# adahbingee/pais-mvs

Measured on AMD Instinct MI355X. Metric: refined+expanded patches/sec, higher is better.
Workload: dtype f64

## Files before the change

### include/pais_test_hooks.h

```cpp
#ifndef PAIS_TEST_HOOKS_H
#define PAIS_TEST_HOOKS_H

#include "pais_feature.h"
#include "pais_mvs.h"

#ifdef __cplusplus
extern "C" {
#endif

int  pais_mvs_emulate(pais_mvs *m, int mode, int rank, int world);

typedef int (*pais_record_source_fn)(void *user, int n, const pais_candidate *cands, pais_patch_result *out, int has_seeds);
int  pais_mvs_set_record_source(pais_mvs *m, pais_record_source_fn fn, void *user);

int  pais_mvs_test_inject(pais_mvs *m, int what, int count);

typedef struct pais_test_swarm {
    double range_l[3], range_u[3];
    double iw, gbest_fitness;
    uint64_t stream_base;
    int32_t n, max_iteration, iteration, g_idx, started, run, local_k, continues;
    double result[4];
} pais_test_swarm;
int  pais_test_swarm_step(int device, pais_test_swarm *s, double *swarm);

typedef struct pais_test_feature_sizes {
    int32_t octaves, W, H, layers;
    int64_t num_cands, num_fit, num_keypoints;
} pais_test_feature_sizes;
int  pais_test_feature_stages(int device, const uint8_t *gray, int width, int height, int64_t stride,
                              const pais_feature_params *prm, int octave, pais_test_feature_sizes *sizes,
                              int64_t layer_floats, float *layers, int max_cands, int32_t *cands, int32_t *fit_int, double *fit_val);

#ifdef __cplusplus
}
#endif
#endif
```

### pais_mvs_amd/csrc/pais_capi.hip

```cpp
#include <hip/hip_runtime.h>
#include <limits.h>
#include <math.h>
#include <stdarg.h>
#include <stddef.h>
#include <stdio.h>
#include <stdlib.h>
#include <string.h>

#include <string>
#include <utility>
#include <vector>
#include <algorithm>

#include "../../include/pais_hip.h"
#include "../../include/pais_test_hooks.h"
#include "pais_dev.hpp"
#include "pais_host.hpp"
#include "pais_internal.h"

static thread_local std::string g_err;
static int fail(const char *what, hipError_t e)
{
    char buf[512];
    snprintf(buf, sizeof(buf), "%s: %s", what, hipGetErrorString(e));
    g_err = buf;
    return -2;
}
static int fail_msg(const char *what)
{
    g_err = what;
    return -1;
}
__attribute__((format(printf, 1, 2))) static int fail_fmt(const char *fmt, ...)
{
    char buf[512];
    va_list ap;
    va_start(ap, fmt);
    vsnprintf(buf, sizeof(buf), fmt, ap);
    va_end(ap);
    return fail_msg(buf);
}
#define HIPCHK(call)                                   \
    do {                                               \
        hipError_t e__ = (call);                       \
        if (e__ != hipSuccess) return fail(#call, e__); \
    } while (0)

struct EventPair {
    hipEvent_t a, b;
};

struct pais_ctx;
struct Timed {
    pais_ctx *ctx = nullptr;
    hipStream_t st = nullptr;
    std::vector<EventPair> *into = nullptr;
    EventPair e{nullptr, nullptr};
    bool on = false;
    int begin(pais_ctx *c, hipStream_t s, std::vector<EventPair> *v);
    int end();
};
struct LaunchStats {
    double ms = 0;
    int64_t launches = 0, items = 0;
};
struct TimedLaunch {
    pais_ctx *ctx;
    EventPair e{nullptr, nullptr};
    explicit TimedLaunch(pais_ctx *c) : ctx(c) {}
    TimedLaunch(TimedLaunch &&o) noexcept : ctx(o.ctx), e(o.e) { o.e = EventPair{nullptr, nullptr}; }
    ~TimedLaunch();
    int begin();
    int end();
    void collect(LaunchStats &s, int64_t items, int64_t launches = 1);
};
struct TraceOut {
    pais_launch::TraceSink sink{nullptr, nullptr, nullptr, 1, 1};
    std::vector<TimedLaunch> passes;
    int64_t launches = 0;
};
struct PassPlan {
    struct Slice { int lo, hi, parts; pais_launch::BatchView v; pais_launch::TraceSink trace; };
    pais_launch::BatchView all{};
    int nSl = 0, S = 1, afterGrid = 0, itNext = 0;
    bool useIter = false, useTile = false, useRing = false, hasSeeds = false;
    bool usePre = false;
    int ringCUs = 0;
    Slice sl[16];
    int *cnt = nullptr, *nextCnt = nullptr;
    const pais_candidate *d_cands = nullptr;
    Timed tp;
    TraceOut *trace = nullptr;
};

struct pais_ctx {
    int device = 0;
    hipStream_t stream = nullptr;
    int numCUs = 256;
    size_t ldsLimit = 64 * 1024;
    DevScene sc;
    DevBuf<DevCamera> d_cams;
    DevBuf<uint8_t> d_img;
    DevBuf<PaisImgT> d_imgF;
    DevBuf<double> d_edge;
    bool edgesOnTheFly = false;
    DevBuf<double> d_gauss;
    size_t imgBytes = 0, edgeBytes = 0;
    std::vector<int> camMaxLod;
    DevBuf<pais_candidate> d_cands;
    DevBuf<pais_patch_result> d_recs;
    PinBuf<pais_candidate> h_cands;
    PinBuf<pais_patch_result> h_recs;
    DevBuf<double> d_hp;
    DevBuf<double> d_ratios;
    DevBuf<int> d_counters;
    unsigned passSerial = 0;
    bool countersDirty = false;
    DevBuf<unsigned char> d_evalBlocks;
    DevBuf<unsigned char> d_win;
    DevBuf<int> d_active;
    DevBuf<unsigned long long> d_stat;
    unsigned long long *stat = nullptr;
    PinBuf<int> h_counters;
    DevBuf<unsigned char> d_psoStates;
    long splitAbove = 0;
    int psoMinPer = 64;
    int evalParts = 0;
    double partFill = 0.5;
    int psoStreams = 2;
    pais_launch::TileOpts tile;
    int arithLiteral = 0;
    bool tileVerify = false;
    bool tileDebug = false;
    int tileMode = 1;
    long tileAbove = 512;
    std::vector<hipStream_t> sub;
    std::vector<hipEvent_t> subDone;
    hipEvent_t forkEv = nullptr;
    DevBuf<pais_patch_state> d_states;
    DevBuf<int32_t> d_idx;
    DevBuf<double> d_particles, d_out;
    DevBuf<pais_view_state> d_vStates;
    DevBuf<pais_view_result> d_vOut;
    DevBuf<double> d_vTables, d_vHp;
    LaunchStats ncc;
    DevBuf<pais_loaded_patch> d_lIn;
    DevBuf<pais_patch_result> d_lOut;
    LaunchStats load;
    DevBuf<pais_patch_state> d_dStates;
    DevBuf<int32_t> d_dIdx;
    DevBuf<double> d_dParticles, d_dWeight, d_dSad, d_dColour, d_dH;
    DevBuf<pais_cost_detail> d_dRec;
    DevBuf<int8_t> d_dCode;
    LaunchStats detail;
    DevBuf<pais_candidate> d_tCands;
    DevBuf<pais_patch_result> d_tRecs;
    DevBuf<pais_pso_run_info> d_tRuns;
    DevBuf<pais_pso_iter> d_tIters;
    DevBuf<double> d_tParts;
    DevBuf<unsigned long long> d_tStat;
    LaunchStats trace;
    DevBuf<double> d_nbC;
    DevBuf<int32_t> d_nbN;
    bool fineTiming = false;
    std::vector<EventPair> evPso, evBegin, evAfter, evEval, evEval2;
    std::vector<EventPair> evFree;
    double psoMs = 0, beginMs = 0, afterMs = 0, evalMs = 0, eval2Ms = 0;
    hipEvent_t refEv = nullptr;
    std::vector<std::pair<float, float>> eval2Intervals;
    int64_t psoLaunches = 0, evalLaunches = 0, eval2Launches = 0, tileLaunches = 0, ringLaunches = 0;
    pais_ctx *parent = nullptr;
    std::vector<pais_ctx *> lanes;
    int openBatch = -1;
    double ringPerCam = 1843.0;
    int ringMode = 1;
    int preMode = 1;
    DevBuf<double> d_pre;
    DevBuf<unsigned> d_ring;
    DevBuf<unsigned> d_ringCtl;
    PinBuf<unsigned> h_ringCtl;
    DevBuf<int> d_arrive;
    bool ringUsed = false;
    bool ringSuppressed = false;
    bool ringSuppressOnce = false;
    int ringPendingN = 0;
    double ringTimeoutMs = 10000.0;
    long ringSeedAbove = 0;
    size_t ringMaxBytes = (size_t)512 << 20;
    int64_t ringFallbacks = 0;
    std::vector<EventPair> evRing;
    double ringMs = 0;
    PassPlan plan;
    bool planDone = true;
    int roundHint = 0;
};

static void build_gauss(const pais_config &cfg, std::vector<double> &g)
{
    const int S = cfg.patchSize, r = cfg.patchRadius;
    g.assign((size_t)S * S, 0.0);
    const double sigma = cfg.distWeighting;
    const double s2 = 1.0 / (2.0 * sigma * sigma);
    const double s = 1.0 / (2.0 * M_PI * sigma * sigma);
    for (int x = 0; x < S; ++x)
        for (int y = 0; y < S; ++y) {
            double e = -(pow((double)(x - r), 2) + pow((double)(y - r), 2)) * s2;
            g[(size_t)x * S + y] = s * exp(e);
        }
    double n = 0;
    for (size_t i = 0; i < g.size(); ++i) n += g[i];
    const double inv = 1.0 / n;
    for (size_t i = 0; i < g.size(); ++i) g[i] = g[i] * inv;
}

static int apply_config(pais_ctx *ctx, const pais_config *cfg)
{
    pais_config c = *cfg;
    c.patchSize = (c.patchRadius << 1) + 1;
    if (c.patchRadius < 1 || c.patchRadius > 127) return fail_msg("patchRadius out of range");
    if (c.particleNum < 1 || c.particleNum * 2 > PAIS_MAX_PARTICLES) return fail_msg("particleNum out of range");
    if (c.maxLOD < 0 || c.maxLOD >= PAIS_MAX_LEVELS) return fail_msg("maxLOD out of range");
    if (c.minLOD < 0) return fail_msg("minLOD out of range (negative)");
    if (!(c.textureVariation > 0)) return fail_msg("textureVariation out of range (must be > 0)");
    if (!(c.lodRatio > 0 && c.lodRatio < 1)) return fail_msg("lodRatio out of range (must be inside (0, 1))");
    if (c.maxIteration < 1) return fail_msg("maxIteration out of range (must be >= 1)");
    if (c.cellSize < 1) return fail_msg("cellSize out of range (must be >= 1)");
    std::vector<double> g;
    build_gauss(c, g);
    if (ctx->d_gauss) HIPCHK(hipStreamSynchronize(ctx->stream));
    HIPCHK(ctx->d_gauss.alloc(g.size() * sizeof(double)));
    HIPCHK(hipMemcpy(ctx->d_gauss, g.data(), g.size() * sizeof(double), hipMemcpyHostToDevice));
    ctx->sc.cfg = c;
    ctx->sc.gauss = ctx->d_gauss;
    for (int l = 0; l < PAIS_MAX_LEVELS; ++l) ctx->sc.lodScale[l] = pow(c.lodRatio, l);
    return 0;
}

extern "C" const char *pais_last_error(void) { return g_err.c_str(); }
extern "C" size_t pais_sizeof_config(void) { return sizeof(pais_config); }
extern "C" size_t pais_sizeof_camera_desc(void) { return sizeof(pais_camera_desc); }
extern "C" size_t pais_sizeof_candidate(void) { return sizeof(pais_candidate); }
extern "C" size_t pais_sizeof_patch_result(void) { return sizeof(pais_patch_result); }
extern "C" size_t pais_sizeof_view_state(void) { return sizeof(pais_view_state); }
extern "C" size_t pais_sizeof_view_result(void) { return sizeof(pais_view_result); }
extern "C" size_t pais_sizeof_cost_detail(void) { return sizeof(pais_cost_detail); }
extern "C" size_t pais_sizeof_pso_run_info(void) { return sizeof(pais_pso_run_info); }
extern "C" size_t pais_sizeof_pso_iter(void) { return sizeof(pais_pso_iter); }
static_assert(offsetof(pais_pso_run_info, range_u) == 24 && offsetof(pais_pso_run_info, init) == 48 && offsetof(pais_pso_run_info, ray) == 72 &&
              offsetof(pais_pso_run_info, run) == 96 && offsetof(pais_pso_run_info, n_particles) == 112 &&
              offsetof(pais_pso_run_info, iterations) == 120 && offsetof(pais_pso_run_info, cam_idx) == 128 &&
              sizeof(pais_pso_run_info) == 128 + 4 * PAIS_MAX_VIS, "pais_pso_run_info layout");
static_assert(offsetof(pais_pso_iter, gbest) == 8 && offsetof(pais_pso_iter, iw) == 32 && offsetof(pais_pso_iter, dispersion) == 40 &&
              offsetof(pais_pso_iter, velocity) == 48 && offsetof(pais_pso_iter, g_idx) == 56 && offsetof(pais_pso_iter, ended) == 64 &&
              sizeof(pais_pso_iter) == 72, "pais_pso_iter layout");
extern "C" uint32_t pais_rand31(uint64_t seed, uint64_t key, uint32_t run, uint32_t k) { return pais::rand31(seed, key, run, k); }
extern "C" uint64_t pais_child_key(uint64_t parent_key, int cam, int cx, int cy) { return pais::child_key(parent_key, cam, cx, cy); }

static int ctx_init(pais_ctx *ctx, const pais_config *cfg, int num_cams, const pais_camera_desc *cams, int device, uint64_t pso_seed);
static int ctx_init_work(pais_ctx *ctx);
extern "C" int pais_ctx_create(const pais_config *cfg, int num_cams, const pais_camera_desc *cams, int device,
                               uint64_t pso_seed, pais_ctx **out)
{
    if (!cfg || !cams || !out || num_cams <= 0) return fail_msg("pais_ctx_create: bad argument");
    int ndev = 0;
    hipError_t e0 = hipGetDeviceCount(&ndev);
    if (e0 != hipSuccess || ndev <= 0) return fail_msg("pais_ctx_create: no HIP device (this library has no CPU path)");
    if (device < 0 || device >= ndev) return fail_msg("pais_ctx_create: bad device index");
    HIPCHK(hipSetDevice(device));
    pais_ctx *ctx = new pais_ctx();
    const int rc = ctx_init(ctx, cfg, num_cams, cams, device, pso_seed);
    if (rc) { pais_ctx_destroy(ctx); return rc; }
    *out = ctx;
    return 0;
}

static int ctx_init(pais_ctx *ctx, const pais_config *cfg, int num_cams, const pais_camera_desc *cams, int device, uint64_t pso_seed)
{
    ctx->device = device;
    memset(&ctx->sc, 0, sizeof(ctx->sc));
    hipDeviceProp_t prop;
    HIPCHK(hipGetDeviceProperties(&prop, device));
    ctx->numCUs = prop.multiProcessorCount > 0 ? prop.multiProcessorCount : 256;
    ctx->ldsLimit = prop.sharedMemPerBlock > 0 ? (size_t)prop.sharedMemPerBlock : 64 * 1024;
    HIPCHK(hipStreamCreateWithFlags(&ctx->stream, hipStreamNonBlocking));
    ctx->sc.seed = pso_seed;
    ctx->sc.numCams = num_cams;
    int rc = apply_config(ctx, cfg);
    if (rc) return rc;
    const bool wantEdge = cfg->adaptiveGradientEnable != 0;
    const bool edgesGiven = wantEdge && cams[0].level_edge[0] != nullptr;

    std::vector<DevCamera> hc((size_t)num_cams);
    std::vector<size_t> imgOff((size_t)num_cams * PAIS_MAX_LEVELS, 0), edgeOff((size_t)num_cams * PAIS_MAX_LEVELS, 0);
    size_t imgBytes = 0, edgeBytes = 0;
    for (int c = 0; c < num_cams; ++c) {
        const pais_camera_desc &d = cams[c];
        if (d.max_lod < 0 || d.max_lod >= PAIS_MAX_LEVELS) return fail_msg("camera max_lod out of range");
        for (int l = 0; l <= d.max_lod; ++l) {
            if (!d.level_image[l] || d.level_width[l] <= 0 || d.level_height[l] <= 0) return fail_msg("camera level missing");
            if (d.level_width[l] > 65535 || d.level_height[l] > 65535) return fail_msg("camera level larger than 65535 pixels in one dimension");
            size_t px = (size_t)d.level_width[l] * d.level_height[l];
            if (px >= ((size_t)1 << 29)) return fail_msg("camera level of 2^29 pixels or more (32-bit tap offsets inside a level)");
            imgOff[(size_t)c * PAIS_MAX_LEVELS + l] = imgBytes;
            imgBytes = (imgBytes + px + 16 + 255) & ~(size_t)255;
            if (wantEdge && edgesGiven) {
                if (!d.level_edge[l]) return fail_msg("level_edge given for some levels only");
                edgeOff[(size_t)c * PAIS_MAX_LEVELS + l] = edgeBytes;
                edgeBytes = (edgeBytes + px * sizeof(double) + 255) & ~(size_t)255;
            }
        }
    }
    if (imgBytes >= ((size_t)1 << 40)) return fail_msg("pyramids of 2^40 bytes or more (a level's start is packed into 40 bits next to its homography)");
    HIPCHK(ctx->d_img.alloc(imgBytes));
    HIPCHK(hipMemsetAsync(ctx->d_img, 0, imgBytes, ctx->stream));
    for (int c = 0; c < num_cams; ++c) {
        const pais_camera_desc &d = cams[c];
        for (int l = 0; l <= d.max_lod; ++l) {
            const int w = d.level_width[l], h = d.level_height[l];
            const size_t stride = d.level_stride[l] > 0 ? (size_t)d.level_stride[l] : (size_t)w;
            HIPCHK(hipMemcpy2DAsync(ctx->d_img + imgOff[(size_t)c * PAIS_MAX_LEVELS + l], (size_t)w, d.level_image[l], stride, (size_t)w,
                                    (size_t)h, hipMemcpyHostToDevice, ctx->stream));
        }
    }
    ctx->imgBytes = imgBytes;
    {
        size_t maxMB = 256;
        if (const char *e = getenv("PAIS_TAP_FLOAT_MAX_MB")) maxMB = (size_t)strtoull(e, nullptr, 10);
        if (imgBytes <= (maxMB << 20)) {
            HIPCHK(ctx->d_imgF.alloc(imgBytes * sizeof(PaisImgT)));
            HIPCHK(pais_launch::expand_image(ctx->d_img, ctx->d_imgF, imgBytes, ctx->stream));
        }
    }
    if (wantEdge && edgesGiven && edgeBytes) {
        HIPCHK(ctx->d_edge.alloc(edgeBytes));
        for (int c = 0; c < num_cams; ++c) {
            const pais_camera_desc &d = cams[c];
            for (int l = 0; l <= d.max_lod; ++l) {
                size_t px = (size_t)d.level_width[l] * d.level_height[l];
                HIPCHK(hipMemcpyAsync((uint8_t *)ctx->d_edge.p + edgeOff[(size_t)c * PAIS_MAX_LEVELS + l], d.level_edge[l],
                                      px * sizeof(double), hipMemcpyHostToDevice, ctx->stream));
            }
        }
        ctx->edgeBytes = edgeBytes;
    }
    std::vector<unsigned long long> mm;
    if (wantEdge && !edgesGiven) {
        mm.assign((size_t)num_cams * PAIS_MAX_LEVELS * 2, 0ULL);
        for (size_t i = 0; i < mm.size(); i += 2) mm[i] = ~0ULL;
        DevBuf<unsigned long long> d_mm;
        HIPCHK(d_mm.alloc(mm.size() * sizeof(unsigned long long)));
        HIPCHK(hipMemcpyAsync(d_mm, mm.data(), mm.size() * sizeof(unsigned long long), hipMemcpyHostToDevice, ctx->stream));
        for (int c = 0; c < num_cams; ++c)
            for (int l = 0; l <= cams[c].max_lod; ++l)
                HIPCHK(pais_launch::level_edge_minmax(ctx->d_img + imgOff[(size_t)c * PAIS_MAX_LEVELS + l], cams[c].level_width[l],
                                                      cams[c].level_height[l], d_mm + ((size_t)c * PAIS_MAX_LEVELS + l) * 2, ctx->stream));
        HIPCHK(hipMemcpyAsync(mm.data(), d_mm, mm.size() * sizeof(unsigned long long), hipMemcpyDeviceToHost, ctx->stream));
        HIPCHK(hipStreamSynchronize(ctx->stream));
    }
    HIPCHK(hipStreamSynchronize(ctx->stream));
    ctx->edgesOnTheFly = wantEdge && !edgesGiven;
    for (int c = 0; c < num_cams; ++c) {
        const pais_camera_desc &d = cams[c];
        DevCamera &h = hc[c];
        memset(&h, 0, sizeof(h));
        memcpy(h.KR, d.KR, sizeof(h.KR));
        memcpy(h.KT, d.KT, sizeof(h.KT));
        memcpy(h.R, d.rotation, sizeof(h.R));
        memcpy(h.T, d.translation, sizeof(h.T));
        memcpy(h.C, d.center, sizeof(h.C));
        memcpy(h.optN, d.optical_normal, sizeof(h.optN));
        h.focal[0] = d.focal[0]; h.focal[1] = d.focal[1];
        h.pp[0] = d.principle_point[0]; h.pp[1] = d.principle_point[1];
        h.maxLOD = d.max_lod;
        ctx->camMaxLod.push_back(d.max_lod);
        for (int l = 0; l <= d.max_lod; ++l) {
            h.w[l] = d.level_width[l];
            h.h[l] = d.level_height[l];
            h.imgOff[l] = (uint64_t)imgOff[(size_t)c * PAIS_MAX_LEVELS + l];
            h.edgeOff[l] = (uint64_t)(edgeOff[(size_t)c * PAIS_MAX_LEVELS + l] / sizeof(double));
            if (!mm.empty()) {
                const unsigned long long lo = mm[((size_t)c * PAIS_MAX_LEVELS + l) * 2], hi = mm[((size_t)c * PAIS_MAX_LEVELS + l) * 2 + 1];
                memcpy(&h.edgeMin[l], &lo, 8);
                memcpy(&h.edgeMax[l], &hi, 8);
            }
        }
    }
    HIPCHK(ctx->d_cams.alloc(sizeof(DevCamera) * (size_t)num_cams));
    HIPCHK(hipMemcpy(ctx->d_cams, hc.data(), sizeof(DevCamera) * (size_t)num_cams, hipMemcpyHostToDevice));
    ctx->sc.cams = ctx->d_cams;
    ctx->sc.imgBlob = ctx->d_img;
    ctx->sc.imgF = ctx->d_imgF;
    ctx->sc.edgeBlob = ctx->d_edge;

    return ctx_init_work(ctx);
}

template <typename T> static void env_int(const char *name, T &v, long lo = LONG_MIN, long hi = LONG_MAX)
{
    const char *e = getenv(name);
    if (!e) return;
    const long x = atol(e);
    if (x >= lo && x <= hi) v = (T)x;
}
template <typename T> static void env_flag(const char *name, T &v)
{
    if (const char *e = getenv(name)) v = atoi(e) != 0;
}
static void env_real(const char *name, double &v, bool positiveOnly = false)
{
    const char *e = getenv(name);
    if (!e) return;
    const double x = atof(e);
    if (!positiveOnly || x > 0) v = x;
}
static int staging_chunk(const char *envName, int n, size_t perItemBytes)
{
    double mb = 256.0;
    env_real(envName, mb);
    const size_t bound = (size_t)std::max(0.0, mb * 1048576.0);
    return (int)std::min((size_t)n, std::max((size_t)1, bound / perItemBytes));
}

static int ctx_init_work(pais_ctx *ctx)
{
    HIPCHK(ctx->d_counters.alloc(sizeof(int) * 8));
    HIPCHK(hipMemset(ctx->d_counters, 0, sizeof(int) * 8));
    HIPCHK(ctx->d_stat.alloc(sizeof(unsigned long long) * 24));
    HIPCHK(hipMemset(ctx->d_stat, 0, sizeof(unsigned long long) * 24));
    ctx->stat = ctx->d_stat;
    HIPCHK(ctx->h_counters.alloc(sizeof(int) * 4));
    HIPCHK(ctx->d_ringCtl.alloc(PAIS_RING_CTL_BYTES * PAIS_RINGS));
    HIPCHK(hipMemset(ctx->d_ringCtl, 0, PAIS_RING_CTL_BYTES * PAIS_RINGS));
    HIPCHK(ctx->h_ringCtl.alloc(PAIS_RING_CTL_BYTES * PAIS_RINGS));
    memset(ctx->h_ringCtl, 0, PAIS_RING_CTL_BYTES * PAIS_RINGS);
    ctx->splitAbove = 3L * ctx->numCUs * 12;
    env_int("PAIS_EVAL_PARTS", ctx->evalParts, 1, 4);
    if (ctx->evalParts == 3) ctx->evalParts = 0;
    env_real("PAIS_PART_FILL", ctx->partFill, true);
    env_int("PAIS_SPLIT_ABOVE", ctx->splitAbove, 1);
    env_int("PAIS_PSO_MINPER", ctx->psoMinPer, 1, INT_MAX);
    env_int("PAIS_PSO_STREAMS", ctx->psoStreams, 1, 16);
    env_int("PAIS_PSO_RING", ctx->ringMode, INT_MIN, INT_MAX);
    env_int("PAIS_PRE_SETUP", ctx->preMode, INT_MIN, INT_MAX);
    env_real("PAIS_RING_PER_CAM", ctx->ringPerCam);
    env_int("PAIS_RING_SEED_ABOVE", ctx->ringSeedAbove);
    long ringMaxMB = 0;
    env_int("PAIS_RING_MAX_MB", ringMaxMB, 1);
    if (ringMaxMB) ctx->ringMaxBytes = (size_t)ringMaxMB << 20;
    env_int("PAIS_TILE", ctx->tileMode, INT_MIN, INT_MAX);
    env_flag("PAIS_TILE_DEBUG", ctx->tileDebug);
    env_flag("PAIS_TILE_VERIFY", ctx->tileVerify);
    env_int("PAIS_TILE_STRIP_SPLIT", ctx->tile.stripSteps, 1, INT_MAX);
    env_flag("PAIS_TILE_NOTILES", ctx->tile.noTiles);
    env_int("PAIS_TILE_ABOVE", ctx->tileAbove, 1);
    env_flag("PAIS_FINE_TIMING", ctx->fineTiming);
    if (const char *e = getenv("PAIS_ARITH")) ctx->arithLiteral = (strcmp(e, "literal") == 0);
    if (const char *e = getenv("PAIS_RING_TIMEOUT_MS")) {
        const double v = atof(e);
        if (v == 0.0 && e[0] == '0') ctx->ringTimeoutMs = 0.0;
        else if (v >= 1.0 && v <= 600000.0) ctx->ringTimeoutMs = v;
        else fprintf(stderr, "pais: PAIS_RING_TIMEOUT_MS=%s ignored (0, or 1 .. 600000 ms)\n", e);
    }
    HIPCHK(hipEventCreateWithFlags(&ctx->forkEv, hipEventDisableTiming));
    for (int i = 0; i + 1 < ctx->psoStreams; ++i) {
        hipStream_t st; hipEvent_t ev;
        HIPCHK(hipStreamCreateWithFlags(&st, hipStreamNonBlocking));
        HIPCHK(hipEventCreateWithFlags(&ev, hipEventDisableTiming));
        ctx->sub.push_back(st);
        ctx->subDone.push_back(ev);
    }
    return 0;
}

extern "C" void pais_ctx_destroy(pais_ctx *ctx)
{
    if (!ctx) return;
    (void)hipSetDevice(ctx->device);
    if (ctx->parent) {
        auto &v = ctx->parent->lanes;
        for (size_t i = 0; i < v.size(); ++i)
            if (v[i] == ctx) { v.erase(v.begin() + (long)i); break; }
        ctx->parent = nullptr;
    }
    while (!ctx->lanes.empty()) {
        pais_ctx *l = ctx->lanes.back();
        ctx->lanes.pop_back();
        l->parent = nullptr;
        pais_ctx_destroy(l);
    }
    if (ctx->stream) (void)hipStreamSynchronize(ctx->stream);
    for (auto *v : {&ctx->evPso, &ctx->evBegin, &ctx->evAfter, &ctx->evEval, &ctx->evEval2, &ctx->evRing, &ctx->evFree})
        for (auto &p : *v) { (void)hipEventDestroy(p.a); (void)hipEventDestroy(p.b); }
    for (auto st : ctx->sub) (void)hipStreamDestroy(st);
    for (auto ev : ctx->subDone) (void)hipEventDestroy(ev);
    if (ctx->forkEv) (void)hipEventDestroy(ctx->forkEv);
    if (ctx->refEv) (void)hipEventDestroy(ctx->refEv);
    pais_launch::ring_profile_print();
    if (ctx->stream) (void)hipStreamDestroy(ctx->stream);
    delete ctx;
}

extern "C" int pais_ctx_set_config(pais_ctx *ctx, const pais_config *cfg)
{
    if (!ctx || !cfg) return fail_msg("pais_ctx_set_config: bad argument");
    HIPCHK(hipSetDevice(ctx->device));
    if (cfg->adaptiveGradientEnable && !ctx->d_edge && !ctx->edgesOnTheFly)
        return fail_msg("adaptiveGradientEnable needs the gradient weighting enabled at create time (edge pyramids or their on-the-fly statistics)");
    if (ctx->parent) return fail_msg("pais_ctx_set_config: a lane takes its configuration from its parent");
    if (ctx->openBatch >= 0) return fail_msg("pais_ctx_set_config: a batch is open on this context");
    for (pais_ctx *l : ctx->lanes)
        if (l->openBatch >= 0) return fail_msg("pais_ctx_set_config: a batch is open on a lane of this context");
    for (pais_ctx *l : ctx->lanes) HIPCHK(hipStreamSynchronize(l->stream));
    int rc = apply_config(ctx, cfg);
    if (rc) return rc;
    for (pais_ctx *l : ctx->lanes) {
        l->sc.cfg = ctx->sc.cfg;
        l->sc.gauss = ctx->sc.gauss;
        for (int i = 0; i < PAIS_MAX_LEVELS; ++i) l->sc.lodScale[i] = ctx->sc.lodScale[i];
    }
    return 0;
}

extern "C" int pais_ctx_fork_lane(pais_ctx *parent, pais_ctx **out)
{
    if (!parent || !out) return fail_msg("pais_ctx_fork_lane: bad argument");
    if (parent->parent) return fail_msg("pais_ctx_fork_lane: a lane cannot be forked");
    HIPCHK(hipSetDevice(parent->device));
    pais_ctx *l = new pais_ctx();
    l->device = parent->device;
    l->numCUs = parent->numCUs;
    l->ldsLimit = parent->ldsLimit;
    l->camMaxLod = parent->camMaxLod;
    l->sc = parent->sc;
    l->edgesOnTheFly = parent->edgesOnTheFly;
    l->imgBytes = parent->imgBytes;
    l->edgeBytes = parent->edgeBytes;
    hipError_t e = hipStreamCreateWithFlags(&l->stream, hipStreamNonBlocking);
    if (e != hipSuccess) { delete l; return fail("hipStreamCreateWithFlags", e); }
    const int rc = ctx_init_work(l);
    if (rc) { pais_ctx_destroy(l); return rc; }
    l->fineTiming = parent->fineTiming;
    l->parent = parent;
    parent->lanes.push_back(l);
    *out = l;
    return 0;
}

extern "C" int pais_ctx_set_neighbor_radius(pais_ctx *ctx, double r)
{
    if (!ctx) return fail_msg("bad ctx");
    ctx->sc.cfg.neighborRadius = r;
    for (pais_ctx *l : ctx->lanes) l->sc.cfg.neighborRadius = r;
    return 0;
}

extern "C" void *pais_ctx_stream(pais_ctx *ctx) { return ctx ? (void *)ctx->stream : nullptr; }
extern "C" int pais_ctx_synchronize(pais_ctx *ctx)
{
    if (!ctx) return fail_msg("bad ctx");
    HIPCHK(hipSetDevice(ctx->device));
    HIPCHK(hipStreamSynchronize(ctx->stream));
    return 0;
}

static int get_event_pair(pais_ctx *ctx, EventPair &p)
{
    if (!ctx->evFree.empty()) {
        p = ctx->evFree.back();
        ctx->evFree.pop_back();
        return 0;
    }
    EventPair q{nullptr, nullptr};
    HIPCHK(hipEventCreate(&q.a));
    const hipError_t e = hipEventCreate(&q.b);
    if (e != hipSuccess) { (void)hipEventDestroy(q.a); return fail("hipEventCreate", e); }
    p = q;
    return 0;
}
static int drain_events(pais_ctx *ctx, std::vector<EventPair> &v, double &acc)
{
    for (auto &p : v) {
        float ms = 0;
        HIPCHK(hipEventElapsedTime(&ms, p.a, p.b));
        acc += ms;
        ctx->evFree.push_back(p);
    }
    v.clear();
    return 0;
}
int Timed::begin(pais_ctx *c, hipStream_t s, std::vector<EventPair> *v)
{
    ctx = c; st = s; into = v; on = c->fineTiming;
    if (!on) return 0;
    if (get_event_pair(c, e)) return -2;
    HIPCHK(hipEventRecord(e.a, s));
    return 0;
}
int Timed::end()
{
    if (!on) return 0;
    HIPCHK(hipEventRecord(e.b, st));
    into->push_back(e);
    return 0;
}

TimedLaunch::~TimedLaunch()
{
    if (e.a) ctx->evFree.push_back(e);
}
int TimedLaunch::begin()
{
    if (get_event_pair(ctx, e)) return -2;
    HIPCHK(hipEventRecord(e.a, ctx->stream));
    return 0;
}
int TimedLaunch::end()
{
    HIPCHK(hipEventRecord(e.b, ctx->stream));
    return 0;
}
void TimedLaunch::collect(LaunchStats &s, int64_t items, int64_t launches)
{
    float ms = 0;
    if (hipEventElapsedTime(&ms, e.a, e.b) == hipSuccess) s.ms += ms;
    s.launches += launches;
    s.items += items;
}

static int read_launch_stats(LaunchStats *s, const char *who, double *kernel_ms, int64_t *launches, int64_t *items, int reset)
{
    if (!s) return fail_fmt("%s: bad argument", who);
    if (kernel_ms) *kernel_ms = s->ms;
    if (launches) *launches = s->launches;
    if (items) *items = s->items;
    if (reset) *s = LaunchStats();
    return 0;
}

struct CamListRules {
    const char *who, *noun;
    int minCam;
    bool distinct;
    enum Ref {
        NoRef,
        AnyLevel,
        OwnLevels
    } ref;
};
static const CamListRules kFitnessRules = {"pais_fitness_batch", "state", 1, false, CamListRules::AnyLevel};
static const CamListRules kDetailRules = {"pais_fitness_detail", "state", 1, false, CamListRules::AnyLevel};
static const CamListRules kNccRules = {"pais_ncc_batch", "state", 2, true, CamListRules::OwnLevels};
static CamListRules candidate_rules(const char *who) { return CamListRules{who, "candidate", 0, false, CamListRules::NoRef}; }

static int check_cam_list(const pais_ctx *ctx, const CamListRules &R, int i, int num_cam, const int32_t *cam_idx, int ref_cam, int lod)
{
    const int nc = ctx->sc.numCams;
    if (num_cam < R.minCam || num_cam > PAIS_MAX_VIS)
        return fail_fmt("%s: %s %d: num_cam %d outside [%d, %d]", R.who, R.noun, i, num_cam, R.minCam, PAIS_MAX_VIS);
    if (R.ref != CamListRules::NoRef && (ref_cam < 0 || ref_cam >= nc))
        return fail_fmt("%s: %s %d: ref_cam %d out of range [0, %d)", R.who, R.noun, i, ref_cam, nc);
    for (int k = 0; k < num_cam; ++k) {
        const int c = cam_idx[k];
        bool twice = false;
        for (int j = 0; R.distinct && j < k; ++j) twice = twice || cam_idx[j] == c;
        if (c >= 0 && c < nc && !twice) continue;
        if (R.distinct)
            return fail_fmt("%s: %s %d: %s (cam_idx[%d] = %d)", R.who, R.noun, i, c < 0 || c >= nc ? "cam_idx out of range" : "duplicate camera in cam_idx",
                            k, c);
        return fail_fmt("%s: %s %d: cam_idx[%d] = %d out of range [0, %d)", R.who, R.noun, i, k, c, nc);
    }
    if (R.ref == CamListRules::AnyLevel && (lod < 0 || lod >= PAIS_MAX_LEVELS))
        return fail_fmt("%s: %s %d: lod %d outside [0, %d)", R.who, R.noun, i, lod, PAIS_MAX_LEVELS);
    if (R.ref == CamListRules::OwnLevels) {
        int maxLod = ctx->camMaxLod[ref_cam], lim = ref_cam;
        for (int k = 0; k < num_cam; ++k)
            if (ctx->camMaxLod[cam_idx[k]] < maxLod) {
                maxLod = ctx->camMaxLod[cam_idx[k]];
                lim = cam_idx[k];
            }
        if (lod < 0 || lod > maxLod)
            return fail_fmt("%s: %s %d: lod %d outside [0, %d] (max_lod of camera %d)", R.who, R.noun, i, lod, maxLod, lim);
    }
    return 0;
}

static int check_states(const pais_ctx *ctx, const CamListRules &R, int n_states, const pais_patch_state *states, int n_evals,
                        const int32_t *state_index, int &Kmax)
{
    Kmax = 1;
    for (int i = 0; i < n_states; ++i) {
        const pais_patch_state &s = states[i];
        const int rc = check_cam_list(ctx, R, i, s.num_cam, s.cam_idx, s.ref_cam, s.lod);
        if (rc) return rc;
        Kmax = std::max(Kmax, (int)s.num_cam);
    }
    for (int e = 0; e < n_evals; ++e)
        if (state_index[e] < 0 || state_index[e] >= n_states)
            return fail_fmt("%s: state_index[%d] = %d out of range [0, %d)", R.who, e, state_index[e], n_states);
    return 0;
}

static int check_candidates(const pais_ctx *ctx, const char *who, int n, const pais_candidate *cands, int &Kmax, int &hasSeeds)
{
    const CamListRules R = candidate_rules(who);
    Kmax = 1;
    hasSeeds = 0;
    for (int i = 0; i < n; ++i) {
        const pais_candidate &c = cands[i];
        const int rc = check_cam_list(ctx, R, i, c.num_cam, c.cam_idx, 0, 0);
        if (rc) return rc;
        if (c.type != PAIS_TYPE_SEED && c.type != PAIS_TYPE_EXPAND)
            return fail_fmt("%s: candidate %d: type %d is neither PAIS_TYPE_SEED nor PAIS_TYPE_EXPAND", who, i, c.type);
        Kmax = std::max(Kmax, (int)c.num_cam);
        if (c.type == PAIS_TYPE_SEED) hasSeeds = 1;
    }
    return 0;
}

extern "C" int pais_neighbor_count(pais_ctx *ctx, int n, const double *centers, double radius, int32_t *counts, double *kernel_ms)
{
    if (!ctx || n < 0 || (n && (!centers || !counts))) return fail_msg("pais_neighbor_count: bad argument");
    if (kernel_ms) *kernel_ms = 0;
    if (n == 0) return 0;
    HIPCHK(hipSetDevice(ctx->device));
    HIPCHK(ctx->d_nbC.reserve(ctx->stream, sizeof(double) * 3 * (size_t)n));
    HIPCHK(ctx->d_nbN.reserve(ctx->stream, sizeof(int32_t) * (size_t)n));
    HIPCHK(hipMemcpyAsync(ctx->d_nbC, centers, sizeof(double) * 3 * (size_t)n, hipMemcpyHostToDevice, ctx->stream));
    TimedLaunch t(ctx);
    if (t.begin()) return -2;
    HIPCHK(pais_launch::neighbor_count(ctx->d_nbC, n, radius, ctx->d_nbN, ctx->stream));
    if (t.end()) return -2;
    HIPCHK(hipMemcpyAsync(counts, ctx->d_nbN, sizeof(int32_t) * (size_t)n, hipMemcpyDeviceToHost, ctx->stream));
    HIPCHK(hipStreamSynchronize(ctx->stream));
    LaunchStats s;
    t.collect(s, n);
    if (kernel_ms) *kernel_ms = s.ms;
    return 0;
}

extern "C" int pais_ctx_set_fine_timing(pais_ctx *ctx, int on)
{
    if (!ctx) return fail_msg("pais_ctx_set_fine_timing: bad argument");
    if (on && !ctx->parent) {
        HIPCHK(hipSetDevice(ctx->device));
        if (!ctx->refEv) HIPCHK(hipEventCreate(&ctx->refEv));
        HIPCHK(hipEventRecord(ctx->refEv, ctx->stream));
        HIPCHK(hipStreamSynchronize(ctx->stream));
    }
    ctx->fineTiming = on != 0;
    for (pais_ctx *l : ctx->lanes) l->fineTiming = on != 0;
    return 0;
}

extern "C" int pais_fitness_batch(pais_ctx *ctx, int n_states, const pais_patch_state *states, int n_evals,
                                  const int32_t *state_index, const double *particles, double *out)
{
    if (!ctx || n_states < 0 || n_evals < 0) return fail_msg("pais_fitness_batch: bad argument");
    if (n_evals == 0) return 0;
    if (!states || !state_index || !particles || !out) return fail_msg("pais_fitness_batch: null pointer");
    HIPCHK(hipSetDevice(ctx->device));
    int Kmax = 1;
    const int rc = check_states(ctx, kFitnessRules, n_states, states, n_evals, state_index, Kmax);
    if (rc) return rc;
    HIPCHK(ctx->d_states.reserve(ctx->stream, sizeof(pais_patch_state) * (size_t)n_states));
    HIPCHK(ctx->d_idx.reserve(ctx->stream, sizeof(int32_t) * (size_t)n_evals));
    HIPCHK(ctx->d_particles.reserve(ctx->stream, sizeof(double) * 3 * (size_t)n_evals));
    HIPCHK(ctx->d_out.reserve(ctx->stream, sizeof(double) * (size_t)n_evals));
    HIPCHK(ctx->d_evalBlocks.reserve(ctx->stream, pais_launch::eval_block_bytes_host(Kmax) * (size_t)n_states));
    HIPCHK(ctx->d_win.reserve(ctx->stream, pais_launch::win_bytes_per_candidate(ctx->sc) * (size_t)n_states));
    HIPCHK(hipMemcpyAsync(ctx->d_states, states, sizeof(pais_patch_state) * (size_t)n_states, hipMemcpyHostToDevice, ctx->stream));
    HIPCHK(hipMemcpyAsync(ctx->d_idx, state_index, sizeof(int32_t) * (size_t)n_evals, hipMemcpyHostToDevice, ctx->stream));
    HIPCHK(hipMemcpyAsync(ctx->d_particles, particles, sizeof(double) * 3 * (size_t)n_evals, hipMemcpyHostToDevice, ctx->stream));
    Timed tf;
    if (tf.begin(ctx, ctx->stream, &ctx->evEval)) return -2;
    HIPCHK(pais_launch::fitness(ctx->sc, ctx->d_states, n_states, ctx->d_idx, ctx->d_particles, ctx->d_out, n_evals, Kmax,
                                ctx->d_evalBlocks, ctx->d_win, ctx->arithLiteral, ctx->stream));
    if (tf.end()) return -2;
    ctx->evalLaunches++;
    HIPCHK(hipMemcpyAsync(out, ctx->d_out, sizeof(double) * (size_t)n_evals, hipMemcpyDeviceToHost, ctx->stream));
    HIPCHK(hipStreamSynchronize(ctx->stream));
    return 0;
}

extern "C" int pais_ncc_batch(pais_ctx *ctx, int n, const pais_view_state *states, pais_view_result *out, double *tables, int stride)
{
    if (!ctx || n < 0) return fail_msg("pais_ncc_batch: bad argument");
    if (n == 0) return 0;
    if (!states || !out) return fail_msg("pais_ncc_batch: null pointer");
    if (tables && stride < 2) return fail_msg("pais_ncc_batch: table stride below 2");
    int Kmax = 2;
    for (int i = 0; i < n; ++i) {
        const pais_view_state &v = states[i];
        const int rc = check_cam_list(ctx, kNccRules, i, v.num_cam, v.cam_idx, v.ref_cam, v.lod);
        if (rc) return rc;
        if (tables && stride < v.num_cam) return fail_fmt("pais_ncc_batch: state %d: table stride %d below num_cam %d", i, stride, v.num_cam);
        Kmax = std::max(Kmax, (int)v.num_cam);
    }
    HIPCHK(hipSetDevice(ctx->device));
    const DevScene &sc = ctx->sc;
    const size_t hpBytes = sizeof(double) * (size_t)Kmax * sc.cfg.patchSize * sc.cfg.patchSize;
    const int hpInLds = (pais_launch::hp_in_lds(sc, Kmax) && pais_launch::ncc_lds_bytes(Kmax) + hpBytes <= ctx->ldsLimit) ? 1 : 0;
    long grid = (long)ctx->numCUs * (hpInLds ? 8 : 2);
    if (!hpInLds) {
        const long cap = (long)(((size_t)256 << 20) / hpBytes);
        grid = std::min(grid, std::max(1L, cap));
    }
    grid = std::min(grid, (long)n);
    const size_t tableBytes = tables ? sizeof(double) * (size_t)stride * stride * (size_t)n : 0;
    HIPCHK(ctx->d_vStates.reserve(ctx->stream, sizeof(pais_view_state) * (size_t)n));
    HIPCHK(ctx->d_vOut.reserve(ctx->stream, sizeof(pais_view_result) * (size_t)n));
    if (tables) HIPCHK(ctx->d_vTables.reserve(ctx->stream, tableBytes));
    if (!hpInLds) HIPCHK(ctx->d_vHp.reserve(ctx->stream, hpBytes * (size_t)grid));
    HIPCHK(hipMemcpyAsync(ctx->d_vStates, states, sizeof(pais_view_state) * (size_t)n, hipMemcpyHostToDevice, ctx->stream));
    TimedLaunch t(ctx);
    if (t.begin()) return -2;
    HIPCHK(pais_launch::ncc_batch(sc, ctx->d_vStates, n, ctx->d_vOut, tables ? ctx->d_vTables.p : nullptr, stride, ctx->d_vHp, (int)grid, Kmax,
                                  hpInLds, ctx->stream));
    if (t.end()) return -2;
    HIPCHK(hipMemcpyAsync(out, ctx->d_vOut, sizeof(pais_view_result) * (size_t)n, hipMemcpyDeviceToHost, ctx->stream));
    if (tables) HIPCHK(hipMemcpyAsync(tables, ctx->d_vTables, tableBytes, hipMemcpyDeviceToHost, ctx->stream));
    HIPCHK(hipStreamSynchronize(ctx->stream));
    t.collect(ctx->ncc, n);
    return 0;
}

extern "C" int pais_get_ncc_stats(pais_ctx *ctx, double *kernel_ms, int64_t *launches, int64_t *states, int reset)
{
    return read_launch_stats(ctx ? &ctx->ncc : nullptr, "pais_get_ncc_stats", kernel_ms, launches, states, reset);
}

static const CamListRules kLoadRules = {"pais_load_state_batch", "patch", 0, false, CamListRules::NoRef};

extern "C" int pais_load_state_batch(pais_ctx *ctx, int n, const pais_loaded_patch *in, pais_patch_result *out)
{
    if (n < 0) return fail_msg("pais_load_state_batch: bad argument (n < 0)");
    if (n == 0) return 0;
    const char *missing = !ctx ? "ctx" : !in ? "in" : !out ? "out" : nullptr;
    if (missing) return fail_fmt("pais_load_state_batch: null pointer (%s)", missing);
    for (int i = 0; i < n; ++i) {
        const int rc = check_cam_list(ctx, kLoadRules, i, in[i].num_cam, in[i].cam_idx, 0, 0);
        if (rc) return rc;
    }
    HIPCHK(hipSetDevice(ctx->device));
    const int chunk = staging_chunk("PAIS_LOAD_STAGING_MB", n, sizeof(pais_loaded_patch) + sizeof(pais_patch_result));
    HIPCHK(ctx->d_lIn.reserve(ctx->stream, sizeof(pais_loaded_patch) * (size_t)chunk));
    HIPCHK(ctx->d_lOut.reserve(ctx->stream, sizeof(pais_patch_result) * (size_t)chunk));
    for (int c0 = 0; c0 < n; c0 += chunk) {
        const int m = std::min(chunk, n - c0);
        HIPCHK(hipMemcpyAsync(ctx->d_lIn, in + c0, sizeof(pais_loaded_patch) * (size_t)m, hipMemcpyHostToDevice, ctx->stream));
        TimedLaunch t(ctx);
        if (t.begin()) return -2;
        HIPCHK(pais_launch::load_state(ctx->sc, ctx->d_lIn, ctx->d_lOut, m, (uint64_t)c0, ctx->stream));
        if (t.end()) return -2;
        HIPCHK(hipMemcpyAsync(out + c0, ctx->d_lOut, sizeof(pais_patch_result) * (size_t)m, hipMemcpyDeviceToHost, ctx->stream));
        HIPCHK(hipStreamSynchronize(ctx->stream));
        t.collect(ctx->load, m);
    }
    return 0;
}

extern "C" int pais_get_load_stats(pais_ctx *ctx, double *kernel_ms, int64_t *launches, int64_t *patches, int reset)
{
    return read_launch_stats(ctx ? &ctx->load : nullptr, "pais_get_load_stats", kernel_ms, launches, patches, reset);
}
extern "C" size_t pais_sizeof_loaded_patch(void) { return sizeof(pais_loaded_patch); }

extern "C" int pais_fitness_detail(pais_ctx *ctx, int n_states, const pais_patch_state *states, int n_evals, const int32_t *state_index,
                                   const double *particles, pais_cost_detail *out, double *weight, double *avg_sad, int8_t *pixel_code,
                                   double *colour, double *homographies, int cam_stride)
{
    if (!ctx || n_states < 0 || n_evals < 0) return fail_msg("pais_fitness_detail: bad argument");
    if (n_evals == 0) return 0;
    const char *missing = !states ? "states" : !state_index ? "state_index" : !particles ? "particles" : !out ? "out" : !weight ? "weight"
                          : !avg_sad ? "avg_sad" : !pixel_code ? "pixel_code" : nullptr;
    if (missing) return fail_fmt("pais_fitness_detail: null pointer (%s)", missing);
    int Kmax = 1;
    const int rc = check_states(ctx, kDetailRules, n_states, states, n_evals, state_index, Kmax);
    if (rc) return rc;
    for (int i = 0; (colour || homographies) && i < n_states; ++i)
        if (cam_stride < states[i].num_cam)
            return fail_fmt("pais_fitness_detail: state %d: cam_stride %d below num_cam %d", i, cam_stride, states[i].num_cam);
    HIPCHK(hipSetDevice(ctx->device));
    const DevScene &sc = ctx->sc;
    const size_t S2 = (size_t)sc.cfg.patchSize * sc.cfg.patchSize;
    const size_t perEval = sizeof(pais_cost_detail) + sizeof(int32_t) + 3 * sizeof(double) + S2 * (2 * sizeof(double) + 1) +
                           (colour ? sizeof(double) * (size_t)Kmax * S2 : 0) + (homographies ? sizeof(double) * 9 * (size_t)Kmax : 0);
    const int chunk = staging_chunk("PAIS_DETAIL_STAGING_MB", n_evals, perEval);
    hipStream_t st = ctx->stream;
    HIPCHK(ctx->d_dStates.reserve(st, sizeof(pais_patch_state) * (size_t)n_states));
    HIPCHK(ctx->d_evalBlocks.reserve(st, pais_launch::eval_block_bytes_host(Kmax) * (size_t)n_states));
    HIPCHK(ctx->d_win.reserve(st, pais_launch::win_bytes_per_candidate(sc) * (size_t)n_states));
    HIPCHK(ctx->d_dIdx.reserve(st, sizeof(int32_t) * (size_t)chunk));
    HIPCHK(ctx->d_dParticles.reserve(st, 3 * sizeof(double) * (size_t)chunk));
    HIPCHK(ctx->d_dRec.reserve(st, sizeof(pais_cost_detail) * (size_t)chunk));
    HIPCHK(ctx->d_dWeight.reserve(st, sizeof(double) * S2 * chunk));
    HIPCHK(ctx->d_dSad.reserve(st, sizeof(double) * S2 * chunk));
    HIPCHK(ctx->d_dCode.reserve(st, S2 * chunk));
    if (colour) HIPCHK(ctx->d_dColour.reserve(st, sizeof(double) * (size_t)Kmax * S2 * chunk));
    if (homographies) HIPCHK(ctx->d_dH.reserve(st, sizeof(double) * 9 * (size_t)Kmax * chunk));
    HIPCHK(hipMemcpyAsync(ctx->d_dStates, states, sizeof(pais_patch_state) * (size_t)n_states, hipMemcpyHostToDevice, ctx->stream));
    HIPCHK(pais_launch::state_blocks(sc, ctx->d_dStates, n_states, Kmax, ctx->d_evalBlocks, ctx->d_win, ctx->stream));
    std::vector<double> hCol(colour ? (size_t)Kmax * S2 * chunk : 0), hH(homographies ? (size_t)9 * Kmax * chunk : 0);
    for (int c0 = 0; c0 < n_evals; c0 += chunk) {
        const int n = std::min(chunk, n_evals - c0);
        HIPCHK(hipMemcpyAsync(ctx->d_dIdx, state_index + c0, sizeof(int32_t) * (size_t)n, hipMemcpyHostToDevice, ctx->stream));
        HIPCHK(hipMemcpyAsync(ctx->d_dParticles, particles + 3 * (size_t)c0, 3 * sizeof(double) * (size_t)n, hipMemcpyHostToDevice, ctx->stream));
        TimedLaunch t(ctx);
        if (t.begin()) return -2;
        HIPCHK(pais_launch::fitness_detail(sc, ctx->d_dIdx, ctx->d_dParticles, n, Kmax, ctx->d_evalBlocks, ctx->d_dRec, ctx->d_dWeight, ctx->d_dSad,
                                           ctx->d_dCode, colour ? ctx->d_dColour.p : nullptr, homographies ? ctx->d_dH.p : nullptr, ctx->stream));
        if (t.end()) return -2;
        HIPCHK(hipMemcpyAsync(out + c0, ctx->d_dRec, sizeof(pais_cost_detail) * (size_t)n, hipMemcpyDeviceToHost, ctx->stream));
        HIPCHK(hipMemcpyAsync(weight + S2 * c0, ctx->d_dWeight, sizeof(double) * S2 * n, hipMemcpyDeviceToHost, ctx->stream));
        HIPCHK(hipMemcpyAsync(avg_sad + S2 * c0, ctx->d_dSad, sizeof(double) * S2 * n, hipMemcpyDeviceToHost, ctx->stream));
        HIPCHK(hipMemcpyAsync(pixel_code + S2 * c0, ctx->d_dCode, S2 * n, hipMemcpyDeviceToHost, ctx->stream));
        if (colour) HIPCHK(hipMemcpyAsync(hCol.data(), ctx->d_dColour, sizeof(double) * (size_t)Kmax * S2 * n, hipMemcpyDeviceToHost, ctx->stream));
        if (homographies) HIPCHK(hipMemcpyAsync(hH.data(), ctx->d_dH, sizeof(double) * 9 * (size_t)Kmax * n, hipMemcpyDeviceToHost, ctx->stream));
        HIPCHK(hipStreamSynchronize(ctx->stream));
        t.collect(ctx->detail, n);
        for (int e = 0; e < n; ++e) {
            const size_t K = (size_t)states[state_index[c0 + e]].num_cam, g = (size_t)c0 + e;
            if (colour) memcpy(colour + g * cam_stride * S2, hCol.data() + (size_t)e * Kmax * S2, sizeof(double) * K * S2);
            if (homographies) memcpy(homographies + g * cam_stride * 9, hH.data() + (size_t)e * Kmax * 9, sizeof(double) * K * 9);
        }
    }
    return 0;
}

extern "C" int pais_get_detail_stats(pais_ctx *ctx, double *kernel_ms, int64_t *launches, int64_t *evals, int reset)
{
    return read_launch_stats(ctx ? &ctx->detail : nullptr, "pais_get_detail_stats", kernel_ms, launches, evals, reset);
}

static int pass_open(pais_ctx *ctx, PassPlan &P, int pass, int againCount)
{
    const DevScene &sc = ctx->sc;
    P.cnt = ctx->d_counters + 4 * (ctx->passSerial & 1);
    P.nextCnt = ctx->d_counters + 4 * ((ctx->passSerial + 1) & 1);
    ctx->passSerial++;
    if (P.tp.begin(ctx, ctx->stream, &ctx->evPso)) return -2;
    if (pass > 0)
        HIPCHK(pais_launch::pso_init(sc, P.all, ctx->d_active, P.cnt + 2));
    const bool tileOk = (ctx->tileMode == 2 || (ctx->tileMode == 1 && ctx->sc.imgF == nullptr)) && pais_launch::tile_eligible(P.all.Kmax);
    const int n = P.all.n, Nmax = P.all.Nmax;
    const int nPlan = ctx->roundHint > n ? ctx->roundHint : n;
    P.useIter = Nmax <= 64 && (long)nPlan * Nmax < (tileOk ? ctx->tileAbove : ctx->splitAbove);
    P.useTile = tileOk && !P.useIter;
    if (ctx->arithLiteral) P.useIter = P.useTile = false;
    const long ringWaves = (long)(P.hasSeeds && pass > 0 ? againCount : n) * Nmax;
    const size_t ringNeed = pais_launch::ring_words(n, Nmax, P.all.maxIt) * sizeof(unsigned);
    P.useRing = ctx->ringMode != 0 && !ctx->arithLiteral && !ctx->ringSuppressed && !P.useTile && Nmax <= 64 && n < (1 << 24) && ringNeed <= ctx->ringMaxBytes &&
                (P.hasSeeds ? (ctx->ringSeedAbove > 0 && ringWaves >= ctx->ringSeedAbove)
                            : (!P.useIter && ringWaves >= (long)(ctx->ringPerCam * P.all.Kmax)));
    if (P.useRing && nPlan > n && ctx->ringMode != 3) P.useRing = false;
    if (P.trace) P.useIter = P.useTile = P.useRing = false;
    if (P.useRing) P.useIter = false;
    P.ringCUs = ctx->numCUs;
    if (P.useRing) {
        HIPCHK(ctx->d_ring.reserve(ctx->stream, ringNeed));
        HIPCHK(ctx->d_arrive.reserve(ctx->stream, sizeof(int) * PAIS_ARRIVE_STRIDE * (size_t)n));
    }
    P.usePre = ctx->preMode != 0 && !ctx->arithLiteral && !P.useIter && !P.useTile && !(P.useRing && !pais_launch::pre_ring_ok(P.all.Kmax)) && !P.trace;
    P.all.pre = nullptr;
    if (P.usePre) {
        HIPCHK(ctx->d_pre.reserve(ctx->stream, pais_launch::pre_bytes_per_candidate(Nmax, P.all.Kmax) * (size_t)n));
        P.all.pre = ctx->d_pre;
        HIPCHK(pais_launch::pso_setup0(sc, P.all));
    }
    const int nRun = P.useIter ? (pass == 0 ? n : againCount) : n;
    int S = P.useRing ? 1 : ctx->psoStreams;
    if (nPlan > n) S = (int)((double)S * n / nPlan + 0.5);
    const int minPer = ctx->psoMinPer;
    if (nRun < S * minPer) S = (nRun + minPer - 1) / minPer;
    if (S < 1 || P.trace) S = 1;
    P.S = S;
    if (S > 1) HIPCHK(hipEventRecord(ctx->forkEv, ctx->stream));
    P.nSl = 0;
    for (int sI = 0; sI < S; ++sI) {
        PassPlan::Slice q;
        q.lo = (int)((long)nRun * sI / S);
        q.hi = (int)((long)nRun * (sI + 1) / S);
        if (q.hi <= q.lo) continue;
        const bool own = (S == 1) || (sI == 0);
        const hipStream_t st = own ? ctx->stream : ctx->sub[sI - 1];
        if (!own) HIPCHK(hipStreamWaitEvent(st, ctx->forkEv, 0));
        q.v = P.useIter ? P.all.slice(sc, 0, n, st) : P.all.slice(sc, q.lo, q.hi, st);
        q.trace = pais_launch::TraceSink{nullptr, nullptr, nullptr, 1, 1};
        if (P.trace) {
            const pais_launch::TraceSink &t = P.trace->sink;
            const size_t slot0 = (size_t)q.lo * t.maxRuns;
            q.trace = pais_launch::TraceSink{t.runs + slot0, t.iters + slot0 * t.rows, t.particles ? t.particles + slot0 * t.rows * Nmax * 11 : nullptr,
                                             t.maxRuns, t.rows};
        }
        q.parts = 1;
        if (P.useIter) {
            const long waves = (long)(q.hi - q.lo) * Nmax, resident = (long)((double)ctx->numCUs * 16 * ctx->partFill * n / nPlan);
            q.parts = ctx->evalParts > 0 ? ctx->evalParts : (waves * 4 <= resident ? 4 : (waves * 2 <= resident ? 2 : 1));
        }
        P.sl[P.nSl++] = q;
    }
    P.itNext = 0;
    return 0;
}

static int pass_iterations(pais_ctx *ctx, PassPlan &P, int itEnd)
{
    const DevScene &sc = ctx->sc;
    if (itEnd > P.all.maxIt + 1) itEnd = P.all.maxIt + 1;
    if (P.useRing) {
        if (P.itNext == 0 && itEnd > 0) {
            const unsigned long long ticks = (unsigned long long)(ctx->ringTimeoutMs * 1e5);
            auto ring = [&](int phase) {
                return pais_launch::pso_ring(sc, P.all, ctx->d_ring, ctx->d_ringCtl, ctx->d_arrive, ctx->stat, P.ringCUs, phase, ticks);
            };
            HIPCHK(ring(0));
            Timed te;
            if (te.begin(ctx, ctx->stream, &ctx->evRing)) return -2;
            HIPCHK(ring(1));
            if (te.end()) return -2;
            HIPCHK(hipMemcpyAsync(ctx->h_ringCtl, ctx->d_ringCtl, PAIS_RING_CTL_BYTES * PAIS_RINGS, hipMemcpyDeviceToHost, ctx->stream));
            ctx->ringUsed = true;
            ctx->evalLaunches++;
            ctx->eval2Launches++;
            ctx->ringLaunches++;
            P.itNext = P.all.maxIt + 1;
        }
        return 0;
    }
    TimedLaunch tpass(ctx);
    const bool timePass = P.trace && itEnd > P.itNext;
    if (timePass && tpass.begin()) return -2;
    for (int it = P.itNext; it < itEnd; ++it) {
        for (int k = 0; k < P.nSl; ++k) {
            const PassPlan::Slice &q = P.sl[k];
            Timed te;
            if (te.begin(ctx, q.v.stream, P.useIter ? &ctx->evEval : &ctx->evEval2)) return -2;
            if (P.useIter)
                HIPCHK(pais_launch::pso_iter(sc, q.v, ctx->d_active, P.cnt + 2, q.lo, q.hi, ctx->stat, it, 0, q.parts));
            else if (P.useTile) {
                HIPCHK(pais_launch::pso_tile(sc, q.v, ctx->tile, ctx->tileDebug ? ctx->stat + 8 : nullptr));
                HIPCHK(pais_launch::pso_eval(sc, q.v, ctx->tileVerify ? 2 : 1, ctx->stat + 18));
            } else if (ctx->arithLiteral)
                HIPCHK(pais_launch::pso_eval_literal(sc, q.v));
            else
                HIPCHK(pais_launch::pso_eval(sc, q.v, 0, nullptr));
            if (te.end()) return -2;
            ctx->evalLaunches++;
            if (!P.useIter) ctx->eval2Launches++;
            if (P.useTile) ctx->tileLaunches++;
            if (P.trace) {
                HIPCHK(pais_launch::pso_step_trace(sc, q.v, ctx->stat, q.trace));
                P.trace->launches++;
            } else if (!P.useIter)
                HIPCHK(pais_launch::pso_step(sc, q.v, ctx->stat));
        }
    }
    if (timePass) {
        if (tpass.end()) return -2;
        P.trace->passes.push_back(std::move(tpass));
    }
    if (itEnd > P.itNext) P.itNext = itEnd;
    return 0;
}

static int pass_join(pais_ctx *ctx, PassPlan &P)
{
    for (int sI = 1; sI < P.S; ++sI) {
        bool used = false;
        for (int k = 0; k < P.nSl; ++k) used = used || (P.sl[k].v.stream == ctx->sub[sI - 1]);
        if (!used) continue;
        HIPCHK(hipEventRecord(ctx->subDone[sI - 1], ctx->sub[sI - 1]));
        HIPCHK(hipStreamWaitEvent(ctx->stream, ctx->subDone[sI - 1], 0));
    }
    P.S = 1;
    return 0;
}

static int pass_close(pais_ctx *ctx, PassPlan &P)
{
    const DevScene &sc = ctx->sc;
    for (int k = 0; k < P.nSl; ++k) {
        const PassPlan::Slice &q = P.sl[k];
        if (P.useIter)
            HIPCHK(pais_launch::pso_iter(sc, q.v, ctx->d_active, P.cnt + 2, q.lo, q.hi, ctx->stat, P.all.maxIt + 1, 1, q.parts));
    }
    if (pass_join(ctx, P)) return -2;
    if (P.tp.end()) return -2;
    ctx->psoLaunches++;
    Timed ta;
    if (ta.begin(ctx, ctx->stream, &ctx->evAfter)) return -2;
    HIPCHK(pais_launch::after(sc, P.all.recs, P.all.n, ctx->d_hp, P.afterGrid, P.cnt, ctx->stat, P.all.Kmax, ctx->d_ratios, P.nextCnt, ctx->stream));
    if (ta.end()) return -2;
    return 0;
}

static int batch_setup(pais_ctx *ctx, PassPlan &P, int n, const pais_candidate *d_cands, pais_patch_result *d_out, int max_num_cam, int has_seeds)
{
    HIPCHK(hipSetDevice(ctx->device));
    const DevScene &sc = ctx->sc;
    int Kmax = max_num_cam > 0 ? max_num_cam : sc.numCams;
    if (Kmax > PAIS_MAX_VIS) Kmax = PAIS_MAX_VIS;
    if (Kmax > sc.numCams) Kmax = sc.numCams;
    if (Kmax < 1) Kmax = 1;
    const int Nmax = has_seeds ? sc.cfg.particleNum * 2 : sc.cfg.particleNum;
    const int S2 = sc.cfg.patchSize * sc.cfg.patchSize;
    const int afterGrid = n < 2048 ? n : 2048;
    {
        size_t hpNeed = (size_t)afterGrid * Kmax * S2 * sizeof(double);
        const size_t full = (size_t)2048 * Kmax * S2 * sizeof(double);
        if (hpNeed > ctx->d_hp.bytes && full < ((size_t)1 << 31)) hpNeed = full;
        HIPCHK(ctx->d_hp.reserve(ctx->stream, hpNeed));
    }
    HIPCHK(ctx->d_active.reserve(ctx->stream, sizeof(int) * (size_t)n));
    HIPCHK(ctx->d_evalBlocks.reserve(ctx->stream, pais_launch::eval_block_bytes_host(Kmax) * (size_t)n));
    HIPCHK(ctx->d_win.reserve(ctx->stream, pais_launch::win_bytes_per_candidate(sc) * (size_t)n));
    HIPCHK(ctx->d_psoStates.reserve(ctx->stream, pais_launch::pso_state_bytes_host(Nmax) * (size_t)n));
    HIPCHK(ctx->d_ratios.reserve(ctx->stream, sizeof(double) * PAIS_MAX_VIS * (size_t)n));
    P.all = pais_launch::BatchView{d_out, ctx->d_psoStates, ctx->d_evalBlocks, ctx->d_win, nullptr, n, Nmax, Kmax,
                                   has_seeds ? sc.cfg.maxIteration * 2 : sc.cfg.maxIteration, ctx->stream};
    P.hasSeeds = has_seeds != 0;
    P.afterGrid = afterGrid;
    P.d_cands = d_cands;

    if (ctx->countersDirty) HIPCHK(hipMemsetAsync(ctx->d_counters, 0, sizeof(int) * 8, ctx->stream));
    ctx->countersDirty = true;
    Timed tb;
    if (tb.begin(ctx, ctx->stream, &ctx->evBegin)) return -2;
    HIPCHK(pais_launch::begin(sc, P.all, d_cands, ctx->d_active, ctx->d_counters + 4 * (ctx->passSerial & 1) + 2));
    if (tb.end()) return -2;
    return 0;
}

static int ring_failed(pais_ctx *ctx, int n)
{
    if (!ctx->ringUsed) return 0;
    ctx->ringUsed = false;
    unsigned done = 0, err = 0;
    for (int r = 0; r < PAIS_RINGS; ++r) { done += ctx->h_ringCtl[(PAIS_RING_CTL_BYTES / 4) * r + PAIS_RING_CTL_DONE_WORD]; err |= ctx->h_ringCtl[(PAIS_RING_CTL_BYTES / 4) * r + PAIS_RING_CTL_ERROR_WORD]; }
    if (err == 0 && done == (unsigned)n) return 0;
    ctx->ringFallbacks++;
    if (getenv("PAIS_RING_VERBOSE") || (ctx->ringFallbacks == 1 && ctx->ringTimeoutMs > 0))
        fprintf(stderr, "[pais] k_pso_ring did not complete (error %u, %u of %d runs ended): the batch is re-run with one launch per iteration\n", err, done, n);
    return 1;
}

static int refine_device_once(pais_ctx *ctx, int n, const pais_candidate *d_cands, pais_patch_result *d_out, int max_num_cam, int has_seeds,
                              bool defer = false, TraceOut *trace = nullptr)
{
    PassPlan &P = ctx->plan;
    P.trace = trace;
    ctx->ringUsed = false;
    ctx->ringPendingN = 0;
    int rc = batch_setup(ctx, P, n, d_cands, d_out, max_num_cam, has_seeds);
    int againCount = 0;
    const int maxPass = has_seeds ? (PAIS_MAX_VIS + 2) : 1;
    for (int pass = 0; !rc && pass < maxPass; ++pass) {
        if ((rc = pass_open(ctx, P, pass, againCount)) != 0) break;
        if ((rc = pass_iterations(ctx, P, P.all.maxIt + 1)) != 0) { (void)pass_join(ctx, P); break; }
        if ((rc = pass_close(ctx, P)) != 0) break;
        if (!has_seeds && !ctx->ringUsed) break;
        if (!has_seeds && defer) { ctx->ringPendingN = n; break; }
        if (has_seeds) HIPCHK(hipMemcpyAsync(ctx->h_counters, P.cnt, sizeof(int) * 2, hipMemcpyDeviceToHost, ctx->stream));
        HIPCHK(hipStreamSynchronize(ctx->stream));
        if (ring_failed(ctx, n)) { ctx->roundHint = 0; return 1; }
        if (!has_seeds || ctx->h_counters[1] == 0) break;
        againCount = ctx->h_counters[1];
    }
    ctx->roundHint = 0;
    if (rc) return rc;
    ctx->countersDirty = false;
    return 0;
}

static int rerun_without_ring(pais_ctx *ctx, int n, const pais_candidate *d_cands, pais_patch_result *d_out, int max_num_cam, int has_seeds,
                              bool defer, int hint)
{
    ctx->ringSuppressed = true;
    ctx->countersDirty = true;
    ctx->roundHint = hint;
    const int rc = refine_device_once(ctx, n, d_cands, d_out, max_num_cam, has_seeds, defer);
    ctx->ringSuppressed = false;
    return rc;
}

static int refine_device(pais_ctx *ctx, int n, const pais_candidate *d_cands, pais_patch_result *d_out, int max_num_cam, int has_seeds, bool defer)
{
    const int hint = ctx->roundHint;
    const int rc = refine_device_once(ctx, n, d_cands, d_out, max_num_cam, has_seeds, defer);
    return rc == 1 ? rerun_without_ring(ctx, n, d_cands, d_out, max_num_cam, has_seeds, defer, hint) : rc;
}

extern "C" int pais_refine_batch_device(pais_ctx *ctx, int n, const pais_candidate *d_cands, pais_patch_result *d_out,
                                        int max_num_cam, int has_seeds)
{
    if (!ctx || n < 0) return fail_msg("pais_refine_batch_device: bad argument");
    if (n == 0) return 0;
    if (!d_cands || !d_out) return fail_msg("pais_refine_batch_device: null pointer");
    if (ctx->openBatch >= 0) return fail_msg("pais_refine_batch_device: a batch is open on this context");
    return refine_device(ctx, n, d_cands, d_out, max_num_cam, has_seeds, false);
}

extern "C" int pais_refine_batch_device_async(pais_ctx *ctx, int n, const pais_candidate *d_cands, pais_patch_result *d_out,
                                              int max_num_cam, int has_seeds)
{
    if (!ctx || n < 0) return fail_msg("pais_refine_batch_device_async: bad argument");
    if (n == 0) return 0;
    if (!d_cands || !d_out) return fail_msg("pais_refine_batch_device_async: null pointer");
    if (ctx->openBatch >= 0) return fail_msg("pais_refine_batch_device_async: a batch is open on this context");
    if (ctx->ringSuppressOnce) {
        ctx->ringSuppressOnce = false;
        return rerun_without_ring(ctx, n, d_cands, d_out, max_num_cam, has_seeds, true, ctx->roundHint);
    }
    return refine_device(ctx, n, d_cands, d_out, max_num_cam, has_seeds, true);
}

extern "C" int pais_ctx_batch_status(pais_ctx *ctx)
{
    if (!ctx) return fail_msg("pais_ctx_batch_status: bad argument");
    if (ctx->ringPendingN <= 0) return 0;
    const int n = ctx->ringPendingN;
    ctx->ringPendingN = 0;
    ctx->countersDirty = false;
    if (!ring_failed(ctx, n)) return 0;
    ctx->countersDirty = true;
    ctx->ringSuppressOnce = true;
    return 1;
}

extern "C" int pais_wire_header_device(pais_ctx *ctx, int rank, int count, int host_rc, uint32_t user_word, void *d_header)
{
    if (!ctx || !d_header) return fail_msg("pais_wire_header_device: bad argument");
    HIPCHK(hipSetDevice(ctx->device));
    HIPCHK(pais_launch::wire_header(d_header, ctx->ringPendingN > 0 ? ctx->d_ringCtl : nullptr, ctx->ringPendingN, rank, count, host_rc, user_word, ctx->stream));
    return 0;
}

extern "C" int pais_test_swarm_step(int device, pais_test_swarm *s, double *swarm)
{
    hipError_t e = hipSetDevice(device);
    if (e != hipSuccess) return (int)e;
    return pais_launch::test_swarm_step(s, swarm);
}

extern "C" int pais_ctx_set_round_hint(pais_ctx *ctx, int n_round)
{
    if (!ctx) return fail_msg("pais_ctx_set_round_hint: bad argument");
    ctx->roundHint = n_round > 0 ? n_round : 0;
    return 0;
}

extern "C" int pais_refine_batch_view(pais_ctx *ctx, int n, const pais_candidate *cands, const pais_patch_result **view)
{
    if (!ctx || n < 0) return fail_msg("pais_refine_batch: bad argument");
    if (n == 0) return 0;
    if (!cands || !view) return fail_msg("pais_refine_batch: null pointer");
    int rc = pais_refine_batch_begin(ctx, n, cands);
    if (rc) return rc;
    return pais_refine_batch_end(ctx, view);
}

extern "C" int pais_refine_batch_begin(pais_ctx *ctx, int n, const pais_candidate *cands)
{
    int rc = pais_refine_batch_open(ctx, n, cands, 1 << 20);
    if (rc) return rc;
    rc = pais_refine_batch_enqueue(ctx, 0);
    return rc < 0 ? rc : 0;
}

extern "C" int pais_refine_batch_enqueue(pais_ctx *ctx, int iterations)
{
    if (!ctx) return fail_msg("pais_refine_batch_enqueue: bad argument");
    if (ctx->openBatch < 0) return fail_msg("pais_refine_batch_enqueue: no batch is open on this context");
    if (ctx->planDone) return 1;
    HIPCHK(hipSetDevice(ctx->device));
    PassPlan &P = ctx->plan;
    const int itEnd = iterations > 0 && iterations < P.all.maxIt + 1 - P.itNext ? P.itNext + iterations : P.all.maxIt + 1;
    int rc = pass_iterations(ctx, P, itEnd);
    if (!rc && P.itNext <= P.all.maxIt) return 0;
    if (!rc) rc = pass_close(ctx, P);
    if (rc) { (void)pass_join(ctx, P); ctx->openBatch = -1; ctx->ringUsed = false; return rc; }
    ctx->countersDirty = false;
    HIPCHK(hipMemcpyAsync(ctx->h_recs, ctx->d_recs, sizeof(pais_patch_result) * (size_t)ctx->openBatch, hipMemcpyDeviceToHost, ctx->stream));
    ctx->planDone = true;
    return 1;
}

extern "C" int pais_refine_batch_end(pais_ctx *ctx, const pais_patch_result **view)
{
    if (!ctx || !view) return fail_msg("pais_refine_batch_end: bad argument");
    if (ctx->openBatch < 0) return fail_msg("pais_refine_batch_end: no batch is open on this context");
    if (!ctx->planDone) {
        const int rc = pais_refine_batch_enqueue(ctx, 0);
        if (rc < 0) return rc;
    }
    ctx->openBatch = -1;
    HIPCHK(hipSetDevice(ctx->device));
    HIPCHK(hipStreamSynchronize(ctx->stream));
    if (ring_failed(ctx, ctx->plan.all.n)) {
        const int n = ctx->plan.all.n;
        const int rc = rerun_without_ring(ctx, n, ctx->d_cands, ctx->d_recs, ctx->plan.all.Kmax, 0, false, ctx->roundHint);
        if (rc) return rc;
        HIPCHK(hipMemcpyAsync(ctx->h_recs, ctx->d_recs, sizeof(pais_patch_result) * (size_t)n, hipMemcpyDeviceToHost, ctx->stream));
        HIPCHK(hipStreamSynchronize(ctx->stream));
    }
    *view = ctx->h_recs;
    return 0;
}

extern "C" int pais_refine_batch_open(pais_ctx *ctx, int n, const pais_candidate *cands, int iterations)
{
    if (!ctx || n <= 0 || !cands) return fail_msg("pais_refine_batch_begin: bad argument");
    if (ctx->openBatch >= 0) return fail_msg("pais_refine_batch_begin: a batch is open on this context already");
    HIPCHK(hipSetDevice(ctx->device));
    ctx->ringUsed = false;
    int Kmax = 1, hasSeeds = 0;
    int rc = check_candidates(ctx, "pais_refine_batch", n, cands, Kmax, hasSeeds);
    if (rc) return rc;
    HIPCHK(ctx->d_cands.reserve(ctx->stream, sizeof(pais_candidate) * (size_t)n));
    HIPCHK(ctx->d_recs.reserve(ctx->stream, sizeof(pais_patch_result) * (size_t)n));
    HIPCHK(ctx->h_cands.reserve(ctx->stream, sizeof(pais_candidate) * (size_t)n));
    HIPCHK(ctx->h_recs.reserve(ctx->stream, sizeof(pais_patch_result) * (size_t)n));
    memcpy(ctx->h_cands, cands, sizeof(pais_candidate) * (size_t)n);
    HIPCHK(hipMemcpyAsync(ctx->d_cands, ctx->h_cands, sizeof(pais_candidate) * (size_t)n, hipMemcpyHostToDevice, ctx->stream));
    if (hasSeeds) {
        rc = pais_refine_batch_device(ctx, n, ctx->d_cands, ctx->d_recs, Kmax, 1);
        if (rc) return rc;
        HIPCHK(hipMemcpyAsync(ctx->h_recs, ctx->d_recs, sizeof(pais_patch_result) * (size_t)n, hipMemcpyDeviceToHost, ctx->stream));
        ctx->openBatch = n;
        ctx->planDone = true;
        return 0;
    }
    PassPlan &P = ctx->plan;
    rc = batch_setup(ctx, P, n, ctx->d_cands, ctx->d_recs, Kmax, 0);
    if (!rc) rc = pass_open(ctx, P, 0, 0);
    ctx->roundHint = 0;
    if (!rc && (rc = pass_iterations(ctx, P, iterations > 0 ? iterations : 0)) != 0) (void)pass_join(ctx, P);
    if (rc) { ctx->ringUsed = false; return rc; }
    ctx->openBatch = n;
    ctx->planDone = false;
    return 0;
}

extern "C" int pais_refine_batch(pais_ctx *ctx, int n, const pais_candidate *cands, pais_patch_result *out)
{
    if (n > 0 && !out) return fail_msg("pais_refine_batch: null pointer");
    const pais_patch_result *view = nullptr;
    int rc = pais_refine_batch_view(ctx, n, cands, &view);
    if (rc || n <= 0) return rc;
    memcpy(out, view, sizeof(pais_patch_result) * (size_t)n);
    return 0;
}

extern "C" int pais_pso_trace_shape(pais_ctx *ctx, int n, const pais_candidate *cands, int *rows_per_run, int *particles_per_row)
{
    if (!ctx || n < 0 || !rows_per_run || !particles_per_row) return fail_msg("pais_pso_trace_shape: bad argument");
    if (n > 0 && !cands) return fail_msg("pais_pso_trace_shape: null pointer (cands)");
    int Kmax = 1, hasSeeds = 0;
    const int rc = check_candidates(ctx, "pais_pso_trace_shape", n, cands, Kmax, hasSeeds);
    if (rc) return rc;
    const pais_config &cfg = ctx->sc.cfg;
    *rows_per_run = (hasSeeds ? 2 * cfg.maxIteration : cfg.maxIteration) + 1;
    *particles_per_row = hasSeeds ? 2 * cfg.particleNum : cfg.particleNum;
    return 0;
}

struct TraceScope {
    pais_ctx *ctx;
    unsigned long long *stat;
    bool fine, ringUsed;
    int roundHint, ringPendingN;
    int64_t launches[6];
    explicit TraceScope(pais_ctx *c) : ctx(c)
    {
        stat = c->stat;
        c->stat = c->d_tStat;
        fine = c->fineTiming;
        c->fineTiming = false;
        ringUsed = c->ringUsed;
        ringPendingN = c->ringPendingN;
        roundHint = c->roundHint;
        c->roundHint = 0;
        const int64_t l[6] = {c->psoLaunches, c->evalLaunches, c->eval2Launches, c->tileLaunches, c->ringLaunches, c->ringFallbacks};
        memcpy(launches, l, sizeof(launches));
    }
    ~TraceScope()
    {
        ctx->stat = stat;
        ctx->fineTiming = fine;
        ctx->ringUsed = ringUsed;
        ctx->ringPendingN = ringPendingN;
        ctx->roundHint = roundHint;
        ctx->psoLaunches = launches[0];
        ctx->evalLaunches = launches[1];
        ctx->eval2Launches = launches[2];
        ctx->tileLaunches = launches[3];
        ctx->ringLaunches = launches[4];
        ctx->ringFallbacks = launches[5];
        ctx->plan.trace = nullptr;
    }
};

extern "C" int pais_pso_trace(pais_ctx *ctx, int n, const pais_candidate *cands, int max_runs, pais_patch_result *out,
                              pais_pso_run_info *runs, pais_pso_iter *iters, double *particles)
{
    if (n == 0) return 0;
    if (!ctx) return fail_msg("pais_pso_trace: null pointer (ctx)");
    if (n < 0) return fail_msg("pais_pso_trace: n < 0");
    const char *missing = !cands ? "cands" : !out ? "out" : !runs ? "runs" : !iters ? "iters" : nullptr;
    if (missing) return fail_fmt("pais_pso_trace: null pointer (%s)", missing);
    if (max_runs < 1) return fail_fmt("pais_pso_trace: max_runs %d < 1", max_runs);
    if (ctx->openBatch >= 0) return fail_msg("pais_pso_trace: a stepwise batch is open on this context (pais_refine_batch_open .. _end)");
    int Kmax = 1, hasSeeds = 0;
    int rc = check_candidates(ctx, "pais_pso_trace", n, cands, Kmax, hasSeeds);
    if (rc) return rc;
    HIPCHK(hipSetDevice(ctx->device));
    const pais_config &cfg = ctx->sc.cfg;
    const int rows = (hasSeeds ? 2 * cfg.maxIteration : cfg.maxIteration) + 1;
    const int NP = hasSeeds ? 2 * cfg.particleNum : cfg.particleNum;
    const size_t runRows = (size_t)max_runs * rows;
    const size_t perCand = sizeof(pais_candidate) + sizeof(pais_patch_result) + (size_t)max_runs * sizeof(pais_pso_run_info) +
                           runRows * sizeof(pais_pso_iter) + (particles ? runRows * NP * 11 * sizeof(double) : 0);
    const int chunk = staging_chunk("PAIS_TRACE_STAGING_MB", n, perCand);
    if (!ctx->d_tStat) {
        HIPCHK(ctx->d_tStat.alloc(sizeof(unsigned long long) * 24));
        HIPCHK(hipMemset(ctx->d_tStat, 0, sizeof(unsigned long long) * 24));
    }
    HIPCHK(ctx->d_tCands.reserve(ctx->stream, sizeof(pais_candidate) * (size_t)chunk));
    HIPCHK(ctx->d_tRecs.reserve(ctx->stream, sizeof(pais_patch_result) * (size_t)chunk));
    HIPCHK(ctx->d_tRuns.reserve(ctx->stream, sizeof(pais_pso_run_info) * (size_t)max_runs * chunk));
    HIPCHK(ctx->d_tIters.reserve(ctx->stream, sizeof(pais_pso_iter) * runRows * chunk));
    if (particles) HIPCHK(ctx->d_tParts.reserve(ctx->stream, sizeof(double) * 11 * runRows * NP * chunk));
    TraceScope scope(ctx);
    for (int c0 = 0; c0 < n; c0 += chunk) {
        const int m = std::min(chunk, n - c0);
        const size_t nRuns = (size_t)max_runs * m;
        HIPCHK(hipMemcpyAsync(ctx->d_tCands, cands + c0, sizeof(pais_candidate) * (size_t)m, hipMemcpyHostToDevice, ctx->stream));
        HIPCHK(hipMemsetAsync(ctx->d_tRuns, 0, sizeof(pais_pso_run_info) * nRuns, ctx->stream));
        HIPCHK(hipMemsetAsync(ctx->d_tIters, 0, sizeof(pais_pso_iter) * nRuns * rows, ctx->stream));
        if (particles) HIPCHK(hipMemsetAsync(ctx->d_tParts, 0, sizeof(double) * 11 * nRuns * rows * NP, ctx->stream));
        TraceOut t;
        t.sink = pais_launch::TraceSink{ctx->d_tRuns, ctx->d_tIters, particles ? ctx->d_tParts.p : nullptr, max_runs, rows};
        rc = refine_device_once(ctx, m, ctx->d_tCands, ctx->d_tRecs, Kmax, hasSeeds, false, &t);
        if (rc) {
            (void)hipStreamSynchronize(ctx->stream);
            return rc < 0 ? rc : fail_msg("pais_pso_trace: unexpected ring pass");
        }
        HIPCHK(hipMemcpyAsync(out + c0, ctx->d_tRecs, sizeof(pais_patch_result) * (size_t)m, hipMemcpyDeviceToHost, ctx->stream));
        HIPCHK(hipMemcpyAsync(runs + (size_t)max_runs * c0, ctx->d_tRuns, sizeof(pais_pso_run_info) * nRuns, hipMemcpyDeviceToHost, ctx->stream));
        HIPCHK(hipMemcpyAsync(iters + runRows * c0, ctx->d_tIters, sizeof(pais_pso_iter) * nRuns * rows, hipMemcpyDeviceToHost, ctx->stream));
        if (particles)
            HIPCHK(hipMemcpyAsync(particles + runRows * NP * 11 * c0, ctx->d_tParts, sizeof(double) * 11 * nRuns * rows * NP, hipMemcpyDeviceToHost,
                                  ctx->stream));
        HIPCHK(hipStreamSynchronize(ctx->stream));
        for (TimedLaunch &p : t.passes) p.collect(ctx->trace, 0, 0);
        ctx->trace.launches += t.launches;
        for (int i = 0; i < m; ++i) ctx->trace.items += out[c0 + i].pso_evals;
    }
    return 0;
}

extern "C" int pais_get_trace_stats(pais_ctx *ctx, double *kernel_ms, int64_t *launches, int64_t *evals, int reset)
{
    return read_launch_stats(ctx ? &ctx->trace : nullptr, "pais_get_trace_stats", kernel_ms, launches, evals, reset);
}

static_assert(offsetof(pais_patch_result, imgPoint) == 136 && offsetof(pais_patch_result, key) == 1160 &&
              offsetof(pais_patch_result, type) == 1168 && offsetof(pais_patch_result, cam_idx) == 1200 &&
              offsetof(pais_patch_result, stage) == 1456 && sizeof(pais_patch_result) == 1488, "pais_patch_result layout");
static inline int wire_kw(int max_num_cam)
{
    int k = max_num_cam < 1 ? 1 : (max_num_cam > PAIS_MAX_VIS ? PAIS_MAX_VIS : max_num_cam);
    return (k + 1) & ~1;
}
extern "C" size_t pais_record_wire_bytes(int max_num_cam) { return 208 + 20 * (size_t)wire_kw(max_num_cam); }
extern "C" int pais_pack_records(int n, const pais_patch_result *recs, int max_num_cam, void *wire)
{
    if (n < 0 || (n && (!recs || !wire))) return fail_msg("pais_pack_records: bad argument");
    const int Kw = wire_kw(max_num_cam);
    const size_t WB = pais_record_wire_bytes(max_num_cam);
    for (int i = 0; i < n; ++i) {
        const unsigned char *r = (const unsigned char *)&recs[i];
        unsigned char *w = (unsigned char *)wire + WB * (size_t)i;
        memcpy(w, r, 136);
        memcpy(w + 136, r + 1160, 8);
        memcpy(w + 144, r + 1168, 32);
        memcpy(w + 176, r + 1456, 32);
        memcpy(w + 208, r + 136, 16 * (size_t)Kw);
        memcpy(w + 208 + 16 * (size_t)Kw, r + 1200, 4 * (size_t)Kw);
    }
    return 0;
}
extern "C" int pais_unpack_records(int n, const void *wire, int max_num_cam, pais_patch_result *recs)
{
    if (n < 0 || (n && (!recs || !wire))) return fail_msg("pais_unpack_records: bad argument");
    const int Kw = wire_kw(max_num_cam);
    const size_t WB = pais_record_wire_bytes(max_num_cam);
    for (int i = 0; i < n; ++i) {
        unsigned char *r = (unsigned char *)&recs[i];
        const unsigned char *w = (const unsigned char *)wire + WB * (size_t)i;
        memset(r, 0, sizeof(pais_patch_result));
        memcpy(r, w, 136);
        memcpy(r + 1160, w + 136, 8);
        memcpy(r + 1168, w + 144, 32);
        memcpy(r + 1456, w + 176, 32);
        memcpy(r + 136, w + 208, 16 * (size_t)Kw);
        memcpy(r + 1200, w + 208 + 16 * (size_t)Kw, 4 * (size_t)Kw);
    }
    return 0;
}
extern "C" int pais_pack_records_device(pais_ctx *ctx, int n, const pais_patch_result *d_recs, int max_num_cam, void *d_wire)
{
    if (!ctx || n < 0 || (n && (!d_recs || !d_wire))) return fail_msg("pais_pack_records_device: bad argument");
    HIPCHK(hipSetDevice(ctx->device));
    HIPCHK(pais_launch::pack_records(d_recs, n, wire_kw(max_num_cam), d_wire, ctx->stream));
    return 0;
}

static int collect_stats(pais_ctx *ctx, unsigned long long *st)
{
    HIPCHK(hipStreamSynchronize(ctx->stream));
    if (drain_events(ctx, ctx->evPso, ctx->psoMs)) return -2;
    if (drain_events(ctx, ctx->evBegin, ctx->beginMs)) return -2;
    if (drain_events(ctx, ctx->evAfter, ctx->afterMs)) return -2;
    if (drain_events(ctx, ctx->evEval, ctx->evalMs)) return -2;
    const hipEvent_t ref = ctx->parent ? ctx->parent->refEv : ctx->refEv;
    for (std::vector<EventPair> *v : {&ctx->evEval2, &ctx->evRing}) {
        for (auto &p : *v) {
            float a = 0, b = 0;
            if (ref && hipEventElapsedTime(&a, ref, p.a) == hipSuccess && hipEventElapsedTime(&b, ref, p.b) == hipSuccess)
                ctx->eval2Intervals.push_back(std::make_pair(a, b));
        }
        double ms = 0;
        if (drain_events(ctx, *v, ms)) return -2;
        if (v == &ctx->evRing) ctx->ringMs += ms;
        ctx->eval2Ms += ms;
        ctx->evalMs += ms;
    }
    HIPCHK(hipMemcpy(st, ctx->d_stat, sizeof(unsigned long long) * 24, hipMemcpyDeviceToHost));
    if (ctx->tileDebug)
        fprintf(stderr, "[pais tile] particles through the tiles %llu, DBL_MAX %llu, pending (checked walk) %llu; tiles staged %llu (%.1f KB each), cameras left in global memory %llu\n",
                st[8], st[9], st[10], st[11], st[11] ? (double)st[13] / (double)st[11] / 1024.0 : 0.0, st[12]);
    if (ctx->tileVerify) {
        double a, b;
        memcpy(&a, &st[20], 8); memcpy(&b, &st[21], 8);
        if (st[18])
// ... 73 lines not shown
```

### pais_mvs_amd/csrc/pais_internal.h

```cpp
#pragma once
#include <hip/hip_runtime.h>
#include <stdint.h>

#include "../../include/pais_hip.h"

#define PAIS_STAGE_DONE  0
#define PAIS_STAGE_PSO   1
#define PAIS_STAGE_AFTER 2
#define PAIS_STAGE_AFTER2 3
#define PAIS_STAGE_AFTER2_KEEP 4
#define PAIS_STAGE_AFTER2_SAME 7

struct DevCamera {
    double KR[9], KT[3], R[9], T[3], C[3], optN[3], focal[2], pp[2];
    int maxLOD;
    int pad;
    int w[PAIS_MAX_LEVELS], h[PAIS_MAX_LEVELS];
    uint64_t imgOff[PAIS_MAX_LEVELS];
    uint64_t edgeOff[PAIS_MAX_LEVELS];
    double edgeMin[PAIS_MAX_LEVELS], edgeMax[PAIS_MAX_LEVELS];
};

typedef float2 PaisImgT;

struct DevScene {
    pais_config cfg;
    const DevCamera *cams;
    const uint8_t *imgBlob;
    const PaisImgT *imgF;
    const double *edgeBlob;
    const double *gauss;
    double lodScale[PAIS_MAX_LEVELS];
    uint64_t seed;
    int numCams;
    int pad;
};

#ifndef PAIS_RINGS
#define PAIS_RINGS 8
#endif
#ifndef PAIS_ARRIVE_STRIDE
#define PAIS_ARRIVE_STRIDE 16
#endif
#define PAIS_RING_CTL_BYTES 128
#define PAIS_RING_CTL_DONE_WORD 17
#define PAIS_RING_CTL_ERROR_WORD 19

struct pais_test_swarm;
namespace pais_launch {
struct BatchView {
    pais_patch_result *recs;
    unsigned char *states;
    unsigned char *evalBlocks;
    unsigned char *win;
    double *pre;
    int n, Nmax, Kmax, maxIt;
    hipStream_t stream;
    BatchView slice(const DevScene &sc, int lo, int hi, hipStream_t st) const;
};
struct TraceSink {
    pais_pso_run_info *runs;
    pais_pso_iter *iters;
    double *particles;
    int maxRuns, rows;
};
struct TileOpts {
    int stripSteps = 16;
    int noTiles = 0;
};

size_t eval_block_bytes_host(int Kmax);
size_t win_bytes_per_candidate(const DevScene &sc);
size_t pso_state_bytes_host(int Nmax);
size_t pre_bytes_per_candidate(int Nmax, int Kmax);
hipError_t state_blocks(const DevScene &sc, const pais_patch_state *states, int nStates, int Kmax, unsigned char *evalBlocks, void *win,
                        hipStream_t stream);
hipError_t fitness(const DevScene &sc, const pais_patch_state *states, int nStates, const int32_t *idx, const double *particles,
                   double *out, int nEvals, int Kmax, unsigned char *evalBlocks, void *win, int literal, hipStream_t stream);
hipError_t fitness_detail(const DevScene &sc, const int32_t *idx, const double *particles, int nEvals, int Kmax, const unsigned char *evalBlocks,
                          pais_cost_detail *rec, double *weight, double *avgSad, int8_t *code, double *colour, double *H, hipStream_t stream);
hipError_t load_state(const DevScene &sc, const pais_loaded_patch *in, pais_patch_result *recs, int n, uint64_t key0, hipStream_t stream);
hipError_t neighbor_count(const double *centers, int n, double radius, int32_t *counts, hipStream_t stream);
hipError_t expand_image(const uint8_t *img, PaisImgT *out, size_t n, hipStream_t stream);
hipError_t level_edge_minmax(const uint8_t *img, int w, int h, unsigned long long *minmax, hipStream_t stream);
hipError_t pack_records(const pais_patch_result *recs, int n, int Kw, void *wire, hipStream_t stream);
hipError_t wire_header(void *header, const unsigned *ringCtl, int ringN, int rank, int count, int hostRc, uint32_t userWord, hipStream_t stream);

hipError_t begin(const DevScene &sc, const BatchView &v, const pais_candidate *cands, int *activeList, int *activeCount);
hipError_t pso_init(const DevScene &sc, const BatchView &v, int *activeList, int *activeCount);
hipError_t pso_setup0(const DevScene &sc, const BatchView &v);
hipError_t pso_eval(const DevScene &sc, const BatchView &v, int pendingOnly, unsigned long long *verify);
hipError_t pso_eval_literal(const DevScene &sc, const BatchView &v);
bool tile_eligible(int Kmax);
hipError_t pso_tile(const DevScene &sc, const BatchView &v, const TileOpts &o, unsigned long long *dbg);
hipError_t pso_iter(const DevScene &sc, const BatchView &v, const int *activeList, const int *activeCount, int listLo, int listHi,
                    unsigned long long *stat, int L, int finishOnly, int nparts);
hipError_t pso_step(const DevScene &sc, const BatchView &v, unsigned long long *stat);
hipError_t pso_step_trace(const DevScene &sc, const BatchView &v, unsigned long long *stat, const TraceSink &t);
size_t ring_words(int n, int Nmax, int maxIt);
bool pre_ring_ok(int Kmax);
hipError_t pso_ring(const DevScene &sc, const BatchView &v, unsigned *ring, unsigned *ctl, int *arrive, unsigned long long *stat, int waves,
                    int phase, unsigned long long timeoutTicks);
void ring_profile_print();
hipError_t after(const DevScene &sc, pais_patch_result *recs, int n, double *hpScratch, int grid, int *counters,
                 unsigned long long *stat, int Kmax, double *ratios, int *nextCounters, hipStream_t stream);
size_t ncc_lds_bytes(int Kmax);
bool hp_in_lds(const DevScene &sc, int Kmax);
hipError_t ncc_batch(const DevScene &sc, const pais_view_state *states, int n, pais_view_result *out, double *tables, int stride,
                     double *hpScratch, int grid, int Kmax, int hpInLds, hipStream_t stream);
int test_swarm_step(pais_test_swarm *s, double *swarm);
}
```

### pais_mvs_amd/csrc/pais_kernels.hip

```cpp
#include <hip/hip_runtime.h>
#include <stdint.h>
#include <stdlib.h>
#include <string.h>

#include "../../include/pais_hip.h"
#include "../../include/pais_test_hooks.h"
#include "pais_dev.hpp"
#include "pais_internal.h"

using namespace pais;

#ifndef PAIS_NS1_WAVES
#define PAIS_NS1_WAVES 2
#endif
#ifndef PAIS_NS2_WAVES
#define PAIS_NS2_WAVES 3
#endif
#define PAIS_EVAL_BOUNDS(NS) __launch_bounds__(64, (NS) == 1 ? PAIS_NS1_WAVES : PAIS_NS2_WAVES)
#ifndef PAIS_ITER_FREE_REGS_FROM
#define PAIS_ITER_FREE_REGS_FROM 2
#endif
#define PAIS_ITER_BOUNDS(P, NS) __launch_bounds__(64, (P) >= PAIS_ITER_FREE_REGS_FROM ? 1 : ((NS) == 1 ? PAIS_NS1_WAVES : PAIS_NS2_WAVES))
#ifndef PAIS_TWO_PIXELS_MAXK
#define PAIS_TWO_PIXELS_MAXK 6
// ... 769 lines not shown
        if (PRE) {
            status0 = rec[0];
            hv = lane < PAIS_H_STRIDE * Kmax ? rec[PAIS_PRE_HDR + lane] : 0.0;
        }
        const double pend = pendingOnly ? A.part[iLoad][0] : 1.0;
        if (!active || i >= Nrun || (pend != 1.0 && pendingOnly != 2)) continue;
        wave_sync();
        stage_eval_block(smem, src, nwMax, lane, v0, v1);
        wave_sync();
        double f4[4], w4[4];
        int st;
        if (PRE) st = eval_fitness_pre<NS, BYTES, ACCR, false>(sc, ep, cams, Hbuf, cbuf, win + (size_t)c * WS, rec, status0, hv, lane, f4, w4);
        else st = eval_fitness_parts<NS, BYTES, ACCR>(sc, ep, cams, Hbuf, cbuf, win + (size_t)c * WS, p0, p1, p2, lane, 0, 1, f4, w4);
        if (lane == 0) {
            const double v = st ? DBL_MAX : combine_parts(f4, w4);
            if (pendingOnly == 2 && pend != 1.0 && verify && A.fit[i] != v && (A.fit[i] == A.fit[i] || v == v)) {
                if (atomicAdd(&verify[0], 1ULL) == 0) {
                    verify[1] = ((unsigned long long)(unsigned)c << 32) | (unsigned)i;
                    verify[2] = (unsigned long long)__double_as_longlong(A.fit[i]);
                    verify[3] = (unsigned long long)__double_as_longlong(v);
                }
            }
            A.fit[i] = v;
        }
    }
}

#include "pais_tile2.hpp"
#include "pais_literal.hpp"


__device__ __forceinline__ int wave_argmin_lex(bool valid, double key, int tie)
{
    double k = key;
    int t = tie;
    int v = valid ? 1 : 0;
#pragma unroll
    for (int m = 32; m >= 1; m >>= 1) {
        const double ok = __shfl_xor(k, m, 64);
        const int ot = __shfl_xor(t, m, 64);
        const int ov = __shfl_xor(v, m, 64);
        const bool take = ov && (!v || ok < k || (ok == k && ot < t));
        k = take ? ok : k;
        t = take ? ot : t;
        v = take ? 1 : v;
    }
    return v ? t : -1;
}

template <int CTRL> __device__ __forceinline__ int dpp_mov_i(int v) { return __builtin_amdgcn_update_dpp(v, v, CTRL, 0xF, 0xF, false); }
template <int CTRL> __device__ __forceinline__ int dpp_get_i(int v) { return __builtin_amdgcn_update_dpp(0, v, CTRL, 0xF, 0xF, true); }
template <int CTRL> __device__ __forceinline__ void argmin_dpp_step(double &k, int &t, int &v)
{
    const int olo = dpp_get_i<CTRL>(__double2loint(k)), ohi = dpp_get_i<CTRL>(__double2hiint(k));
    const int ot = dpp_get_i<CTRL>(t), ov = dpp_get_i<CTRL>(v);
    const double ok = __hiloint2double(ohi, olo);
    const bool take = ov && (!v || ok < k || (ok == k && ot < t));
    k = take ? ok : k;
    t = take ? ot : t;
    v = take ? 1 : v;
}
__device__ __forceinline__ int wave_argmin_lex_n(bool valid, double key, int tie, int N)
{
    if (N > 32) return wave_argmin_lex(valid, key, tie);
    double k = key;
    int t = tie;
    int v = valid ? 1 : 0;
    if (N > 16) {
        const double ok = __shfl_xor(k, 16, 64);
        const int ot = __shfl_xor(t, 16, 64), ov = __shfl_xor(v, 16, 64);
        const bool take = ov && (!v || ok < k || (ok == k && ot < t));
        k = take ? ok : k;
        t = take ? ot : t;
        v = take ? 1 : v;
    }
    argmin_dpp_step<0x140>(k, t, v);
    argmin_dpp_step<0x141>(k, t, v);
    argmin_dpp_step<0x1B>(k, t, v);
    argmin_dpp_step<0xB1>(k, t, v);
    return __builtin_amdgcn_readfirstlane(v ? t : -1);
}

template <int CTRL> __device__ __forceinline__ double dpp_mov_d(double v)
{
    return __hiloint2double(dpp_mov_i<CTRL>(__double2hiint(v)), dpp_mov_i<CTRL>(__double2loint(v)));
}
template <int CTRL> __device__ __forceinline__ double dpp_get_d(double v)
{
    return __hiloint2double(dpp_get_i<CTRL>(__double2hiint(v)), dpp_get_i<CTRL>(__double2loint(v)));
}
__device__ __forceinline__ double swarm_sum_fast(double v, int N)
{
    if (N > 16) v += __shfl_xor(v, 16, 64);
    v += dpp_get_d<0x140>(v);
    v += dpp_get_d<0x141>(v);
    v += dpp_get_d<0x1B>(v);
    v += dpp_get_d<0xB1>(v);
    return lane_get(v, 0);
}
__device__ __forceinline__ bool swarm_mean_below(double t0, double t1, double t2, int lane, int N)
{
    const double own = lane < N ? (t0 + t1) + t2 : 0.0;
    const double fast = swarm_sum_fast(own, N) / (double)(3 * N);
    if (fabs(fast - 0.01) > 1e-9) return fast < 0.01;
    double s = 0;
    for (int j = 0; j < N; ++j) {
        s += lane_get(t0, j);
        s += lane_get(t1, j);
        s += lane_get(t2, j);
    }
    s /= (double)(3 * N);
    return s < 0.01;
}
__device__ __forceinline__ void swarm_update_gbest(double pbf, int lane, int N, double &gf, int &g)
{
    const int w = wave_argmin_lex_n(lane < N && pbf == pbf, pbf, 63 - lane, N);
    const int j = 63 - (w < 0 ? 63 : w);
    const double m = lane_get(pbf, j);
    if (w >= 0 && m <= gf) {
        gf = m;
        g = j;
    }
}
__device__ __forceinline__ bool swarm_mean_below_any(double t0, double t1, double t2, int lane, int N)
{
    if (N <= 32) return swarm_mean_below(t0, t1, t2, lane, N);
    double s = 0;
    for (int j = 0; j < N; ++j) {
        s += lane_get(t0, j);
        s += lane_get(t1, j);
        s += lane_get(t2, j);
    }
    s /= (double)(3 * N);
    return s < 0.01;
}
__device__ __forceinline__ void swarm_update_gbest_any(double pbf, int lane, int N, double &gf, int &g)
{
    if (N <= 32) {
        swarm_update_gbest(pbf, lane, N, gf, g);
        return;
    }
    for (int j = 0; j < N; ++j) {
        const double v = lane_get(pbf, j);
        if (v <= gf) {
            gf = v;
            g = j;
        }
    }
}
template <int n> __device__ __forceinline__ int rank_ror(double dj, int lane)
{
    const double o = dpp_get_d<0x120 + n>(dj);
    const int j = dpp_get_i<0x120 + n>(lane);
    return (o < dj || (o == dj && j < lane)) ? 1 : 0;
}
template <int n> __device__ __forceinline__ int rank_ror_other(double dj, double od, bool hiRow)
{
    const double o = dpp_get_d<0x120 + n>(od);
    return (o < dj || (o == dj && hiRow)) ? 1 : 0;
}
__device__ __forceinline__ int swarm_rank(double dj, int lane, int N)
{
    int rank = 0;
    rank += rank_ror<1>(dj, lane);  rank += rank_ror<2>(dj, lane);  rank += rank_ror<3>(dj, lane);  rank += rank_ror<4>(dj, lane);
    rank += rank_ror<5>(dj, lane);  rank += rank_ror<6>(dj, lane);  rank += rank_ror<7>(dj, lane);  rank += rank_ror<8>(dj, lane);
    rank += rank_ror<9>(dj, lane);  rank += rank_ror<10>(dj, lane); rank += rank_ror<11>(dj, lane); rank += rank_ror<12>(dj, lane);
    rank += rank_ror<13>(dj, lane); rank += rank_ror<14>(dj, lane); rank += rank_ror<15>(dj, lane);
    if (N > 16) {
        const double od = __shfl_xor(dj, 16, 64);
        const bool hiRow = (lane & 16) != 0;
        rank += (od < dj || (od == dj && hiRow)) ? 1 : 0;
        rank += rank_ror_other<1>(dj, od, hiRow);  rank += rank_ror_other<2>(dj, od, hiRow);  rank += rank_ror_other<3>(dj, od, hiRow);
        rank += rank_ror_other<4>(dj, od, hiRow);  rank += rank_ror_other<5>(dj, od, hiRow);  rank += rank_ror_other<6>(dj, od, hiRow);
        rank += rank_ror_other<7>(dj, od, hiRow);  rank += rank_ror_other<8>(dj, od, hiRow);  rank += rank_ror_other<9>(dj, od, hiRow);
        rank += rank_ror_other<10>(dj, od, hiRow); rank += rank_ror_other<11>(dj, od, hiRow); rank += rank_ror_other<12>(dj, od, hiRow);
        rank += rank_ror_other<13>(dj, od, hiRow); rank += rank_ror_other<14>(dj, od, hiRow); rank += rank_ror_other<15>(dj, od, hiRow);
    }
    return rank;
}

template <int CTRL> __device__ __forceinline__ void argmin4_dpp_step(double (&k)[4], int (&t)[4], int (&v)[4])
{
    int olo[4], ohi[4], ot[4], ov[4];
#pragma unroll
    for (int c = 0; c < 4; ++c) {
        olo[c] = dpp_get_i<CTRL>(__double2loint(k[c]));
        ohi[c] = dpp_get_i<CTRL>(__double2hiint(k[c]));
        ot[c] = dpp_get_i<CTRL>(t[c]);
        ov[c] = dpp_get_i<CTRL>(v[c]);
    }
#pragma unroll
    for (int c = 0; c < 4; ++c) {
        const double ok = __hiloint2double(ohi[c], olo[c]);
        const bool take = ov[c] && (!v[c] || ok < k[c] || (ok == k[c] && ot[c] < t[c]));
        k[c] = take ? ok : k[c];
        t[c] = take ? ot[c] : t[c];
        v[c] = take ? 1 : v[c];
    }
}
__device__ __forceinline__ void wave_argmin4_lex_n(const bool (&valid)[4], const double (&key)[4], const int (&tie)[4], int N, int (&out)[4])
{
    double k[4];
    int t[4], v[4];
#pragma unroll
    for (int c = 0; c < 4; ++c) { k[c] = key[c]; t[c] = tie[c]; v[c] = valid[c] ? 1 : 0; }
    if (N > 16) {
#pragma unroll
        for (int c = 0; c < 4; ++c) {
            const double ok = __shfl_xor(k[c], 16, 64);
            const int ot = __shfl_xor(t[c], 16, 64), ov = __shfl_xor(v[c], 16, 64);
            const bool take = ov && (!v[c] || ok < k[c] || (ok == k[c] && ot < t[c]));
            k[c] = take ? ok : k[c];
            t[c] = take ? ot : t[c];
            v[c] = take ? 1 : v[c];
        }
    }
    argmin4_dpp_step<0x140>(k, t, v);
    argmin4_dpp_step<0x141>(k, t, v);
    argmin4_dpp_step<0x1B>(k, t, v);
    argmin4_dpp_step<0xB1>(k, t, v);
#pragma unroll
    for (int c = 0; c < 4; ++c) out[c] = __builtin_amdgcn_readfirstlane(v[c] ? t[c] : -1);
}

__device__ __forceinline__ void pso_move_own(int i, int N, int localK, double iw, const double *u, const double *pos,
                                             const double *pb, double fitj, double pbf, int lane, const double *gB,
                                             const double *rl, const double *ru, const double *vecI, const double *nbI,
                                             double *outP, double *outV, double *outNb)
{
    const double pw = 1.2, gw = 1.5, lw = 1.0, nw = 1.0;
    const double pVecW = pw * u[0], gVecW = gw * u[1], lVecW = lw * u[2], nVecW = nw * u[3];
    const bool pv = lane < N;
    const double pp0 = lane_get(pb[0], i), pp1 = lane_get(pb[1], i), pp2 = lane_get(pb[2], i);
    double dj;
    {
        const double d0 = pp0 - pb[0], d1 = pp1 - pb[1], d2 = pp2 - pb[2];
        dj = 0;
        dj += d0 * d0;
        dj += d1 * d1;
        dj += d2 * d2;
        dj = (lane == i) ? DBL_MAX : (!pv ? __builtin_inf() : dj);
    }
    int rank = 0;
    if (N <= 32) {
        rank = swarm_rank(dj, lane, N);
    } else {
        for (int j = 0; j < N; ++j) {
            const double o = lane_get(dj, j);
            rank += (o < dj || (o == dj && j < lane)) ? 1 : 0;
        }
    }
    const bool sel = pv && rank < localK;
    const double fitI = lane_get(fitj, i);
    if (N <= 32) {
        double FDR[3];
        for (int d = 0; d < 3; ++d) {
            const double pd = lane_get(pos[d], i);
            FDR[d] = (fitI - pbf) / fabs(pd - pb[d]);
        }
        const bool valid[4] = {sel && pbf < DBL_MAX, pv && lane != i && FDR[0] > -DBL_MAX, pv && lane != i && FDR[1] > -DBL_MAX,
                               pv && lane != i && FDR[2] > -DBL_MAX};
        const double key[4] = {pbf, -FDR[0], -FDR[1], -FDR[2]};
        const int tie[4] = {rank * 64 + lane, lane, lane, lane};
        int win[4];
        wave_argmin4_lex_n(valid, key, tie, N, win);
        const int lIdx4 = (win[0] < 0) ? i : (win[0] & 63);
        for (int d = 0; d < 3; ++d) {
            const int wn = win[1 + d];
            const double o = lane_get(pb[d], wn < 0 ? 0 : wn);
            outNb[d] = (wn < 0) ? nbI[d] : o;
        }
        for (int d = 0; d < 3; ++d) {
            double p = lane_get(pos[d], i);
            const double pbi = lane_get(pb[d], i), pbl = lane_get(pb[d], lIdx4);
            double v = iw * vecI[d] + pVecW * (pbi - p) + gVecW * (gB[d] - p) + lVecW * (pbl - p) + nVecW * (outNb[d] - p);
            outV[d] = v;
            p += v;
            if (p > ru[d]) p = ru[d];
            if (p < rl[d]) p = rl[d];
            outP[d] = p;
        }
        return;
    }
    const int w = wave_argmin_lex_n(sel && pbf < DBL_MAX, pbf, rank * 64 + lane, N);
    const int lIdx = (w < 0) ? i : (w & 63);
    for (int d = 0; d < 3; ++d) {
        const double pd = lane_get(pos[d], i);
        const double FDR = (fitI - pbf) / fabs(pd - pb[d]);
        const bool cand = pv && lane != i && FDR > -DBL_MAX;
        const int wn = wave_argmin_lex_n(cand, -FDR, lane, N);
        const double o = lane_get(pb[d], wn < 0 ? 0 : wn);
        outNb[d] = (wn < 0) ? nbI[d] : o;
    }
    for (int d = 0; d < 3; ++d) {
        double p = lane_get(pos[d], i);
        const double pbi = lane_get(pb[d], i), pbl = lane_get(pb[d], lIdx);
        double v = iw * vecI[d] + pVecW * (pbi - p) + gVecW * (gB[d] - p) + lVecW * (pbl - p) + nVecW * (outNb[d] - p);
        outV[d] = v;
        p += v;
        if (p > ru[d]) p = ru[d];
        if (p < rl[d]) p = rl[d];
        outP[d] = p;
    }
}

template <int nparts, int NS, bool BYTES, bool ACCR>
__global__ PAIS_ITER_BOUNDS(nparts, NS) void k_pso_iter(DevScene sc, unsigned char *states, const int *activeList,
                                            const int *activeCount, int listLo, int listHi, int Nmax, int Kmax,
                                            pais_patch_result *recs, unsigned long long *stat, int L, int finishOnly,
                                            const unsigned char *evalBlocks, size_t evalBlockBytes, const WinPix *win)
{
    extern __shared__ __attribute__((aligned(16))) unsigned char smem0[];
    unsigned char *smem = smem0 + (threadIdx.x >> 6) * eval_lds_bytes(NS, Kmax, ACCR);
    EvalPatch *ep = (EvalPatch *)smem;
    EvalCam *cams = (EvalCam *)(smem + sizeof(EvalPatch));
    double *Hbuf = (double *)(smem + eval_block_bytes(Kmax));
    double *cbuf = Hbuf + Kmax * PAIS_H_STRIDE;
    const int lane = threadIdx.x & 63;
    const size_t SB = pso_state_bytes(Nmax);
    const int WS = win_stride(sc);
    const int per = finishOnly ? 1 : Nmax * nparts;
    const int nAct = *activeCount;
    const int total = ((listHi < nAct ? listHi : nAct) - listLo) * per;
    for (int t = eval_first_task(); t < total; t += eval_task_stride()) {
        const int lp = t / per, ip = t - lp * per;
        const int c = activeList[listLo + lp];
        const int i = ip / nparts, part = ip - i * nparts;
        PsoState *hd = (PsoState *)(states + SB * (size_t)c);
        const uint64_t *src = (const uint64_t *)(evalBlocks + evalBlockBytes * (size_t)c);
        const int nwMax = (int)(eval_block_bytes(Kmax) / 8);
        const uint64_t v0 = lane < nwMax ? src[lane] : 0, v1 = lane + 64 < nwMax ? src[lane + 64] : 0;
        PsoArrays Wb = pso_arrays((unsigned char *)hd, Nmax, L & 1);
        PsoArrays Rb = pso_arrays((unsigned char *)hd, Nmax, (L > 0 ? L - 1 : 0) & 1);
        const int jl = lane < Nmax ? lane : 0;
        const int active = __builtin_amdgcn_readfirstlane(hd->active), N = __builtin_amdgcn_readfirstlane(hd->N),
                  maxIt = __builtin_amdgcn_readfirstlane(hd->maxIt);
        PsoState::IterDyn dr = hd->dyn[(L > 0 ? L - 1 : 0) & 1];
        dr.started = __builtin_amdgcn_readfirstlane(dr.started);
        dr.iteration = __builtin_amdgcn_readfirstlane(dr.iteration);
        dr.gIdx = __builtin_amdgcn_readfirstlane(dr.gIdx);
        const double rl[3] = {hd->rangeL[0], hd->rangeL[1], hd->rangeL[2]};
        const double ru[3] = {hd->rangeU[0], hd->rangeU[1], hd->rangeU[2]};
        const uint64_t streamBase = hd->streamBase;
        const int runIdx = __builtin_amdgcn_readfirstlane(hd->run), localK = __builtin_amdgcn_readfirstlane(hd->localK);
        double pos[3], pb[3];
        for (int d = 0; d < 3; ++d) {
            pos[d] = Rb.pos[jl][d];
            pb[d] = Rb.pBest[jl][d];
        }
        double fitj;
        if (nparts == 1) {
            fitj = Rb.fit[jl];
        } else {
            double f4[4], w4[4];
            bool bad = false;
            for (int a = 0; a < 4; ++a) {
                f4[a] = Rb.part[jl][2 * a];
                w4[a] = Rb.part[jl][2 * a + 1];
                bad = bad || (w4[a] < 0);
            }
            fitj = bad ? DBL_MAX : combine_parts(f4, w4);
        }
        double pbf = Rb.pBestFit[jl];
        const double vecI[3] = {Rb.vec[i][0], Rb.vec[i][1], Rb.vec[i][2]};
        const double nbI[3] = {Rb.nBest[i][0], Rb.nBest[i][1], Rb.nBest[i][2]};
        const double q0 = Wb.pos[i][0], q1 = Wb.pos[i][1], q2 = Wb.pos[i][2];
        if (!active || i >= N) continue;
        double p0, p1, p2;
        if (L == 0) {
            p0 = q0;
            p1 = q1;
            p2 = q2;
        } else {
            int it, g;
            double gf, iw;
            if (!dr.started) {
                pbf = fitj;
                g = 0;
                gf = lane_get(pbf, 0);
                iw = dr.iw;
                it = 0;
            } else {
                if (fitj < pbf) {
                    pbf = fitj;
                    pb[0] = pos[0];
                    pb[1] = pos[1];
                    pb[2] = pos[2];
                }
                g = dr.gIdx;
                gf = dr.gBestFitness;
                const double niw = dr.iw - 1.0 / maxIt;
                iw = niw > 0.4 ? niw : 0.4;
                it = dr.iteration + 1;
            }
            if (N <= 32) {
                swarm_update_gbest(pbf, lane, N, gf, g);
            } else {
                for (int j = 0; j < N; ++j) {
                    const double v = lane_get(pbf, j);
                    if (v <= gf) {
                        gf = v;
                        g = j;
                    }
                }
            }
            const double gB[3] = {lane_get(pb[0], g), lane_get(pb[1], g), lane_get(pb[2], g)};
            bool finished = it >= maxIt;
            if (!finished) {
                const double a0 = fabs(pos[0] - gB[0]), a1 = fabs(pos[1] - gB[1]), a2 = fabs(pos[2] - gB[2]);
                bool dispBelow;
                if (N <= 32) {
                    dispBelow = swarm_mean_below(a0, a1, a2, lane, N);
                } else {
                    double disp = 0;
                    for (int j = 0; j < N; ++j) {
                        disp += lane_get(a0, j);
                        disp += lane_get(a1, j);
                        disp += lane_get(a2, j);
                    }
                    disp /= (double)(3 * N);
                    dispBelow = disp < 0.01;
                }
                if (dispBelow) {
                    const double v0 = fabs(Rb.vec[jl][0]), v1 = fabs(Rb.vec[jl][1]), v2 = fabs(Rb.vec[jl][2]);
                    if (N <= 32) {
                        finished = swarm_mean_below(v0, v1, v2, lane, N);
                    } else {
                        double vel = 0;
                        for (int j = 0; j < N; ++j) {
                            vel += lane_get(v0, j);
                            vel += lane_get(v1, j);
                            vel += lane_get(v2, j);
                        }
                        vel /= (double)(3 * N);
                        finished = vel < 0.01;
                    }
                }
            }
            if (finished) {
                if (i == 0 && part == 0 && lane == 0) {
                    pais_patch_result *P = &recs[c];
                    double nn[3];
                    spherical2normal(gB[0], gB[1], nn);
                    P->fitness = gf;
                    P->normalS[0] = gB[0];
                    P->normalS[1] = gB[1];
                    for (int q = 0; q < 3; ++q) P->normal[q] = nn[q];
                    P->depth = gB[2];
                    const DevCamera &rc = sc.cams[hd->refCam];
                    for (int q = 0; q < 3; ++q) P->center[q] = hd->ray[q] * gB[2] + rc.C[q];
                    P->pso_runs += 1;
                    P->pso_iterations += it;
                    const int evals = N * (1 + it);
                    P->pso_evals += evals;
                    if (gf > sc.cfg.maxFitness) {
                        P->dropped = 1;
                        P->stage = PAIS_STAGE_DONE;
                    } else {
                        P->stage = PAIS_STAGE_AFTER;
                    }
                    hd->active = 0;
                    const int K = hd->K;
                    const unsigned long long perEval = (unsigned long long)(4 * K + 1 + (sc.cfg.adaptiveDistanceEnable ? 8 : 0) +
                                                                            (sc.cfg.adaptiveGradientEnable ? 8 : 0));
                    atomicAdd(&stat[0], (unsigned long long)evals);
                    atomicAdd(&stat[1], (unsigned long long)evals * perEval);
                    atomicAdd(&stat[2], 1ULL);
                }
                continue;
            }
            double u[4];
            const uint32_t k0 = (uint32_t)(6 * N + 3 + 4 * (it * N + i));
            for (int q = 0; q < 4; ++q) u[q] = uniform_from(streamBase, (uint32_t)runIdx, k0 + q);
            double nP[3], nV[3], nNb[3];
            pso_move_own(i, N, localK, iw, u, pos, pb, fitj, pbf, lane, gB, rl, ru, vecI, nbI, nP, nV, nNb);
            const double pbI[3] = {lane_get(pb[0], i), lane_get(pb[1], i), lane_get(pb[2], i)};
            const double pbfI = lane_get(pbf, i);
            if (lane == 0 && part == 0) {
                for (int d = 0; d < 3; ++d) {
                    Wb.pos[i][d] = nP[d];
                    Wb.vec[i][d] = nV[d];
                    Wb.pBest[i][d] = pbI[d];
                    Wb.nBest[i][d] = nNb[d];
                }
                Wb.pBestFit[i] = pbfI;
                if (i == 0) {
                    PsoState::IterDyn dw;
                    dw.iw = iw;
                    dw.gBestFitness = gf;
                    dw.gIdx = g;
                    dw.iteration = it;
                    dw.started = 1;
                    dw.pad = 0;
                    hd->dyn[L & 1] = dw;
                }
            }
            p0 = nP[0];
            p1 = nP[1];
            p2 = nP[2];
        }
        if (finishOnly) continue;
        wave_sync();
        stage_eval_block(smem, src, nwMax, lane, v0, v1);
        wave_sync();
        double f4[4], w4[4];
        const int st = eval_fitness_parts<NS, BYTES, ACCR>(sc, ep, cams, Hbuf, cbuf, win + (size_t)c * WS, p0, p1, p2, lane, part, nparts, f4, w4);
        if (lane == 0) {
            if (nparts == 1) {
                Wb.fit[i] = st ? DBL_MAX : combine_parts(f4, w4);
            } else {
                for (int a = part; a < 4; a += nparts) {
                    Wb.part[i][2 * a] = st ? 0.0 : f4[a];
                    Wb.part[i][2 * a + 1] = st ? -1.0 : w4[a];
                }
            }
        }
    }
}


template <int CTRL> __device__ __forceinline__ void group_min_step(double &k, int &j)
{
    const double ok = dpp_get_d<CTRL>(k);
    const int oj = dpp_get_i<CTRL>(j);
    const bool take = oj >= 0 && (j < 0 || ok < k || (ok == k && oj < j));
    k = take ? ok : k;
    j = take ? oj : j;
}
template <int CTRL> __device__ __forceinline__ void group_max_step(double &k, int &j, double &val)
{
    const double ok = dpp_get_d<CTRL>(k), oval = dpp_get_d<CTRL>(val);
    const int oj = dpp_get_i<CTRL>(j);
    const bool take = oj >= 0 && (j < 0 || ok > k || (ok == k && oj < j));
    k = take ? ok : k;
    j = take ? oj : j;
    val = take ? oval : val;
}
__device__ __forceinline__ void pso_move_lanes(int N, int localK, double iw, int it, uint64_t sb, uint32_t run, double (*pos)[3],
                                               double (*vec)[3], const double (*pBest)[3], double (*nBest)[3], const double *fit,
                                               const double *pBestFit, const double *gBest, const double *rangeL, const double *rangeU,
                                               int lane)
{
    const double pw = 1.2, gw = 1.5, lw = 1.0, nw = 1.0;
    const int sh = N <= 16 ? 2 : (N <= 32 ? 1 : 0), G = 1 << sh;
    const int i0 = lane >> sh, s = lane & (G - 1);
    const bool live = i0 < N;
    const int i = live ? i0 : 0;
    const double pp0 = pBest[i][0], pp1 = pBest[i][1], pp2 = pBest[i][2];
    const double pI[3] = {pos[i][0], pos[i][1], pos[i][2]};
    const double vI[3] = {vec[i][0], vec[i][1], vec[i][2]};
    const double nbI[3] = {nBest[i][0], nBest[i][1], nBest[i][2]};
    const double fitness = fit[i];
    double u[4];
    const uint32_t k0 = (uint32_t)(6 * N + 3 + 4 * (it * N + i));
    for (int q = 0; q < 4; ++q) u[q] = uniform_from(sb, run, k0 + q);
    const double pVecW = pw * u[0], gVecW = gw * u[1], lVecW = lw * u[2], nVecW = nw * u[3];
    const int np = (N + G - 1) >> sh;
    double maxFDR[3] = {-DBL_MAX, -DBL_MAX, -DBL_MAX};
    double nb[3] = {nbI[0], nbI[1], nbI[2]};
    int nj[3] = {-1, -1, -1};
#pragma unroll 1
    for (int p = 0; p < np; ++p) {
        const int j = s + (p << sh);
        const int jj = j < N ? j : 0;
        const double bd[3] = {pBest[jj][0], pBest[jj][1], pBest[jj][2]}, bf = pBestFit[jj];
        const bool other = j < N && j != i;
#pragma unroll
        for (int d = 0; d < 3; ++d) {
            const double FDR = (fitness - bf) / fabs(pI[d] - bd[d]);
            if (other && FDR > maxFDR[d]) {
                maxFDR[d] = FDR;
                nb[d] = bd[d];
                nj[d] = j;
            }
        }
    }
    if (G >= 2) {
#pragma unroll
        for (int d = 0; d < 3; ++d) group_max_step<0xB1>(maxFDR[d], nj[d], nb[d]);
    }
    if (G == 4) {
#pragma unroll
        for (int d = 0; d < 3; ++d) group_max_step<0x4E>(maxFDR[d], nj[d], nb[d]);
    }
    uint64_t taken = 0;
    double minFitness = DBL_MAX;
    int lIdx = i;
#pragma unroll 1
    for (int k = 0; k < localK; ++k) {
        double bd = 0;
        int bj = -1;
#pragma unroll 1
        for (int p = 0; p < np; ++p) {
            const int j = s + (p << sh);
            const int jj = j < N ? j : 0;
            double dj;
            {
                const double d0 = pp0 - pBest[jj][0], d1 = pp1 - pBest[jj][1], d2 = pp2 - pBest[jj][2];
                dj = 0;
                dj += d0 * d0;
                dj += d1 * d1;
                dj += d2 * d2;
                if (j == i) dj = DBL_MAX;
            }
            if (j < N && !((taken >> p) & 1) && (bj < 0 || dj < bd)) {
                bd = dj;
// ... 76 lines not shown
        }
        sb = hd->streamBase;
        run = hd->run;
        localK = hd->localK;
        double rNb[3];
        for (int d = 0; d < 3; ++d) {
            rPos[d] = sload<COH>(&A.pos[jl][d]);
            rVec[d] = sload<COH>(&A.vec[jl][d]);
            rPb[d] = sload<COH>(&A.pBest[jl][d]);
            rNb[d] = sload<COH>(&A.nBest[jl][d]);
        }
        const double rFit = sload<COH>(&A.fit[jl]);
        double rPbf = sload<COH>(&A.pBestFit[jl]);
        it = __builtin_amdgcn_readfirstlane(it);
        g = __builtin_amdgcn_readfirstlane(g);
        maxIt = __builtin_amdgcn_readfirstlane(maxIt);
        started = __builtin_amdgcn_readfirstlane(started);
        run = __builtin_amdgcn_readfirstlane(run);
        localK = __builtin_amdgcn_readfirstlane(localK);
        gf = lane_get(gf, 0);
        iw = lane_get(iw, 0);
        for (int d = 0; d < 3; ++d) {
            rl[d] = lane_get(rl[d], 0);
            ru[d] = lane_get(ru[d], 0);
        }
        sb = (uint64_t)__double_as_longlong(lane_get(__longlong_as_double((long long)sb), 0));
        if (!started) {
            rPbf = rFit;
            g = 0;
            gf = lane_get(rPbf, 0);
            it = 0;
        } else {
            if (rFit < rPbf) {
                rPbf = rFit;
                rPb[0] = rPos[0];
                rPb[1] = rPos[1];
                rPb[2] = rPos[2];
            }
            const double niw = iw - 1.0 / maxIt;
            iw = niw > 0.4 ? niw : 0.4;
            it += 1;
        }
        swarm_update_gbest_any(rPbf, lane, N, gf, g);
        if (lane < N) {
            for (int d = 0; d < 3; ++d) {
                pos[lane][d] = rPos[d];
                vec[lane][d] = rVec[d];
                pBest[lane][d] = rPb[d];
                nBest[lane][d] = rNb[d];
            }
            fit[lane] = rFit;
            pBestFit[lane] = rPbf;
        }
        __syncthreads();
    } else {
        for (int i = lane; i < N; i += 64) {
            for (int d = 0; d < 3; ++d) {
                pos[i][d] = sload<COH>(&A.pos[i][d]);
                vec[i][d] = sload<COH>(&A.vec[i][d]);
                pBest[i][d] = sload<COH>(&A.pBest[i][d]);
                nBest[i][d] = sload<COH>(&A.nBest[i][d]);
            }
            fit[i] = sload<COH>(&A.fit[i]);
            pBestFit[i] = sload<COH>(&A.pBestFit[i]);
        }
        __syncthreads();
        it = sload<COH>(&hd->iteration);
        g = sload<COH>(&hd->gIdx);
        gf = sload<COH>(&hd->gBestFitness);
        iw = sload<COH>(&hd->iw);
        const int started = sload<COH>(&hd->started);
        if (!started) {
            for (int i = lane; i < N; i += 64) pBestFit[i] = fit[i];
            __syncthreads();
            g = 0;
            gf = pBestFit[0];
            for (int j = 0; j < N; ++j)
                if (pBestFit[j] <= gf) { gf = pBestFit[j]; g = j; }
            it = 0;
        } else {
            for (int i = lane; i < N; i += 64) {
                if (fit[i] < pBestFit[i]) {
                    pBestFit[i] = fit[i];
                    pBest[i][0] = pos[i][0];
                    pBest[i][1] = pos[i][1];
                    pBest[i][2] = pos[i][2];
                }
            }
            __syncthreads();
            for (int j = 0; j < N; ++j)
                if (pBestFit[j] <= gf) { gf = pBestFit[j]; g = j; }
            const double niw = iw - 1.0 / maxIt;
            iw = niw > 0.4 ? niw : 0.4;
            it += 1;
        }
    }
    bool finished = it >= maxIt;
    double tDisp = __builtin_nan(""), tVel = __builtin_nan("");
    if (!finished && lanes && !Sink::on) {
        const double g0 = lane_get(rPb[0], g), g1 = lane_get(rPb[1], g), g2 = lane_get(rPb[2], g);
        if (swarm_mean_below_any(fabs(rPos[0] - g0), fabs(rPos[1] - g1), fabs(rPos[2] - g2), lane, N))
            finished = swarm_mean_below_any(fabs(rVec[0]), fabs(rVec[1]), fabs(rVec[2]), lane, N);
    } else if (!finished) {
        const double g0 = pBest[g][0], g1 = pBest[g][1], g2 = pBest[g][2];
        double disp = 0;
        for (int i = 0; i < N; ++i) {
            disp += fabs(pos[i][0] - g0);
            disp += fabs(pos[i][1] - g1);
            disp += fabs(pos[i][2] - g2);
        }
        disp /= (double)(3 * N);
        if constexpr (Sink::on) tDisp = disp;
        if (disp < 0.01) {
            double vel = 0;
            for (int i = 0; i < N; ++i) {
                vel += fabs(vec[i][0]);
                vel += fabs(vec[i][1]);
                vel += fabs(vec[i][2]);
            }
            vel /= (double)(3 * N);
            if constexpr (Sink::on) tVel = vel;
            finished = vel < 0.01;
        }
    }
    if constexpr (Sink::on) {
        const int run = hd->run;
        if (run >= 0 && run < sink.maxRuns && it >= 0 && it < sink.rows) {
            const size_t slot = (size_t)c * sink.maxRuns + run;
            if (lane == 0) {
                pais_pso_iter *row = sink.iters + slot * sink.rows + it;
                row->gbest_fitness = gf;
                row->gbest[0] = pBest[g][0];
                row->gbest[1] = pBest[g][1];
                row->gbest[2] = pBest[g][2];
                row->iw = iw;
                row->dispersion = tDisp;
                row->velocity = tVel;
                row->g_idx = g;
                row->iteration = it;
                row->ended = finished ? 1 : 0;
            }
            pais_pso_run_info *ri = sink.runs + slot;
            if (it == 0) {
                if (lane == 0) {
                    for (int d = 0; d < 3; ++d) {
                        ri->range_l[d] = hd->rangeL[d];
                        ri->range_u[d] = hd->rangeU[d];
                        ri->init[d] = hd->init[d];
                        ri->ray[d] = hd->ray[d];
                    }
                    ri->run = run;
                    ri->ref_cam = hd->refCam;
                    ri->lod = hd->LOD;
                    ri->num_cam = hd->K;
                    ri->n_particles = N;
                    ri->max_iteration = maxIt;
                }
                for (int k = lane; k < hd->K && k < PAIS_MAX_VIS; k += 64) ri->cam_idx[k] = hd->camIdx[k];
            }
            if (finished && lane == 0) ri->iterations = it;
            if (sink.particles) {
                double *dst = sink.particles + (slot * sink.rows + it) * (size_t)sink.NP * 11;
                for (int i = lane; i < N && i < sink.NP; i += 64) {
                    double *q = dst + (size_t)i * 11;
                    for (int d = 0; d < 3; ++d) {
                        q[d] = pos[i][d];
                        q[3 + d] = vec[i][d];
                        q[6 + d] = pBest[i][d];
                    }
                    q[9] = fit[i];
                    q[10] = pBestFit[i];
                }
            }
        }
    }
    if (!finished) {
        const double gB[3] = {pBest[g][0], pBest[g][1], pBest[g][2]};
        if (lanes) {
            pso_move_lanes(N, localK, iw, it, sb, (uint32_t)run, pos, vec, pBest, nBest, fit, pBestFit, gB, rl, ru, lane);
        } else {
            const double rangeL[3] = {hd->rangeL[0], hd->rangeL[1], hd->rangeL[2]};
            const double rangeU[3] = {hd->rangeU[0], hd->rangeU[1], hd->rangeU[2]};
            const uint64_t streamBase = hd->streamBase;
            const uint32_t runIdx = (uint32_t)hd->run;
            const int nearK = hd->localK;
            for (int i = lane; i < N; i += 64) {
                double u[4];
                const uint32_t k0 = (uint32_t)(6 * N + 3 + 4 * (it * N + i));
                for (int q = 0; q < 4; ++q) u[q] = uniform_from(streamBase, runIdx, k0 + q);
                pso_move_particle(i, N, nearK, iw, u, pos, vec, pBest, nBest, fit, pBestFit, gB, rangeL, rangeU);
            }
        }
        __syncthreads();
        for (int i = lane; i < N; i += 64) {
            for (int d = 0; d < 3; ++d) {
                sstore<COH>(&A.pos[i][d], pos[i][d]);
                sstore<COH>(&A.vec[i][d], vec[i][d]);
                sstore<COH>(&A.pBest[i][d], pBest[i][d]);
                sstore<COH>(&A.nBest[i][d], nBest[i][d]);
            }
            sstore<COH>(&A.pBestFit[i], pBestFit[i]);
        }
        if (pre) swarm_eval_setup<COH>(sc, preEp, preCams, pos, N, pBestFit + Nmax, pre, preD, lane);
        if (lane == 0) {
            sstore<COH>(&hd->iteration, it);
            sstore<COH>(&hd->gIdx, g);
            sstore<COH>(&hd->gBestFitness, gf);
            sstore<COH>(&hd->iw, iw);
            sstore<COH>(&hd->started, 1);
        }
        return 1;
    } else if (lane == 0) {
        pais_patch_result *P = &recs[c];
        const double th = pBest[g][0], ph = pBest[g][1], dp = pBest[g][2];
        double nn[3];
        spherical2normal(th, ph, nn);
        P->fitness = gf;
        P->normalS[0] = th;
        P->normalS[1] = ph;
        for (int q = 0; q < 3; ++q) P->normal[q] = nn[q];
        P->depth = dp;
        const DevCamera &rc = sc.cams[hd->refCam];
        for (int q = 0; q < 3; ++q) P->center[q] = hd->ray[q] * dp + rc.C[q];
        P->pso_runs += 1;
        P->pso_iterations += it;
        const int evals = N * (1 + it);
        P->pso_evals += evals;
        if (gf > sc.cfg.maxFitness) {
            P->dropped = 1;
            P->stage = PAIS_STAGE_DONE;
        } else {
            P->stage = PAIS_STAGE_AFTER;
        }
        hd->active = 0;
        const int K = hd->K;
        const unsigned long long perEval = (unsigned long long)(4 * K + 1 + (sc.cfg.adaptiveDistanceEnable ? 8 : 0) +
                                                                (sc.cfg.adaptiveGradientEnable ? 8 : 0));
        atomicAdd(&stat[0], (unsigned long long)evals);
        atomicAdd(&stat[1], (unsigned long long)evals * perEval);
        atomicAdd(&stat[2], 1ULL);
        atomicAdd(&stat[5], (unsigned long long)evals);
        atomicAdd(&stat[6], (unsigned long long)evals * perEval);
        if (COH) {
            atomicAdd(&stat[22], (unsigned long long)evals);
            atomicAdd(&stat[23], (unsigned long long)evals * perEval);
        }
    }
    return 0;
}
template <bool COH = false, class Sink = StepNoSink>
__device__ int pso_step_wave(const DevScene &sc, pais_patch_result *recs, int c, PsoState *hd, int N, int Nmax,
                             unsigned char *smem, unsigned long long *stat, int lane, const EvalPatch *preEp = nullptr,
                             const EvalCam *preCams = nullptr, double *pre = nullptr, size_t preD = 0, const Sink &sink = Sink())
{
    if (N <= 64) return pso_step_body<COH, Sink, true>(sc, recs, c, hd, N, Nmax, smem, stat, lane, preEp, preCams, pre, preD, sink);
    return pso_step_body<COH, Sink, false>(sc, recs, c, hd, N, Nmax, smem, stat, lane, preEp, preCams, pre, preD, sink);
}
__device__ int pso_step_wave_ring(const DevScene &sc, pais_patch_result *recs, int c, PsoState *hd, int N, int Nmax, unsigned char *smem,
                                  unsigned long long *stat, int lane, const EvalPatch *preEp, const EvalCam *preCams, double *pre, size_t preD)
{
    return pso_step_body<true, StepNoSink, true>(sc, recs, c, hd, N, Nmax, smem, stat, lane, preEp, preCams, pre, preD, StepNoSink());
}
__global__ __launch_bounds__(64, 4) void k_pso_step(DevScene sc, pais_patch_result *recs, unsigned char *states, int n,
                                                 int Nmax, unsigned long long *stat, const unsigned char *evalBlocks, size_t evalBlockBytes,
                                                 double *pre, int Kmax)
{
    extern __shared__ __attribute__((aligned(16))) unsigned char smem0[];
    unsigned char *smem = smem0 + (pre ? evalBlockBytes : 0);
    const size_t preD = pre_rec_doubles(Kmax);
    const int nwMax = (int)(evalBlockBytes / 8);
    __builtin_amdgcn_s_setprio(3);
    const int lane = threadIdx.x;
    const size_t SB = pso_state_bytes(Nmax);
    for (int c = blockIdx.x; c < n; c += gridDim.x) {
        PsoState *hd = (PsoState *)(states + SB * (size_t)c);
        const int active = hd->active, N = __builtin_amdgcn_readfirstlane(hd->N);
        if (!active) continue;
        if (pre) {
            const uint64_t *src = (const uint64_t *)(evalBlocks + evalBlockBytes * (size_t)c);
            wave_sync();
            stage_eval_block(smem0, src, nwMax, lane, lane < nwMax ? src[lane] : 0, lane + 64 < nwMax ? src[lane + 64] : 0);
            wave_sync();
        }
        pso_step_wave(sc, recs, c, hd, N, Nmax, smem, stat, lane, (const EvalPatch *)smem0, (const EvalCam *)(smem0 + sizeof(EvalPatch)),
                      pre ? pre + preD * (size_t)Nmax * (size_t)c : nullptr, preD);
    }
}

__global__ __launch_bounds__(64, 4) void k_pso_step_trace(DevScene sc, pais_patch_result *recs, unsigned char *states, int n, int Nmax,
                                                       unsigned long long *stat, StepTraceSink sink)
{
    extern __shared__ __attribute__((aligned(16))) unsigned char smem0[];
    __builtin_amdgcn_s_setprio(3);
    const int lane = threadIdx.x;
    const size_t SB = pso_state_bytes(Nmax);
    for (int c = blockIdx.x; c < n; c += gridDim.x) {
        PsoState *hd = (PsoState *)(states + SB * (size_t)c);
        const int active = hd->active, N = __builtin_amdgcn_readfirstlane(hd->N);
        if (!active) continue;
        pso_step_wave<false, StepTraceSink>(sc, recs, c, hd, N, Nmax, smem0, stat, lane, nullptr, nullptr, nullptr, 0, sink);
    }
}

__global__ __launch_bounds__(64) void k_pso_setup0(DevScene sc, unsigned char *states, int n, int Nmax, const unsigned char *evalBlocks,
                                                   size_t evalBlockBytes, double *pre, int Kmax)
{
    extern __shared__ __attribute__((aligned(16))) unsigned char smem0[];
    double(*pos)[3] = (double(*)[3])(smem0 + evalBlockBytes);
    double *scr = (double *)(pos + Nmax);
    const int lane = threadIdx.x;
    const size_t SB = pso_state_bytes(Nmax);
    const size_t preD = pre_rec_doubles(Kmax);
    const int nwMax = (int)(evalBlockBytes / 8);
    for (int c = blockIdx.x; c < n; c += gridDim.x) {
        PsoState *hd = (PsoState *)(states + SB * (size_t)c);
        if (!hd->active) continue;
        PsoArrays A = pso_arrays((unsigned char *)hd, Nmax);
        const int N = hd->N;
        const uint64_t *src = (const uint64_t *)(evalBlocks + evalBlockBytes * (size_t)c);
        wave_sync();
        stage_eval_block(smem0, src, nwMax, lane, lane < nwMax ? src[lane] : 0, lane + 64 < nwMax ? src[lane + 64] : 0);
        for (int i = lane; i < N; i += 64)
            for (int d = 0; d < 3; ++d) pos[i][d] = A.pos[i][d];
        wave_sync();
        swarm_eval_setup<false>(sc, (const EvalPatch *)smem0, (const EvalCam *)(smem0 + sizeof(EvalPatch)), pos, N, scr,
                                pre + preD * (size_t)Nmax * (size_t)c, preD, lane);
    }
}

#define PAIS_RING_EMPTY 0xFFFFFFFFu
struct RingCtl { unsigned head, pad0[15]; unsigned tail, done, total, error, pad1[12]; };
static_assert(sizeof(RingCtl) == PAIS_RING_CTL_BYTES, "RingCtl layout (pais_internal.h)");

__global__ __launch_bounds__(256) void k_ring_init(unsigned char *states, int n, int Nmax, unsigned *ring, unsigned segWords, RingCtl *ctl)
{
    const int c = blockIdx.x * 256 + threadIdx.x;
    if (c >= n) return;
    RingCtl *rc = &ctl[c % PAIS_RINGS];
    atomicAdd(&rc->total, 1u);
    const PsoState *hd = (const PsoState *)(states + pso_state_bytes(Nmax) * (size_t)c);
    if (!hd->active) {
        atomicAdd(&rc->done, 1u);
        return;
    }
    const int N = hd->N;
    const unsigned base = atomicAdd(&rc->tail, (unsigned)N);
    unsigned *seg = ring + (size_t)(c % PAIS_RINGS) * segWords;
    for (int j = 0; j < N; ++j) seg[base + j] = ((unsigned)c << 8) | (unsigned)j;
}

#ifndef PAIS_RING_PROFILE
#define PAIS_RING_PROFILE 0
#endif
#if PAIS_RING_PROFILE
__device__ unsigned long long g_ringProf[8];
#define PAIS_RP_MARK(v) const unsigned long long v = __builtin_amdgcn_s_memtime();
#else
#define PAIS_RP_MARK(v)
#endif
template <int NS, bool BYTES, bool ACCR, bool PRE>
__global__ PAIS_EVAL_BOUNDS(NS) void k_pso_ring(DevScene sc, pais_patch_result *recs, unsigned char *states, int n, int Nmax, int Kmax,
                                                const unsigned char *evalBlocks, size_t evalBlockBytes, const WinPix *win, unsigned *ringAll,
                                                unsigned segWords, RingCtl *ctlAll, int *arrive, unsigned long long *stat, size_t ldsPerWave,
                                                unsigned long long timeoutTicks, double *pre)
{
    const size_t preD = pre_rec_doubles(Kmax);
    extern __shared__ __attribute__((aligned(16))) unsigned char smem0[];
    unsigned char *smem = smem0 + (threadIdx.x >> 6) * ldsPerWave;
    EvalPatch *ep = (EvalPatch *)smem;
    EvalCam *cams = (EvalCam *)(smem + sizeof(EvalPatch));
    double *Hbuf = (double *)(smem + eval_block_bytes(Kmax));
    double *cbuf = Hbuf + Kmax * PAIS_H_STRIDE;
    const int lane = threadIdx.x & 63;
    const size_t SB = pso_state_bytes(Nmax);
    const int WS = win_stride(sc);
    const int nwMax = (int)(eval_block_bytes(Kmax) / 8);
    const int myRing = (int)(blockIdx.x % PAIS_RINGS);
    RingCtl *ctl = &ctlAll[myRing];
    unsigned *ring = ringAll + (size_t)myRing * segWords;
    const unsigned cap = segWords;
    const unsigned total = ctl->total;
    for (;;) {
        PAIS_RP_MARK(rpA)
        unsigned idx = 0;
        if (lane == 0) idx = __hip_atomic_fetch_add(&ctl->head, 1u, __ATOMIC_RELAXED, __HIP_MEMORY_SCOPE_AGENT);
        idx = (unsigned)__builtin_amdgcn_readfirstlane((int)idx);
        if (idx >= cap) break;
        PAIS_RP_MARK(rpB)
        unsigned e = PAIS_RING_EMPTY;
        unsigned long long t0 = 0;
        for (int spins = 0;; ++spins) {
            e = rload(&ring[idx]);
            if (e != PAIS_RING_EMPTY) break;
            if ((spins & 7) == 7) {
                if (rload(&ctl->done) >= total) break;
                if (rload(&ctl->error) != 0) break;
                const unsigned long long now = __builtin_amdgcn_s_memrealtime();
                if (spins == 7) t0 = now;
                if (now - t0 >= timeoutTicks) {
                    if (lane == 0) rstore(&ctl->error, 1u);
                    break;
                }
            }
            __builtin_amdgcn_s_sleep(32);
        }
        e = (unsigned)__builtin_amdgcn_readfirstlane((int)e);
        if (e == PAIS_RING_EMPTY) break;
        PAIS_RP_MARK(rpC)
        const int c = (int)(e >> 8), i = (int)(e & 255u);
        PsoState *hd = (PsoState *)(states + SB * (size_t)c);
        PsoArrays A = pso_arrays((unsigned char *)hd, Nmax);
        const uint64_t *src = (const uint64_t *)(evalBlocks + evalBlockBytes * (size_t)c);
        double *crec = PRE ? pre + preD * (size_t)Nmax * (size_t)c : nullptr;
        const double *rec = PRE ? crec + preD * (size_t)i : nullptr;
        double p0 = 0, p1 = 0, p2 = 0, status0 = 0, hv = 0;
        if (PRE) {
            status0 = cload(&rec[0]);
            hv = lane < PAIS_H_STRIDE * Kmax ? cload(&rec[PAIS_PRE_HDR + lane]) : 0.0;
        } else {
            p0 = cload(&A.pos[i][0]); p1 = cload(&A.pos[i][1]); p2 = cload(&A.pos[i][2]);
        }
        const uint64_t v0 = lane < nwMax ? src[lane] : 0, v1 = lane + 64 < nwMax ? src[lane + 64] : 0;
        const int N = hd->N;
        wave_sync();
        stage_eval_block(smem, src, nwMax, lane, v0, v1);
        wave_sync();
#if PAIS_RING_PROFILE
        asm volatile("s_waitcnt vmcnt(0)" ::: "memory");
#endif
        PAIS_RP_MARK(rpD)
        double f4[4], w4[4];
        int st;
        if (PRE) st = eval_fitness_pre<NS, BYTES, ACCR, true>(sc, ep, cams, Hbuf, cbuf, win + (size_t)c * WS, rec, status0, hv, lane, f4, w4);
        else st = eval_fitness_parts<NS, BYTES, ACCR>(sc, ep, cams, Hbuf, cbuf, win + (size_t)c * WS, p0, p1, p2, lane, 0, 1, f4, w4);
        int old = 0;
        PAIS_RP_MARK(rpE)
        if (lane == 0) {
            cstore(&A.fit[i], st ? DBL_MAX : combine_parts(f4, w4));
            asm volatile("s_waitcnt vmcnt(0)" ::: "memory");
            old = __hip_atomic_fetch_add(&arrive[(size_t)c * PAIS_ARRIVE_STRIDE], 1, __ATOMIC_RELAXED, __HIP_MEMORY_SCOPE_AGENT);
        }
        old = __builtin_amdgcn_readfirstlane(old);
#if PAIS_RING_PROFILE
        {
            const unsigned long long rpF = __builtin_amdgcn_s_memtime();
            if (lane == 0) {
                atomicAdd(&g_ringProf[0], rpB - rpA); atomicAdd(&g_ringProf[1], rpC - rpB); atomicAdd(&g_ringProf[2], rpD - rpC);
                atomicAdd(&g_ringProf[3], rpE - rpD); atomicAdd(&g_ringProf[4], rpF - rpE); atomicAdd(&g_ringProf[6], 1ULL);
            }
        }
        PAIS_RP_MARK(rpG)
#endif
        if (old != N - 1) continue;
        __builtin_amdgcn_s_setprio(3);
        if (lane == 0) cstore(&arrive[(size_t)c * PAIS_ARRIVE_STRIDE], 0);
        wave_sync();
        const int cont = pso_step_wave_ring(sc, recs, c, hd, __builtin_amdgcn_readfirstlane(N), Nmax, smem + (PRE ? eval_block_bytes(Kmax) : 0), stat, lane, ep, cams, crec, preD);
        asm volatile("s_waitcnt vmcnt(0)" ::: "memory");
        wave_sync();
        if (__builtin_amdgcn_readfirstlane(cont)) {
            unsigned base = 0;
            if (lane == 0) base = __hip_atomic_fetch_add(&ctl->tail, (unsigned)N, __ATOMIC_RELAXED, __HIP_MEMORY_SCOPE_AGENT);
            base = (unsigned)__builtin_amdgcn_readfirstlane((int)base);
            if (base + (unsigned)N > cap) {
                if (lane == 0) rstore(&ctl->error, 2u);
                break;
            }
            if (lane < N) rstore(&ring[base + lane], ((unsigned)c << 8) | (unsigned)lane);
        } else if (lane == 0) {
            __hip_atomic_fetch_add(&ctl->done, 1u, __ATOMIC_RELAXED, __HIP_MEMORY_SCOPE_AGENT);
        }
        __builtin_amdgcn_s_setprio(0);
#if PAIS_RING_PROFILE
        {
            const unsigned long long rpH = __builtin_amdgcn_s_memtime();
            if (lane == 0) { atomicAdd(&g_ringProf[5], rpH - rpG); atomicAdd(&g_ringProf[7], 1ULL); }
        }
#endif
    }
}

__global__ __launch_bounds__(64) void k_region_ratio(DevScene sc, const pais_patch_result *recs, int n, int stage, double *ratios, int Kmax)
{
    const int t = blockIdx.x * 64 + threadIdx.x;
    const int c = t / Kmax, k = t - c * Kmax;
    if (c >= n) return;
    const pais_patch_result *P = &recs[c];
    if (P->stage != stage || P->dropped || k >= P->num_cam) return;
    const int LOD = P->lod, refCam = P->ref_cam;
    const DevCamera &rc = sc.cams[refCam];
    const double s = sc.lodScale[LOD];
    const double center[3] = {P->center[0], P->center[1], P->center[2]};
    const double nrm[3] = {P->normal[0], P->normal[1], P->normal[2]};
    const int ci = P->cam_idx[k];
    const double d = -dot3(center, nrm);
    double invH[9], H[9];
    ref_plane_inverse(d, s, rc.KR, rc.KT, nrm, invH);
    patch_homography(ci == refCam, d, s, sc.cams[ci].KR, sc.cams[ci].KT, nrm, invH, H);
    double pt[2];
    cam_project(sc, refCam, center, pt, LOD);
    ratios[(size_t)c * PAIS_MAX_VIS + k] = region_ratio(pt[0], pt[1], sc.cfg.patchRadius, H);
}

template <int PHASE>
__global__ __launch_bounds__(64 * AFTER_WAVES) void k_after(DevScene sc, pais_patch_result *recs, int n, double *hpScratch,
                                                              int *counters, unsigned long long *stat, int Kmax, double *ratios,
                                                              int hpInLds, int *nextCounters)
{
    if (PHASE == 2 && nextCounters && blockIdx.x == 0 && threadIdx.x == 0) {
        nextCounters[0] = 0;
        nextCounters[1] = 0;
        nextCounters[2] = 0;
    }
    extern __shared__ __attribute__((aligned(16))) unsigned char smem[];
    pais_patch_result *st = (pais_patch_result *)smem;
    size_t off = (sizeof(pais_patch_result) + 15) & ~(size_t)15;
    double *table = (double *)(smem + off); off += sizeof(double) * Kmax * Kmax;
    double *Hn = (double *)(smem + off); off += sizeof(double) * 9 * Kmax;
    int *flag = (int *)(smem + off); off += 16;
    const int lane = threadIdx.x & 63, wave = threadIdx.x >> 6;
    const bool lead = threadIdx.x == 0;
    const int S2 = sc.cfg.patchSize * sc.cfg.patchSize;
    double *hp = hpInLds ? (double *)(smem + off) : hpScratch + (size_t)blockIdx.x * Kmax * S2;
    for (int c = blockIdx.x; c < n; c += gridDim.x) {
        const int stg = recs[c].stage;
        if (PHASE == 1 ? (stg != PAIS_STAGE_AFTER) : (stg != PAIS_STAGE_AFTER2 && stg != PAIS_STAGE_AFTER2_KEEP && stg != PAIS_STAGE_AFTER2_SAME))
            continue;
        __syncthreads();
        copy_record(st, &recs[c], threadIdx.x, 64 * AFTER_WAVES);
        __syncthreads();

        const int nccBefore = st->ncc_tables;
        double *rat = ratios + (size_t)c * PAIS_MAX_VIS;
        if (PHASE == 1) {
            const int refBefore = st->ref_cam, lodBefore = st->lod, numBefore = st->num_cam;
            remove_invisible_camera(sc, st, hp, table, Hn, flag, rat, lane, wave);
            const bool removedNone = st->num_cam == numBefore;
            set_reference_camera(sc, st, lane);
            set_depth_and_ray(sc, st, lane);
            set_depth_range(sc, st, lane);
            set_lod(sc, st, lane);

            bool again = false;
            if (st->type != PAIS_TYPE_EXPAND && !st->dropped) {
                const int afterRef = st->ref_cam, afterNum = st->num_cam;
                const int cnt = st->count;
                const bool cond = (st->before_ref != afterRef || st->before_num != afterNum) && (cnt <= st->total_cam_num);
                __syncthreads();
                if (lead) {
                    st->after_ref = afterRef;
                    st->after_num = afterNum;
                    st->count = cnt + 1;
                }
                __syncthreads();
                if (cond) {
                    if (st->num_cam < sc.cfg.minCamNum) {
                        __syncthreads();
                        if (lead) {
                            st->fitness = DBL_MAX;
                            st->priority = DBL_MAX;
                            st->dropped = 1;
                        }
                        __syncthreads();
                    } else {
                        again = true;
                        __syncthreads();
                        if (lead) {
                            st->before_ref = st->ref_cam;
                            st->before_num = st->num_cam;
                            st->stage = PAIS_STAGE_PSO;
                        }
                        __syncthreads();
                    }
                }
            }
            if (!again) {
                set_priority_and_image_point(sc, st, lane);
                __syncthreads();
                if (lead)
                    st->stage = st->dropped ? PAIS_STAGE_DONE
                                            : ((st->ref_cam == refBefore && st->lod == lodBefore)
                                                   ? (removedNone ? PAIS_STAGE_AFTER2_SAME : PAIS_STAGE_AFTER2_KEEP)
                                                   : PAIS_STAGE_AFTER2);
            }
            __syncthreads();
            if (lead && again) atomicAdd(&counters[1], 1);
        } else {
            if (stg == PAIS_STAGE_AFTER2_SAME) {
                if (lead) st->ncc_tables += 1;
            } else {
                remove_invisible_camera(sc, st, hp, table, Hn, flag, rat, lane, wave);
            }
            __syncthreads();
            int finalStage = PAIS_DONE;
            if (!st->dropped) {
                bool off = false;
                const double X[3] = {st->center[0], st->center[1], st->center[2]};
                for (int i = threadIdx.x; i < sc.numCams; i += 64 * AFTER_WAVES) {
                    const DevCamera &cam = sc.cams[i];
                    double pt[2];
                    project_raw(cam.R, cam.T, cam.focal, cam.pp, 1.0, X, pt);
                    if (!in_image_d(pt, cam.w[0], cam.h[0])) {
                        off = true;
                    } else {
                        const int rx = min(cv_round(pt[0]), cam.w[0] - 1), ry = min(cv_round(pt[1]), cam.h[0] - 1);
                        if (sc.imgBlob[cam.imgOff[0] + (size_t)ry * cam.w[0] + rx] == 0) off = true;
                    }
                }
                finalStage = __syncthreads_or(off ? 1 : 0) ? PAIS_DONE_OFF_SCENE : PAIS_DONE_IN_SCENE;
            }
            if (lead) st->stage = finalStage;
        }
        __syncthreads();
        if (lead) {
            atomicAdd(&stat[3], (unsigned long long)(st->ncc_tables - nccBefore));
            atomicAdd(&stat[4], (unsigned long long)(st->ncc_tables - nccBefore) * (unsigned long long)st->total_cam_num);
        }
        __syncthreads();
        copy_record(&recs[c], st, threadIdx.x, 64 * AFTER_WAVES);
    }
}

__global__ __launch_bounds__(64 * AFTER_WAVES) void k_ncc_batch(DevScene sc, const pais_view_state *states, int n,
                                                                  pais_view_result *out, double *tables, int stride,
                                                                  double *hpScratch, int Kmax, int hpInLds)
{
    extern __shared__ __attribute__((aligned(16))) unsigned char smem[];
    pais_view_result *res = (pais_view_result *)smem;
    size_t off = (sizeof(pais_view_result) + 15) & ~(size_t)15;
    double *table = (double *)(smem + off); off += sizeof(double) * Kmax * Kmax;
    double *Hn = (double *)(smem + off); off += sizeof(double) * 9 * Kmax;
    int *flag = (int *)(smem + off); off += 16;
    const int tid = threadIdx.x, lane = tid & 63, wave = tid >> 6;
    const int r = sc.cfg.patchRadius, S = sc.cfg.patchSize, S2 = S * S;
    double *hp = hpInLds ? (double *)(smem + off) : hpScratch + (size_t)blockIdx.x * Kmax * S2;
    for (int s = blockIdx.x; s < n; s += gridDim.x) {
        const pais_view_state *V = &states[s];
        const int K = V->num_cam, LOD = V->lod, refCam = V->ref_cam;
        const double center[3] = {V->center[0], V->center[1], V->center[2]};
        const double nrm[3] = {V->normal[0], V->normal[1], V->normal[2]};
        __syncthreads();
        {
            uint32_t *w = (uint32_t *)res;
            for (int i = tid; i < (int)(sizeof(pais_view_result) / 4); i += 64 * AFTER_WAVES) w[i] = 0;
        }
        for (int i = tid; i < K * K; i += 64 * AFTER_WAVES) table[i] = 0;
        if (tid == 0) *flag = 0;
        if (wave == 0) view_homographies(sc, refCam, sc.lodScale[LOD], V->cam_idx, K, center, nrm, Hn, lane);
        __syncthreads();

        double pt[2];
        cam_project(sc, refCam, center, pt, LOD);
        if (wave == AFTER_WAVES - 1)
            for (int c = lane; c < K; c += 64) res->region_ratio[c] = region_ratio(pt[0], pt[1], r, Hn + 9 * c);

        view_warp_patches(sc, V->cam_idx, K, LOD, Hn, pt[0] - r, pt[1] - r, hp, flag, lane, wave);
        __syncthreads();
        const bool dropSample = *flag != 0;
        if (!dropSample) view_fill_table(hp, K, S2, table, lane, wave);
        __syncthreads();
        if (tid == 0) {
            if (dropSample) {
                res->dropped = PAIS_VIEW_DROP_SAMPLE;
            } else {
                double correlation = 0;
                for (int i = 0; i < K; ++i)
                    for (int j = 0; j < K; ++j) correlation += table[i * K + j];
                correlation /= (double)(K * K - K);
                double maxCorr = -DBL_MAX;
                int maxIdx = 0;
                for (int i = 0; i < K; ++i) {
                    double corrSum = 0;
                    for (int j = 0; j < K; ++j) corrSum += table[i * K + j];
                    if (corrSum >= maxCorr) {
                        maxIdx = i;
                        maxCorr = corrSum;
                    }
                }
                int nn = 0;
                for (int i = 0; i < K; ++i) {
                    const int ci = V->cam_idx[i];
                    const DevCamera &cam = sc.cams[ci];
                    const double dd = nrm[0] * (-cam.optN[0]) + nrm[1] * (-cam.optN[1]) + nrm[2] * (-cam.optN[2]);
                    int why = PAIS_VIEW_KEEP;
                    if (res->region_ratio[i] < sc.cfg.minRegionRatio) why = PAIS_VIEW_REGION;
                    else if (dd < 0) why = PAIS_VIEW_BACKFACING;
                    else if (i != maxIdx && table[maxIdx * K + i] < sc.cfg.minCorrelation) why = PAIS_VIEW_CORRELATION;
                    res->reason[i] = why;
                    if (why == PAIS_VIEW_KEEP) res->kept_idx[nn++] = ci;
                }
                res->correlation = correlation;
                res->max_idx = maxIdx;
                res->num_kept = nn;
                res->dropped = nn < sc.cfg.minCamNum ? PAIS_VIEW_DROP_MINCAM : 0;
            }
        }
        if (tables) {
            double *T = tables + (size_t)s * stride * stride;
            for (int i = tid; i < stride * stride; i += 64 * AFTER_WAVES) {
                const int a = i / stride, b = i - a * stride;
                T[i] = (a < K && b < K) ? table[a * K + b] : 0.0;
            }
        }
        __syncthreads();
        {
            const uint32_t *src = (const uint32_t *)res;
            uint32_t *dst = (uint32_t *)&out[s];
            for (int i = tid; i < (int)(sizeof(pais_view_result) / 4); i += 64 * AFTER_WAVES) dst[i] = src[i];
        }
    }
}

__global__ __launch_bounds__(256) void k_pack_records(const pais_patch_result *recs, int n, int Kw, uint32_t *wire)
{
    const int wordsPerSlot = 52 + 5 * Kw;
    for (size_t t = (size_t)blockIdx.x * 256 + threadIdx.x; t < (size_t)n * wordsPerSlot; t += (size_t)gridDim.x * 256) {
        const int r = (int)(t / wordsPerSlot), w = (int)(t - (size_t)r * wordsPerSlot);
        const uint32_t *src = (const uint32_t *)&recs[r];
        int sw;
        if (w < 34) sw = w;
        else if (w < 36) sw = 290 + (w - 34);
        else if (w < 44) sw = 292 + (w - 36);
        else if (w < 52) sw = 364 + (w - 44);
        else if (w < 52 + 4 * Kw) sw = 34 + (w - 52);
        else sw = 300 + (w - 52 - 4 * Kw);
        wire[t] = src[sw];
    }
}

__global__ __launch_bounds__(64) void k_wire_header(uint32_t *hdr, const RingCtl *ctl, int ringN, int rank, int count, int hostRc, uint32_t userWord)
{
    if (threadIdx.x >= 16) return;
    int rc = hostRc;
    if (rc == 0 && ctl) {
        unsigned done = 0, err = 0;
        for (int r = 0; r < PAIS_RINGS; ++r) { done += ctl[r].done; err |= ctl[r].error; }
        if (err != 0 || done != (unsigned)ringN) rc = PAIS_WIRE_RC_RING_RETRY;
    }
    const uint32_t w[4] = {PAIS_WIRE_MAGIC, (uint32_t)rc, (uint32_t)count, (uint32_t)rank};
    hdr[threadIdx.x] = threadIdx.x < 4 ? w[threadIdx.x] : (threadIdx.x == 4 ? userWord : 0u);
}

__global__ __launch_bounds__(256) void k_expand_image(const uint8_t *img, PaisImgT *out, size_t n)
{
    for (size_t i = (size_t)blockIdx.x * 256 + threadIdx.x; i < n; i += (size_t)gridDim.x * 256) {
        const int a = img[i], b = (i + 1 < n) ? img[i + 1] : 0;
        PaisImgT v;
        v.x = a;
        v.y = b - a;
        out[i] = v;
    }
}
__global__ __launch_bounds__(256) void k_level_edge_minmax(const uint8_t *img, int w, int h, unsigned long long *minmax)
{
    __shared__ unsigned long long red[8];
    const int x = blockIdx.x * 256 + threadIdx.x;
    unsigned long long lo = ~0ULL, hi = 0ULL;
    if (x < w) {
        const int xl = x > 0 ? x - 1 : (w > 1 ? 1 : 0), xr = x < w - 1 ? x + 1 : (w > 1 ? w - 2 : 0);
        for (int r = 0; r < 16; ++r) {
            const int y = blockIdx.y * 16 + r;
            if (y >= h) break;
            const int yu = y > 0 ? y - 1 : (h > 1 ? 1 : 0), yd = y < h - 1 ? y + 1 : (h > 1 ? h - 2 : 0);
            const double gx = (double)img[(size_t)y * w + xr] - (double)img[(size_t)y * w + xl];
            const double gy = (double)img[(size_t)yd * w + x] - (double)img[(size_t)yu * w + x];
            const unsigned long long u = (unsigned long long)__double_as_longlong(sqrt(gx * gx + gy * gy));
            lo = u < lo ? u : lo;
            hi = u > hi ? u : hi;
        }
    }
    for (int s = 32; s >= 1; s >>= 1) {
        const unsigned long long ol = __shfl_xor(lo, s, 64), oh = __shfl_xor(hi, s, 64);
        lo = ol < lo ? ol : lo;
        hi = oh > hi ? oh : hi;
    }
    const int wave = threadIdx.x >> 6;
    if ((threadIdx.x & 63) == 0) {
        red[wave] = lo;
        red[4 + wave] = hi;
    }
    __syncthreads();
    if (threadIdx.x == 0) {
        for (int q = 1; q < 4; ++q) {
            lo = red[q] < lo ? red[q] : lo;
            hi = red[4 + q] > hi ? red[4 + q] : hi;
        }
        if (lo != ~0ULL) atomicMin(&minmax[0], lo);
        atomicMax(&minmax[1], hi);
    }
}

__global__ __launch_bounds__(256) void k_neighbor_count(const double *centers, int n, double radius, int32_t *counts)
{
    __shared__ double tile[256 * 3];
    const int i = blockIdx.x * 256 + threadIdx.x;
    const bool has = i < n;
    const double cx = has ? centers[3 * i] : 0, cy = has ? centers[3 * i + 1] : 0, cz = has ? centers[3 * i + 2] : 0;
    int cnt = 0;
    for (int base = 0; base < n; base += 256) {
        const int m = (n - base) < 256 ? (n - base) : 256;
        __syncthreads();
        for (int t = threadIdx.x; t < 3 * m; t += 256) tile[t] = centers[3 * (size_t)base + t];
        __syncthreads();
        for (int j = 0; j < m; ++j) {
            const double dx = cx - tile[3 * j], dy = cy - tile[3 * j + 1], dz = cz - tile[3 * j + 2];
            double s2 = 0;
            s2 += dx * dx;
            s2 += dy * dy;
            s2 += dz * dz;
            const double dist = sqrt(s2);
            cnt += ((base + j) != i && !(dist > radius)) ? 1 : 0;
        }
    }
    if (has) counts[i] = cnt;
}

namespace pais_launch {

template <auto Kern, class... A> static hipError_t launch(dim3 grid, dim3 block, size_t lds, hipStream_t stream, const A &...args)
{
    if (lds > 64 * 1024) {
        static size_t setFor[64] = {0};
        int dev = 0;
        hipError_t e = hipGetDevice(&dev);
        if (e != hipSuccess) return e;
        const bool known = dev >= 0 && dev < 64;
        if (!known || lds > setFor[dev]) {
            e = hipFuncSetAttribute((const void *)Kern, hipFuncAttributeMaxDynamicSharedMemorySize, (int)lds);
            if (e != hipSuccess) return e;
            if (known) setFor[dev] = lds;
        }
    }
    hipLaunchKernelGGL(Kern, grid, block, lds, stream, args...);
    return hipGetLastError();
}
static inline unsigned grid_for(long n, long cap) { return (unsigned)(n < 1 ? 1 : (n < cap ? n : cap)); }
static const long EVAL_GRID_CAP = 262144;

static size_t ncc_scratch_bytes(size_t recBytes, int Kmax)
{
    return ((recBytes + 15) & ~(size_t)15) + sizeof(double) * Kmax * Kmax + sizeof(double) * 9 * Kmax + 16;
}
size_t ncc_lds_bytes(int Kmax) { return ncc_scratch_bytes(sizeof(pais_view_result), Kmax); }
static size_t hp_bytes(const DevScene &sc, int Kmax) { return sizeof(double) * (size_t)Kmax * sc.cfg.patchSize * sc.cfg.patchSize; }
bool hp_in_lds(const DevScene &sc, int Kmax) { return hp_bytes(sc, Kmax) <= 60 * 1024; }

#ifndef PAIS_TWO_PIXELS_REG_MAXK
#define PAIS_TWO_PIXELS_REG_MAXK 12
#endif
static inline int eval_shape(int Kmax) { return Kmax <= PAIS_TWO_PIXELS_MAXK ? 0 : (Kmax <= PAIS_TWO_PIXELS_REG_MAXK ? 1 : 2); }
static inline bool byte_taps(const DevScene &sc) { return sc.imgF == nullptr; }
template <class T, T V> struct Const { constexpr operator T() const { return V; } };
template <int V> using Int = Const<int, V>;
template <bool V> using Bool = Const<bool, V>;
template <class F> static hipError_t shape_dispatch(const DevScene &sc, int Kmax, F f)
{
    const int shape = eval_shape(Kmax);
    if (byte_taps(sc))
        return shape == 0 ? f(Int<2>(), Bool<true>(), Bool<false>())
                          : (shape == 1 ? f(Int<2>(), Bool<true>(), Bool<true>()) : f(Int<1>(), Bool<true>(), Bool<true>()));
    return shape == 0 ? f(Int<2>(), Bool<false>(), Bool<false>())
                      : (shape == 1 ? f(Int<2>(), Bool<false>(), Bool<true>()) : f(Int<1>(), Bool<false>(), Bool<true>()));
}

size_t eval_block_bytes_host(int Kmax) { return eval_block_bytes(Kmax); }
size_t win_bytes_per_candidate(const DevScene &sc) { return sizeof(WinPix) * (size_t)win_stride(sc); }
size_t pso_state_bytes_host(int Nmax) { return pso_state_bytes(Nmax); }
size_t pre_bytes_per_candidate(int Nmax, int Kmax) { return pre_rec_bytes(Kmax) * (size_t)Nmax; }

BatchView BatchView::slice(const DevScene &sc, int lo, int hi, hipStream_t st) const
{
    BatchView s = *this;
    s.recs = recs + lo;
    s.states = states + pso_state_bytes(Nmax) * (size_t)lo;
    s.evalBlocks = evalBlocks + eval_block_bytes(Kmax) * (size_t)lo;
    s.win = win + win_bytes_per_candidate(sc) * (size_t)lo;
    if (pre) s.pre = (double *)((unsigned char *)pre + pre_bytes_per_candidate(Nmax, Kmax) * (size_t)lo);
    s.n = hi - lo;
    s.stream = st;
    return s;
}

hipError_t state_blocks(const DevScene &sc, const pais_patch_state *states, int nStates, int Kmax, unsigned char *evalBlocks, void *win,
                        hipStream_t stream)
{
    if (nStates <= 0) return hipSuccess;
    return launch<k_state_blocks>(grid_for(nStates, 65536), dim3(64), 0, stream, sc, states, nStates, evalBlocks, eval_block_bytes(Kmax),
                                  (WinPix *)win);
}
hipError_t fitness(const DevScene &sc, const pais_patch_state *states, int nStates, const int32_t *idx, const double *particles,
                   double *out, int nEvals, int Kmax, unsigned char *evalBlocks, void *win, int literal, hipStream_t stream)
{
    if (nEvals <= 0) return hipSuccess;
    const hipError_t e = state_blocks(sc, states, nStates, Kmax, evalBlocks, win, stream);
    if (e != hipSuccess) return e;
    const unsigned char *blocks = evalBlocks;
    if (literal)
        return launch<k_fitness_lit>(grid_for(nEvals, 1 << 20), dim3(64), literal_lds_bytes(Kmax, sc.cfg.patchSize), stream, sc, idx, particles,
                                     out, nEvals, Kmax, blocks, eval_block_bytes(Kmax));
    return shape_dispatch(sc, Kmax, [&](auto ns, auto bytes, auto accr) {
        return launch<k_fitness<ns, bytes, accr>>(grid_for(nEvals, EVAL_GRID_CAP), dim3(64), eval_lds_bytes(ns, Kmax, accr), stream, sc, idx,
                                                  particles, out, nEvals, Kmax, blocks, eval_block_bytes(Kmax), (const WinPix *)win);
    });
}
hipError_t fitness_detail(const DevScene &sc, const int32_t *idx, const double *particles, int nEvals, int Kmax, const unsigned char *evalBlocks,
                          pais_cost_detail *rec, double *weight, double *avgSad, int8_t *code, double *colour, double *H, hipStream_t stream)
{
    if (nEvals <= 0) return hipSuccess;
    return launch<k_fitness_detail>(grid_for(nEvals, 1 << 20), dim3(64), literal_lds_bytes(Kmax, sc.cfg.patchSize), stream, sc, idx, particles,
                                    nEvals, Kmax, evalBlocks, eval_block_bytes(Kmax), rec, weight, avgSad, code, colour, H);
}

hipError_t begin(const DevScene &sc, const BatchView &v, const pais_candidate *cands, int *activeList, int *activeCount)
{
    if (v.n <= 0) return hipSuccess;
    return launch<k_begin<true>>(grid_for(v.n, 16384), dim3(64), 0, v.stream, sc, cands, v.recs, v.n, v.states, v.Nmax, activeList, activeCount,
                                 v.evalBlocks, eval_block_bytes(v.Kmax), (WinPix *)v.win);
}
hipError_t pso_init(const DevScene &sc, const BatchView &v, int *activeList, int *activeCount)
{
    return launch<k_pso_init>(grid_for(v.n, 65536), dim3(64), 0, v.stream, sc, v.recs, v.n, v.states, v.Nmax, activeList, activeCount,
                              v.evalBlocks, eval_block_bytes(v.Kmax), (WinPix *)v.win);
}

hipError_t load_state(const DevScene &sc, const pais_loaded_patch *in, pais_patch_result *recs, int n, uint64_t key0, hipStream_t stream)
{
    if (n <= 0) return hipSuccess;
    return launch<k_load_state>(grid_for(n, 16384), dim3(64), 0, stream, sc, in, recs, n, key0);
}
hipError_t expand_image(const uint8_t *img, PaisImgT *out, size_t n, hipStream_t stream)
{
    if (n == 0) return hipSuccess;
    return launch<k_expand_image>(grid_for((long)((n + 255) / 256), 1 << 20), dim3(256), 0, stream, img, out, n);
}
hipError_t level_edge_minmax(const uint8_t *img, int w, int h, unsigned long long *minmax, hipStream_t stream)
{
    return launch<k_level_edge_minmax>(dim3((w + 255) / 256, (h + 15) / 16), dim3(256), 0, stream, img, w, h, minmax);
}
hipError_t neighbor_count(const double *centers, int n, double radius, int32_t *counts, hipStream_t stream)
{
    if (n <= 0) return hipSuccess;
    return launch<k_neighbor_count>(dim3((n + 255) / 256), dim3(256), 0, stream, centers, n, radius, counts);
}
hipError_t pack_records(const pais_patch_result *recs, int n, int Kw, void *wire, hipStream_t stream)
{
    if (n <= 0) return hipSuccess;
    const size_t words = (size_t)n * (52 + 5 * Kw);
    return launch<k_pack_records>(grid_for((long)((words + 255) / 256), 65536), dim3(256), 0, stream, recs, n, Kw, (uint32_t *)wire);
}
hipError_t wire_header(void *header, const unsigned *ringCtl, int ringN, int rank, int count, int hostRc, uint32_t userWord, hipStream_t stream)
{
    return launch<k_wire_header>(dim3(1), dim3(64), 0, stream, (uint32_t *)header, (const RingCtl *)ringCtl, ringN, rank, count, hostRc, userWord);
}

hipError_t pso_eval(const DevScene &sc, const BatchView &v, int pendingOnly, unsigned long long *verify)
{
    const unsigned grid = grid_for((long)v.n * v.Nmax, pendingOnly == 1 ? 256 : EVAL_GRID_CAP);
    return shape_dispatch(sc, v.Kmax, [&](auto ns, auto bytes, auto accr) {
        constexpr int NS = ns;
        constexpr bool BYTES = bytes, ACCR = accr;
        auto go = [&](auto usePre) {
            return launch<k_pso_eval2<NS, BYTES, ACCR, usePre>>(grid, dim3(64), eval_lds_bytes(NS, v.Kmax, ACCR), v.stream, sc, v.states, v.n, v.Nmax,
                                                                v.Kmax, (const unsigned char *)v.evalBlocks, eval_block_bytes(v.Kmax),
                                                                (const WinPix *)v.win, pendingOnly, verify, (const double *)v.pre);
        };
        return v.pre ? go(Bool<true>()) : go(Bool<false>());
    });
}
#ifndef PAIS_PRE_RING_NS1
#define PAIS_PRE_RING_NS1 0
#endif
bool pre_ring_ok(int Kmax) { return PAIS_PRE_RING_NS1 || eval_shape(Kmax) != 2; }
hipError_t pso_setup0(const DevScene &sc, const BatchView &v)
{
    if (v.n <= 0) return hipSuccess;
    const size_t lds = eval_block_bytes(v.Kmax) + sizeof(double) * 3 * (size_t)v.Nmax + pre_scratch_bytes(v.Nmax);
    return launch<k_pso_setup0>(grid_for(v.n, 65536), dim3(64), lds, v.stream, sc, v.states, v.n, v.Nmax, (const unsigned char *)v.evalBlocks,
                                eval_block_bytes(v.Kmax), v.pre, v.Kmax);
}
hipError_t pso_eval_literal(const DevScene &sc, const BatchView &v)
{
    return launch<k_pso_eval_lit>(grid_for((long)v.n * v.Nmax, 1 << 20), dim3(64), literal_lds_bytes(v.Kmax, sc.cfg.patchSize), v.stream, sc,
                                  v.states, v.n, v.Nmax, v.Kmax, (const unsigned char *)v.evalBlocks, eval_block_bytes(v.Kmax));
}
bool tile_eligible(int Kmax) { return eval_shape(Kmax) == 2 && Kmax <= TILE_MAX_CAMS; }
template <int NP>
static hipError_t tile_launch(const DevScene &sc, const BatchView &v, const TileOpts &o, unsigned long long *dbg)
{
    const size_t lds = (160 * 1024) & ~(size_t)1023, fixed = tile2_fixed_lds_bytes(v.Kmax);
    if (fixed + 4096 > lds) return hipErrorInvalidValue;
    const int groups = (v.Nmax + TILE2_SLOTS - 1) / TILE2_SLOTS;
    return launch<k_pso_tile2<NP>>(grid_for((long)v.n * groups, 65536), dim3(64 * TILE2_WAVES), lds, v.stream, sc, v.states, v.n, v.Nmax, v.Kmax,
                                   (const unsigned char *)v.evalBlocks, eval_block_bytes(v.Kmax), (const WinPix *)v.win,
                                   o.noTiles ? 0 : (int)(lds - fixed), groups, o.stripSteps, dbg);
}
hipError_t pso_tile(const DevScene &sc, const BatchView &v, const TileOpts &o, unsigned long long *dbg)
{
    if (v.Kmax <= 28) return tile_launch<8>(sc, v, o, dbg);
    if (v.Kmax <= 44) return tile_launch<12>(sc, v, o, dbg);
    return tile_launch<16>(sc, v, o, dbg);
}
hipError_t pso_iter(const DevScene &sc, const BatchView &v, const int *activeList, const int *activeCount, int listLo, int listHi,
                    unsigned long long *stat, int L, int finishOnly, int nparts)
{
    if (listHi <= listLo) return hipSuccess;
    return shape_dispatch(sc, v.Kmax, [&](auto ns, auto bytes, auto accr) {
        constexpr int NS = ns;
        constexpr bool BYTES = bytes, ACCR = accr;
        auto go = [&](auto parts) {
            return launch<k_pso_iter<parts, NS, BYTES, ACCR>>(grid_for((long)(listHi - listLo) * (finishOnly ? 1 : v.Nmax * parts), EVAL_GRID_CAP),
                                                              dim3(64), eval_lds_bytes(NS, v.Kmax, ACCR), v.stream, sc, v.states, activeList, activeCount,
                                                              listLo, listHi, v.Nmax, v.Kmax, v.recs, stat, L, finishOnly,
                                                              (const unsigned char *)v.evalBlocks, eval_block_bytes(v.Kmax), (const WinPix *)v.win);
        };
        return nparts == 4 ? go(Int<4>()) : (nparts == 2 ? go(Int<2>()) : go(Int<1>()));
    });
}
static size_t ring_seg_words(int n, int Nmax, int maxIt) { return (size_t)((n + PAIS_RINGS - 1) / PAIS_RINGS) * Nmax * ((size_t)maxIt + 2); }
size_t ring_words(int n, int Nmax, int maxIt) { return ring_seg_words(n, Nmax, maxIt) * PAIS_RINGS; }
hipError_t pso_ring(const DevScene &sc, const BatchView &v, unsigned *ring, unsigned *ctl, int *arrive, unsigned long long *stat, int waves,
                    int phase, unsigned long long timeoutTicks)
{
    const int n = v.n, Nmax = v.Nmax, Kmax = v.Kmax;
    if (Nmax > 64) return hipErrorInvalidValue;
    const size_t words = ring_words(n, Nmax, v.maxIt), seg = ring_seg_words(n, Nmax, v.maxIt);
    if (seg >= 0xFFFFFFF0ull) return hipErrorInvalidValue;
    if (phase == 0) {
        hipError_t e = hipMemsetAsync(ring, 0xFF, words * sizeof(unsigned), v.stream);
        if (e != hipSuccess) return e;
        e = hipMemsetAsync(ctl, 0, sizeof(RingCtl) * PAIS_RINGS, v.stream);
        if (e != hipSuccess) return e;
        e = hipMemsetAsync(arrive, 0, sizeof(int) * PAIS_ARRIVE_STRIDE * (size_t)n, v.stream);
        if (e != hipSuccess) return e;
        return launch<k_ring_init>(dim3((n + 255) / 256), dim3(256), 0, v.stream, v.states, n, Nmax, ring, (unsigned)seg, (RingCtl *)ctl);
    }
    return shape_dispatch(sc, Kmax, [&](auto ns, auto bytes, auto accr) {
        constexpr int NS = ns;
        constexpr bool BYTES = bytes, ACCR = accr;
        const size_t stepBytes = v.pre ? eval_block_bytes(Kmax) + step_lds_bytes(Nmax) : sizeof(double) * (size_t)Nmax * (3 * 4 + 2) + 16;
        size_t per = eval_lds_bytes(NS, Kmax, ACCR);
        if (per < stepBytes) per = stepBytes;
        per = (per + 15) & ~(size_t)15;
        const long resident = (long)waves * (NS == 1 ? 4 * PAIS_NS1_WAVES : 4 * PAIS_NS2_WAVES);
        const unsigned grid = (grid_for((long)n * Nmax, resident) + PAIS_RINGS - 1) / PAIS_RINGS * PAIS_RINGS;
        auto go = [&](auto usePre) {
            return launch<k_pso_ring<NS, BYTES, ACCR, usePre>>(dim3(grid), dim3(64), per, v.stream, sc, v.recs, v.states, n, Nmax, Kmax,
                                                               (const unsigned char *)v.evalBlocks, eval_block_bytes(Kmax), (const WinPix *)v.win, ring,
                                                               (unsigned)seg, (RingCtl *)ctl, arrive, stat, per, timeoutTicks, v.pre);
        };
        return v.pre ? go(Bool<true>()) : go(Bool<false>());
    });
}
hipError_t pso_step(const DevScene &sc, const BatchView &v, unsigned long long *stat)
{
    const size_t lds = v.pre ? eval_block_bytes(v.Kmax) + step_lds_bytes(v.Nmax) : sizeof(double) * (size_t)v.Nmax * (3 * 4 + 2);
    return launch<k_pso_step>(grid_for(v.n, 65536), dim3(64), lds, v.stream, sc, v.recs, v.states, v.n, v.Nmax, stat,
                              (const unsigned char *)v.evalBlocks, eval_block_bytes(v.Kmax), v.pre, v.Kmax);
}
hipError_t pso_step_trace(const DevScene &sc, const BatchView &v, unsigned long long *stat, const TraceSink &t)
{
    if (v.n <= 0) return hipSuccess;
    StepTraceSink sink;
    sink.runs = t.runs;
    sink.iters = t.iters;
    sink.particles = t.particles;
    sink.maxRuns = t.maxRuns;
    sink.rows = t.rows;
    sink.NP = v.Nmax;
    return launch<k_pso_step_trace>(grid_for(v.n, 65536), dim3(64), sizeof(double) * (size_t)v.Nmax * (3 * 4 + 2), v.stream, sc, v.recs, v.states,
                                    v.n, v.Nmax, stat, sink);
}

hipError_t after(const DevScene &sc, pais_patch_result *recs, int n, double *hpScratch, int grid, int *counters,
                 unsigned long long *stat, int Kmax, double *ratios, int *nextCounters, hipStream_t stream)
{
    if (n <= 0) return hipSuccess;
    const int hpInLds = hp_in_lds(sc, Kmax) ? 1 : 0;
    const size_t lds = ncc_scratch_bytes(sizeof(pais_patch_result), Kmax) + (hpInLds ? hp_bytes(sc, Kmax) : 0);
    const dim3 rgrid((unsigned)(((long)n * Kmax + 63) / 64)), block(64 * AFTER_WAVES);
    hipError_t e = launch<k_region_ratio>(rgrid, dim3(64), 0, stream, sc, recs, n, PAIS_STAGE_AFTER, ratios, Kmax);
    if (e == hipSuccess)
        e = launch<k_after<1>>(dim3(grid), block, lds, stream, sc, recs, n, hpScratch, counters, stat, Kmax, ratios, hpInLds, (int *)nullptr);
    if (e == hipSuccess) e = launch<k_region_ratio>(rgrid, dim3(64), 0, stream, sc, recs, n, PAIS_STAGE_AFTER2, ratios, Kmax);
    if (e == hipSuccess)
        e = launch<k_after<2>>(dim3(grid), block, lds, stream, sc, recs, n, hpScratch, counters, stat, Kmax, ratios, hpInLds, nextCounters);
    return e;
}
hipError_t ncc_batch(const DevScene &sc, const pais_view_state *states, int n, pais_view_result *out, double *tables, int stride,
                     double *hpScratch, int grid, int Kmax, int hpInLds, hipStream_t stream)
{
    if (n <= 0) return hipSuccess;
    const size_t lds = ncc_lds_bytes(Kmax) + (hpInLds ? hp_bytes(sc, Kmax) : 0);
    return launch<k_ncc_batch>(dim3(grid), dim3(64 * AFTER_WAVES), lds, stream, sc, states, n, out, tables, stride, hpScratch, Kmax, hpInLds);
}

__global__ __launch_bounds__(64) void k_test_swarm_step(DevScene sc, pais_patch_result *recs, unsigned char *states, int Nmax,
                                                        unsigned long long *stat, int *continues)
{
    extern __shared__ __attribute__((aligned(16))) unsigned char smem0[];
    PsoState *hd = (PsoState *)states;
    const int N = __builtin_amdgcn_readfirstlane(hd->N);
    const int cont = pso_step_wave(sc, recs, 0, hd, N, Nmax, smem0, stat, (int)threadIdx.x);
    if (threadIdx.x == 0) *continues = cont;
}
int test_swarm_step(pais_test_swarm *s, double *swarm)
{
    if (!s || !swarm || s->n < 1 || s->n > 128) return (int)hipErrorInvalidValue;
    const int N = s->n;
    const size_t SB = pso_state_bytes(N), head = (sizeof(PsoState) + 15) & ~(size_t)15;
    unsigned char *host = (unsigned char *)calloc(1, SB);
    if (!host) return (int)hipErrorOutOfMemory;
    PsoState *hd = (PsoState *)host;
    for (int d = 0; d < 3; ++d) {
        hd->rangeL[d] = s->range_l[d];
        hd->rangeU[d] = s->range_u[d];
        hd->ray[d] = d == 2 ? 1.0 : 0.0;
    }
    hd->iw = s->iw;
    hd->gBestFitness = s->gbest_fitness;
    hd->streamBase = s->stream_base;
    hd->gIdx = s->g_idx;
    hd->N = N;
    hd->maxIt = s->max_iteration;
    hd->iteration = s->iteration;
    hd->active = 1;
    hd->run = s->run;
    hd->localK = s->local_k;
    hd->started = s->started;
    hd->K = 3;
    double *arr = (double *)(host + head);
    for (int i = 0; i < N; ++i) {
        for (int a = 0; a < 4; ++a)
            for (int d = 0; d < 3; ++d) arr[(size_t)a * 3 * N + 3 * i + d] = swarm[14 * i + 3 * a + d];
        arr[(size_t)12 * N + i] = swarm[14 * i + 12];
        arr[(size_t)13 * N + i] = swarm[14 * i + 13];
    }
    unsigned char *dev = nullptr;
    const size_t offRec = (SB + 255) & ~(size_t)255, offStat = offRec + ((sizeof(pais_patch_result) + 255) & ~(size_t)255),
                 offCam = offStat + 256, offCont = offCam + ((sizeof(DevCamera) + 255) & ~(size_t)255), total = offCont + 256;
    hipError_t e = hipMalloc((void **)&dev, total);
    if (e == hipSuccess) e = hipMemset(dev, 0, total);
    if (e == hipSuccess) e = hipMemcpy(dev, host, SB, hipMemcpyHostToDevice);
    pais_patch_result rec;
    int cont = 0;
    if (e == hipSuccess) {
        DevScene sc;
        memset(&sc, 0, sizeof(sc));
        sc.cams = (const DevCamera *)(dev + offCam);
        sc.cfg.maxFitness = 10.0;
        sc.numCams = 1;
        e = launch<k_test_swarm_step>(dim3(1), dim3(64), sizeof(double) * (size_t)N * (3 * 4 + 2) + 16, nullptr, sc,
                                      (pais_patch_result *)(dev + offRec), dev, N, (unsigned long long *)(dev + offStat), (int *)(dev + offCont));
    }
    if (e == hipSuccess) e = hipDeviceSynchronize();
    if (e == hipSuccess) e = hipMemcpy(host, dev, SB, hipMemcpyDeviceToHost);
    if (e == hipSuccess) e = hipMemcpy(&rec, dev + offRec, sizeof(rec), hipMemcpyDeviceToHost);
    if (e == hipSuccess) e = hipMemcpy(&cont, dev + offCont, sizeof(int), hipMemcpyDeviceToHost);
    if (e == hipSuccess) {
        for (int i = 0; i < N; ++i) {
            for (int a = 0; a < 4; ++a)
                for (int d = 0; d < 3; ++d) swarm[14 * i + 3 * a + d] = arr[(size_t)a * 3 * N + 3 * i + d];
            swarm[14 * i + 12] = arr[(size_t)12 * N + i];
            swarm[14 * i + 13] = arr[(size_t)13 * N + i];
        }
        s->iw = hd->iw;
        s->gbest_fitness = hd->gBestFitness;
        s->g_idx = hd->gIdx;
        s->iteration = hd->iteration;
        s->started = hd->started;
        s->continues = cont;
        s->result[0] = rec.fitness;
        s->result[1] = rec.normalS[0];
        s->result[2] = rec.normalS[1];
        s->result[3] = rec.depth;
    }
    if (dev) (void)hipFree(dev);
    free(host);
    return (int)e;
}

void ring_profile_print()
{
#if PAIS_RING_PROFILE
    unsigned long long h[8] = {0};
    if (hipMemcpyFromSymbol(h, HIP_SYMBOL(g_ringProf), sizeof(h)) != hipSuccess || h[6] == 0) return;
    const char *nm[6] = {"index (head atomic)", "entry wait", "loads + staging", "evaluation", "fitness store + arrival", "swarm step + publish"};
    double tot = 0;
    for (int k = 0; k < 6; ++k) tot += (double)h[k];
    fprintf(stderr, "[ring profile] %llu tasks, %llu steps; s_memtime ticks per task:\n", h[6], h[7]);
    for (int k = 0; k < 6; ++k)
        fprintf(stderr, "[ring profile]   %-26s %10.1f  (%5.1f %%)%s\n", nm[k], (double)h[k] / (double)h[6], 100.0 * (double)h[k] / tot,
                k == 5 ? "  (per step: see steps)" : "");
    fprintf(stderr, "[ring profile]   per step %.1f ticks\n", h[7] ? (double)h[5] / (double)h[7] : 0.0);
#endif
}
}
```

Baseline: 201,900.

## Fold ring init and iteration tail into setup and after kernels, skip memsets

```diff
diff --git a/include/pais_test_hooks.h b/include/pais_test_hooks.h
--- a/include/pais_test_hooks.h
+++ b/include/pais_test_hooks.h
@@ -24,6 +24,9 @@
 } pais_test_swarm;
 int  pais_test_swarm_step(int device, pais_test_swarm *s, double *swarm);
 
+int  pais_test_ring_scribble(pais_ctx *ctx);
+int  pais_test_ring_dirty(pais_ctx *ctx);
+
 typedef struct pais_test_feature_sizes {
     int32_t octaves, W, H, layers;
     int64_t num_cands, num_fit, num_keypoints;
diff --git a/pais_mvs_amd/csrc/pais_capi.hip b/pais_mvs_amd/csrc/pais_capi.hip
--- a/pais_mvs_amd/csrc/pais_capi.hip
+++ b/pais_mvs_amd/csrc/pais_capi.hip
@@ -88,6 +88,7 @@
     int ringCUs = 0;
     Slice sl[16];
     int *cnt = nullptr, *nextCnt = nullptr;
+    unsigned *ringCtl = nullptr, *nextRingCtl = nullptr;
     const pais_candidate *d_cands = nullptr;
     Timed tp;
     TraceOut *trace = nullptr;
@@ -178,9 +179,11 @@
     DevBuf<double> d_pre;
     DevBuf<unsigned> d_ring;
     DevBuf<unsigned> d_ringCtl;
+    unsigned *ringCtlCur = nullptr;
     PinBuf<unsigned> h_ringCtl;
     DevBuf<int> d_arrive;
     bool ringUsed = false;
+    bool ringDirty = true;
     bool ringSuppressed = false;
     bool ringSuppressOnce = false;
     int ringPendingN = 0;
@@ -429,8 +432,9 @@
     HIPCHK(hipMemset(ctx->d_stat, 0, sizeof(unsigned long long) * 24));
     ctx->stat = ctx->d_stat;
     HIPCHK(ctx->h_counters.alloc(sizeof(int) * 4));
-    HIPCHK(ctx->d_ringCtl.alloc(PAIS_RING_CTL_BYTES * PAIS_RINGS));
-    HIPCHK(hipMemset(ctx->d_ringCtl, 0, PAIS_RING_CTL_BYTES * PAIS_RINGS));
+    HIPCHK(ctx->d_ringCtl.alloc(2 * PAIS_RING_CTL_BYTES * PAIS_RINGS));
+    HIPCHK(hipMemset(ctx->d_ringCtl, 0, 2 * PAIS_RING_CTL_BYTES * PAIS_RINGS));
+    ctx->ringCtlCur = ctx->d_ringCtl;
     HIPCHK(ctx->h_ringCtl.alloc(PAIS_RING_CTL_BYTES * PAIS_RINGS));
     memset(ctx->h_ringCtl, 0, PAIS_RING_CTL_BYTES * PAIS_RINGS);
     ctx->splitAbove = 3L * ctx->numCUs * 12;
@@ -937,6 +941,8 @@
     const DevScene &sc = ctx->sc;
     P.cnt = ctx->d_counters + 4 * (ctx->passSerial & 1);
     P.nextCnt = ctx->d_counters + 4 * ((ctx->passSerial + 1) & 1);
+    P.ringCtl = ctx->d_ringCtl + (PAIS_RING_CTL_BYTES / 4) * PAIS_RINGS * (ctx->passSerial & 1);
+    P.nextRingCtl = ctx->d_ringCtl + (PAIS_RING_CTL_BYTES / 4) * PAIS_RINGS * ((ctx->passSerial + 1) & 1);
     ctx->passSerial++;
     if (P.tp.begin(ctx, ctx->stream, &ctx->evPso)) return -2;
     if (pass > 0)
@@ -957,16 +963,21 @@
     if (P.useRing) P.useIter = false;
     P.ringCUs = ctx->numCUs;
     if (P.useRing) {
+        const size_t ringHad = ctx->d_ring.bytes, arriveHad = ctx->d_arrive.bytes;
         HIPCHK(ctx->d_ring.reserve(ctx->stream, ringNeed));
         HIPCHK(ctx->d_arrive.reserve(ctx->stream, sizeof(int) * PAIS_ARRIVE_STRIDE * (size_t)n));
+        if (ctx->d_ring.bytes != ringHad || ctx->d_arrive.bytes != arriveHad) ctx->ringDirty = true;
+        if (ctx->ringDirty)
+            HIPCHK(pais_launch::ring_clean(ctx->d_ring, ctx->d_ring.bytes, ctx->d_ringCtl, ctx->d_arrive, ctx->d_arrive.bytes, ctx->stream));
+        ctx->ringDirty = true;
     }
     P.usePre = ctx->preMode != 0 && !ctx->arithLiteral && !P.useIter && !P.useTile && !(P.useRing && !pais_launch::pre_ring_ok(P.all.Kmax)) && !P.trace;
     P.all.pre = nullptr;
     if (P.usePre) {
         HIPCHK(ctx->d_pre.reserve(ctx->stream, pais_launch::pre_bytes_per_candidate(Nmax, P.all.Kmax) * (size_t)n));
         P.all.pre = ctx->d_pre;
-        HIPCHK(pais_launch::pso_setup0(sc, P.all));
-    }
+    }
+    if (P.usePre || P.useRing) HIPCHK(pais_launch::pso_setup0(sc, P.all, P.useRing ? ctx->d_ring.p : nullptr, P.ringCtl));
     const int nRun = P.useIter ? (pass == 0 ? n : againCount) : n;
     int S = P.useRing ? 1 : ctx->psoStreams;
     if (nPlan > n) S = (int)((double)S * n / nPlan + 0.5);
@@ -1010,15 +1021,12 @@
     if (P.useRing) {
         if (P.itNext == 0 && itEnd > 0) {
             const unsigned long long ticks = (unsigned long long)(ctx->ringTimeoutMs * 1e5);
-            auto ring = [&](int phase) {
-                return pais_launch::pso_ring(sc, P.all, ctx->d_ring, ctx->d_ringCtl, ctx->d_arrive, ctx->stat, P.ringCUs, phase, ticks);
-            };
-            HIPCHK(ring(0));
             Timed te;
             if (te.begin(ctx, ctx->stream, &ctx->evRing)) return -2;
-            HIPCHK(ring(1));
+            HIPCHK(pais_launch::pso_ring(sc, P.all, ctx->d_ring, P.ringCtl, ctx->d_arrive, ctx->stat, P.ringCUs, ticks));
             if (te.end()) return -2;
-            HIPCHK(hipMemcpyAsync(ctx->h_ringCtl, ctx->d_ringCtl, PAIS_RING_CTL_BYTES * PAIS_RINGS, hipMemcpyDeviceToHost, ctx->stream));
+            HIPCHK(hipMemcpyAsync(ctx->h_ringCtl, P.ringCtl, PAIS_RING_CTL_BYTES * PAIS_RINGS, hipMemcpyDeviceToHost, ctx->stream));
+            ctx->ringCtlCur = P.ringCtl;
             ctx->ringUsed = true;
             ctx->evalLaunches++;
             ctx->eval2Launches++;
@@ -1079,17 +1087,24 @@
 static int pass_close(pais_ctx *ctx, PassPlan &P)
 {
     const DevScene &sc = ctx->sc;
+    pais_launch::IterTail tail{ctx->d_active, P.cnt + 2, P.all.states, P.all.Nmax, P.all.maxIt + 1, 0, P.nSl, {0}, {0}};
     for (int k = 0; k < P.nSl; ++k) {
         const PassPlan::Slice &q = P.sl[k];
-        if (P.useIter)
-            HIPCHK(pais_launch::pso_iter(sc, q.v, ctx->d_active, P.cnt + 2, q.lo, q.hi, ctx->stat, P.all.maxIt + 1, 1, q.parts));
-    }
+        tail.lo[k] = q.lo;
+        tail.parts[k] = q.parts;
+        tail.nRun = q.hi;
+    }
+    const bool useTail = P.useIter && P.nSl > 0;
     if (pass_join(ctx, P)) return -2;
     if (P.tp.end()) return -2;
     ctx->psoLaunches++;
     Timed ta;
     if (ta.begin(ctx, ctx->stream, &ctx->evAfter)) return -2;
-    HIPCHK(pais_launch::after(sc, P.all.recs, P.all.n, ctx->d_hp, P.afterGrid, P.cnt, ctx->stat, P.all.Kmax, ctx->d_ratios, P.nextCnt, ctx->stream));
+    if (P.trace) ctx->ringDirty = true;
+    HIPCHK(pais_launch::after(sc, P.all.recs, P.all.n, ctx->d_hp, P.afterGrid, P.cnt, ctx->stat, P.all.Kmax, ctx->d_ratios, P.nextCnt,
+                              useTail ? &tail : nullptr, P.trace ? nullptr : P.nextRingCtl,
+                              P.useRing ? ctx->d_ring.p : nullptr,
+                              pais_launch::ring_words(P.all.n, P.all.Nmax, P.all.maxIt), P.ringCtl, ctx->stream));
     if (ta.end()) return -2;
     return 0;
 }
@@ -1137,7 +1152,10 @@
     ctx->ringUsed = false;
     unsigned done = 0, err = 0;
     for (int r = 0; r < PAIS_RINGS; ++r) { done += ctx->h_ringCtl[(PAIS_RING_CTL_BYTES / 4) * r + PAIS_RING_CTL_DONE_WORD]; err |= ctx->h_ringCtl[(PAIS_RING_CTL_BYTES / 4) * r + PAIS_RING_CTL_ERROR_WORD]; }
-    if (err == 0 && done == (unsigned)n) return 0;
+    if (err == 0 && done == (unsigned)n) {
+        ctx->ringDirty = false;
+        return 0;
+    }
     ctx->ringFallbacks++;
     if (getenv("PAIS_RING_VERBOSE") || (ctx->ringFallbacks == 1 && ctx->ringTimeoutMs > 0))
         fprintf(stderr, "[pais] k_pso_ring did not complete (error %u, %u of %d runs ended): the batch is re-run with one launch per iteration\n", err, done, n);
@@ -1231,7 +1249,7 @@
 {
     if (!ctx || !d_header) return fail_msg("pais_wire_header_device: bad argument");
     HIPCHK(hipSetDevice(ctx->device));
-    HIPCHK(pais_launch::wire_header(d_header, ctx->ringPendingN > 0 ? ctx->d_ringCtl : nullptr, ctx->ringPendingN, rank, count, host_rc, user_word, ctx->stream));
+    HIPCHK(pais_launch::wire_header(d_header, ctx->ringPendingN > 0 ? ctx->ringCtlCur : nullptr, ctx->ringPendingN, rank, count, host_rc, user_word, ctx->stream));
     return 0;
 }
 
@@ -1241,6 +1259,21 @@
     if (e != hipSuccess) return (int)e;
     return pais_launch::test_swarm_step(s, swarm);
 }
+
+extern "C" int pais_test_ring_scribble(pais_ctx *ctx)
+{
+    if (!ctx) return fail_msg("pais_test_ring_scribble: bad argument");
+    if (ctx->openBatch >= 0) return fail_msg("pais_test_ring_scribble: a batch is open on this context");
+    HIPCHK(hipSetDevice(ctx->device));
+    ctx->ringDirty = true;
+    HIPCHK(hipStreamSynchronize(ctx->stream));
+    if (ctx->d_ring.p) HIPCHK(hipMemsetAsync(ctx->d_ring, 0x5A, ctx->d_ring.bytes, ctx->stream));
+    if (ctx->d_arrive.p) HIPCHK(hipMemsetAsync(ctx->d_arrive, 0x5A, ctx->d_arrive.bytes, ctx->stream));
+    HIPCHK(hipMemsetAsync(ctx->d_ringCtl, 0x5A, ctx->d_ringCtl.bytes, ctx->stream));
+    HIPCHK(hipStreamSynchronize(ctx->stream));
+    return 0;
+}
+extern "C" int pais_test_ring_dirty(pais_ctx *ctx) { return ctx ? (ctx->ringDirty ? 1 : 0) : -1; }
 
 extern "C" int pais_ctx_set_round_hint(pais_ctx *ctx, int n_round)
 {
diff --git a/pais_mvs_amd/csrc/pais_internal.h b/pais_mvs_amd/csrc/pais_internal.h
--- a/pais_mvs_amd/csrc/pais_internal.h
+++ b/pais_mvs_amd/csrc/pais_internal.h
@@ -88,7 +88,7 @@
 
 hipError_t begin(const DevScene &sc, const BatchView &v, const pais_candidate *cands, int *activeList, int *activeCount);
 hipError_t pso_init(const DevScene &sc, const BatchView &v, int *activeList, int *activeCount);
-hipError_t pso_setup0(const DevScene &sc, const BatchView &v);
+hipError_t pso_setup0(const DevScene &sc, const BatchView &v, unsigned *ring, unsigned *ringCtl);
 hipError_t pso_eval(const DevScene &sc, const BatchView &v, int pendingOnly, unsigned long long *verify);
 hipError_t pso_eval_literal(const DevScene &sc, const BatchView &v);
 bool tile_eligible(int Kmax);
@@ -100,10 +100,18 @@
 size_t ring_words(int n, int Nmax, int maxIt);
 bool pre_ring_ok(int Kmax);
 hipError_t pso_ring(const DevScene &sc, const BatchView &v, unsigned *ring, unsigned *ctl, int *arrive, unsigned long long *stat, int waves,
-                    int phase, unsigned long long timeoutTicks);
+                    unsigned long long timeoutTicks);
+hipError_t ring_clean(unsigned *ring, size_t ringBytes, unsigned *ctlSets, int *arrive, size_t arriveBytes, hipStream_t stream);
 void ring_profile_print();
+struct IterTail {
+    const int *activeList, *activeCount;
+    unsigned char *states;
+    int Nmax, L, nRun, nSl;
+    int lo[16], parts[16];
+};
 hipError_t after(const DevScene &sc, pais_patch_result *recs, int n, double *hpScratch, int grid, int *counters,
-                 unsigned long long *stat, int Kmax, double *ratios, int *nextCounters, hipStream_t stream);
+                 unsigned long long *stat, int Kmax, double *ratios, int *nextCounters, const IterTail *tail, unsigned *nextRingCtl,
+                 unsigned *ring, size_t ringWords, const unsigned *ringCtl, hipStream_t stream);
 size_t ncc_lds_bytes(int Kmax);
 bool hp_in_lds(const DevScene &sc, int Kmax);
 hipError_t ncc_batch(const DevScene &sc, const pais_view_state *states, int n, pais_view_result *out, double *tables, int stride,
diff --git a/pais_mvs_amd/csrc/pais_kernels.hip b/pais_mvs_amd/csrc/pais_kernels.hip
--- a/pais_mvs_amd/csrc/pais_kernels.hip
+++ b/pais_mvs_amd/csrc/pais_kernels.hip
@@ -1095,6 +1095,95 @@
         if (p < rl[d]) p = rl[d];
         outP[d] = p;
     }
+}
+
+__device__ __forceinline__ void pso_iter_end_run(const DevScene &sc, pais_patch_result *P, PsoState *hd, const double *gB, double gf, int it,
+                                                 int N, unsigned long long *stat)
+{
+    double nn[3];
+    spherical2normal(gB[0], gB[1], nn);
+    P->fitness = gf;
+    P->normalS[0] = gB[0];
+    P->normalS[1] = gB[1];
+    for (int q = 0; q < 3; ++q) P->normal[q] = nn[q];
+    P->depth = gB[2];
+    const DevCamera &rc = sc.cams[hd->refCam];
+    for (int q = 0; q < 3; ++q) P->center[q] = hd->ray[q] * gB[2] + rc.C[q];
+    P->pso_runs += 1;
+    P->pso_iterations += it;
+    const int evals = N * (1 + it);
+    P->pso_evals += evals;
+    if (gf > sc.cfg.maxFitness) {
+        P->dropped = 1;
+        P->stage = PAIS_STAGE_DONE;
+    } else {
+        P->stage = PAIS_STAGE_AFTER;
+    }
+    hd->active = 0;
+    const int K = hd->K;
+    const unsigned long long perEval = (unsigned long long)(4 * K + 1 + (sc.cfg.adaptiveDistanceEnable ? 8 : 0) +
+                                                            (sc.cfg.adaptiveGradientEnable ? 8 : 0));
+    atomicAdd(&stat[0], (unsigned long long)evals);
+    atomicAdd(&stat[1], (unsigned long long)evals * perEval);
+    atomicAdd(&stat[2], 1ULL);
+}
+__device__ void pso_iter_finish(const DevScene &sc, pais_patch_result *P, PsoState *hd, int Nmax, int L, int parts, unsigned long long *stat,
+                                int lane)
+{
+    const PsoArrays Rb = pso_arrays((unsigned char *)hd, Nmax, (L - 1) & 1);
+    const int jl = lane < Nmax ? lane : 0;
+    const int N = __builtin_amdgcn_readfirstlane(hd->N);
+    const PsoState::IterDyn dr = hd->dyn[(L - 1) & 1];
+    double pos[3], pb[3];
+    for (int d = 0; d < 3; ++d) {
+        pos[d] = Rb.pos[jl][d];
+        pb[d] = Rb.pBest[jl][d];
+    }
+    double fitj;
+    if (parts == 1) {
+        fitj = Rb.fit[jl];
+    } else {
+        double f4[4], w4[4];
+        bool bad = false;
+        for (int a = 0; a < 4; ++a) {
+            f4[a] = Rb.part[jl][2 * a];
+            w4[a] = Rb.part[jl][2 * a + 1];
+            bad = bad || (w4[a] < 0);
+        }
+        fitj = bad ? DBL_MAX : combine_parts(f4, w4);
+    }
+    double pbf = Rb.pBestFit[jl];
+    int it, g;
+    double gf;
+    if (!__builtin_amdgcn_readfirstlane(dr.started)) {
+        pbf = fitj;
+        g = 0;
+        gf = lane_get(pbf, 0);
+        it = 0;
+    } else {
+        if (fitj < pbf) {
+            pbf = fitj;
+            pb[0] = pos[0];
+            pb[1] = pos[1];
+            pb[2] = pos[2];
+        }
+        g = __builtin_amdgcn_readfirstlane(dr.gIdx);
+        gf = dr.gBestFitness;
+        it = __builtin_amdgcn_readfirstlane(dr.iteration) + 1;
+    }
+    if (N <= 32) {
+        swarm_update_gbest(pbf, lane, N, gf, g);
+    } else {
+        for (int j = 0; j < N; ++j) {
+            const double v = lane_get(pbf, j);
+            if (v <= gf) {
+                gf = v;
+                g = j;
+            }
+        }
+    }
+    const double gB[3] = {lane_get(pb[0], g), lane_get(pb[1], g), lane_get(pb[2], g)};
+    if (lane == 0) pso_iter_end_run(sc, P, hd, gB, gf, it, N, stat);
 }
 
 template <int nparts, int NS, bool BYTES, bool ACCR>
@@ -1777,8 +1866,11 @@
     }
 }
 
+struct RingCtl { unsigned head, pad0[15]; unsigned tail, done, total, error, pad1[12]; };
+static_assert(sizeof(RingCtl) == PAIS_RING_CTL_BYTES, "RingCtl layout (pais_internal.h)");
+
 __global__ __launch_bounds__(64) void k_pso_setup0(DevScene sc, unsigned char *states, int n, int Nmax, const unsigned char *evalBlocks,
-                                                   size_t evalBlockBytes, double *pre, int Kmax)
+                                                   size_t evalBlockBytes, double *pre, int Kmax, unsigned *ring, unsigned segWords, RingCtl *ctl)
 {
     extern __shared__ __attribute__((aligned(16))) unsigned char smem0[];
     double(*pos)[3] = (double(*)[3])(smem0 + evalBlockBytes);
@@ -1789,9 +1881,22 @@
     const int nwMax = (int)(evalBlockBytes / 8);
     for (int c = blockIdx.x; c < n; c += gridDim.x) {
         PsoState *hd = (PsoState *)(states + SB * (size_t)c);
-        if (!hd->active) continue;
+        const int active = __builtin_amdgcn_readfirstlane(hd->active);
+        const int N = __builtin_amdgcn_readfirstlane(hd->N);
+        if (ring) {
+            RingCtl *rc = &ctl[c % PAIS_RINGS];
+            unsigned base = 0;
+            if (lane == 0) {
+                atomicAdd(&rc->total, 1u);
+                if (active) base = atomicAdd(&rc->tail, (unsigned)N);
+                else atomicAdd(&rc->done, 1u);
+            }
+            base = (unsigned)__builtin_amdgcn_readfirstlane((int)base);
+            if (active && lane < N && base + (unsigned)N <= segWords)
+                ring[(size_t)(c % PAIS_RINGS) * segWords + base + lane] = ((unsigned)c << 8) | (unsigned)lane;
+        }
+        if (!active || !pre) continue;
         PsoArrays A = pso_arrays((unsigned char *)hd, Nmax);
-        const int N = hd->N;
         const uint64_t *src = (const uint64_t *)(evalBlocks + evalBlockBytes * (size_t)c);
         wave_sync();
         stage_eval_block(smem0, src, nwMax, lane, lane < nwMax ? src[lane] : 0, lane + 64 < nwMax ? src[lane + 64] : 0);
@@ -1804,25 +1909,6 @@
 }
 
 #define PAIS_RING_EMPTY 0xFFFFFFFFu
-struct RingCtl { unsigned head, pad0[15]; unsigned tail, done, total, error, pad1[12]; };
-static_assert(sizeof(RingCtl) == PAIS_RING_CTL_BYTES, "RingCtl layout (pais_internal.h)");
-
-__global__ __launch_bounds__(256) void k_ring_init(unsigned char *states, int n, int Nmax, unsigned *ring, unsigned segWords, RingCtl *ctl)
-{
-    const int c = blockIdx.x * 256 + threadIdx.x;
-    if (c >= n) return;
-    RingCtl *rc = &ctl[c % PAIS_RINGS];
-    atomicAdd(&rc->total, 1u);
-    const PsoState *hd = (const PsoState *)(states + pso_state_bytes(Nmax) * (size_t)c);
-    if (!hd->active) {
-        atomicAdd(&rc->done, 1u);
-        return;
-    }
-    const int N = hd->N;
-    const unsigned base = atomicAdd(&rc->tail, (unsigned)N);
-    unsigned *seg = ring + (size_t)(c % PAIS_RINGS) * segWords;
-    for (int j = 0; j < N; ++j) seg[base + j] = ((unsigned)c << 8) | (unsigned)j;
-}
 
 #ifndef PAIS_RING_PROFILE
 #define PAIS_RING_PROFILE 0
@@ -1955,13 +2041,8 @@
     }
 }
 
-__global__ __launch_bounds__(64) void k_region_ratio(DevScene sc, const pais_patch_result *recs, int n, int stage, double *ratios, int Kmax)
-{
-    const int t = blockIdx.x * 64 + threadIdx.x;
-    const int c = t / Kmax, k = t - c * Kmax;
-    if (c >= n) return;
-    const pais_patch_result *P = &recs[c];
-    if (P->stage != stage || P->dropped || k >= P->num_cam) return;
+__device__ double record_region_ratio(const DevScene &sc, const pais_patch_result *P, int k)
+{
     const int LOD = P->lod, refCam = P->ref_cam;
     const DevCamera &rc = sc.cams[refCam];
     const double s = sc.lodScale[LOD];
@@ -1974,19 +2055,59 @@
     patch_homography(ci == refCam, d, s, sc.cams[ci].KR, sc.cams[ci].KT, nrm, invH, H);
     double pt[2];
     cam_project(sc, refCam, center, pt, LOD);
-    ratios[(size_t)c * PAIS_MAX_VIS + k] = region_ratio(pt[0], pt[1], sc.cfg.patchRadius, H);
+    return region_ratio(pt[0], pt[1], sc.cfg.patchRadius, H);
+}
+__global__ __launch_bounds__(64) void k_region_ratio(DevScene sc, const pais_patch_result *recs, int n, int stage, double *ratios, int Kmax)
+{
+    const int t = blockIdx.x * 64 + threadIdx.x;
+    const int c = t / Kmax, k = t - c * Kmax;
+    if (c >= n) return;
+    const pais_patch_result *P = &recs[c];
+    if (P->stage != stage || P->dropped || k >= P->num_cam) return;
+    ratios[(size_t)c * PAIS_MAX_VIS + k] = record_region_ratio(sc, P, k);
+}
+__global__ __launch_bounds__(64) void k_iter_tail_ratio(DevScene sc, pais_launch::IterTail t, pais_patch_result *recs, unsigned long long *stat,
+                                                        double *ratios)
+{
+    const int lane = threadIdx.x;
+    const size_t SB = pso_state_bytes(t.Nmax);
+    const int nAct = *t.activeCount;
+    const int nRun = t.nRun < nAct ? t.nRun : nAct;
+    for (int lp = blockIdx.x; lp < nRun; lp += gridDim.x) {
+        const int c = t.activeList[lp];
+        pais_patch_result *P = &recs[c];
+        PsoState *hd = (PsoState *)(t.states + SB * (size_t)c);
+        if (__builtin_amdgcn_readfirstlane(hd->active)) {
+            int parts = t.parts[0];
+            for (int k = 1; k < t.nSl; ++k)
+                if (lp >= t.lo[k]) parts = t.parts[k];
+            pso_iter_finish(sc, P, hd, t.Nmax, t.L, parts, stat, lane);
+        }
+        __syncthreads();
+        if (P->stage == PAIS_STAGE_AFTER && !P->dropped && lane < P->num_cam) ratios[(size_t)c * PAIS_MAX_VIS + lane] = record_region_ratio(sc, P, lane);
+    }
 }
 
 template <int PHASE>
 __global__ __launch_bounds__(64 * AFTER_WAVES) void k_after(DevScene sc, pais_patch_result *recs, int n, double *hpScratch,
                                                               int *counters, unsigned long long *stat, int Kmax, double *ratios,
-                                                              int hpInLds, int *nextCounters)
+                                                              int hpInLds, int *nextCounters, unsigned *nextRingCtl, unsigned *ring,
+                                                              unsigned segWords, const unsigned *ringCtl)
 {
     if (PHASE == 2 && nextCounters && blockIdx.x == 0 && threadIdx.x == 0) {
         nextCounters[0] = 0;
         nextCounters[1] = 0;
         nextCounters[2] = 0;
     }
+    if (PHASE == 2 && nextRingCtl && blockIdx.x == 0)
+        for (int i = threadIdx.x; i < (int)(PAIS_RING_CTL_BYTES / 4) * PAIS_RINGS; i += 64 * AFTER_WAVES) nextRingCtl[i] = 0;
+    if (PHASE == 2 && ring)
+        for (int r = 0; r < PAIS_RINGS; ++r) {
+            unsigned tail = ringCtl[(PAIS_RING_CTL_BYTES / 4) * r + 16];
+            if (tail > segWords) tail = segWords;
+            for (unsigned i = blockIdx.x * (64 * AFTER_WAVES) + threadIdx.x; i < tail; i += gridDim.x * (64 * AFTER_WAVES))
+                ring[(size_t)r * segWords + i] = 0xFFFFFFFFu;
+        }
     extern __shared__ __attribute__((aligned(16))) unsigned char smem[];
     pais_patch_result *st = (pais_patch_result *)smem;
     size_t off = (sizeof(pais_patch_result) + 15) & ~(size_t)15;
@@ -2446,12 +2567,16 @@
 #define PAIS_PRE_RING_NS1 0
 #endif
 bool pre_ring_ok(int Kmax) { return PAIS_PRE_RING_NS1 || eval_shape(Kmax) != 2; }
-hipError_t pso_setup0(const DevScene &sc, const BatchView &v)
+static size_t ring_seg_words(int n, int Nmax, int maxIt) { return (size_t)((n + PAIS_RINGS - 1) / PAIS_RINGS) * Nmax * ((size_t)maxIt + 2); }
+size_t ring_words(int n, int Nmax, int maxIt) { return ring_seg_words(n, Nmax, maxIt) * PAIS_RINGS; }
+hipError_t pso_setup0(const DevScene &sc, const BatchView &v, unsigned *ring, unsigned *ringCtl)
 {
     if (v.n <= 0) return hipSuccess;
-    const size_t lds = eval_block_bytes(v.Kmax) + sizeof(double) * 3 * (size_t)v.Nmax + pre_scratch_bytes(v.Nmax);
+    const size_t seg = ring_seg_words(v.n, v.Nmax, v.maxIt);
+    if (ring && (v.Nmax > 64 || seg >= 0xFFFFFFF0ull)) return hipErrorInvalidValue;
+    const size_t lds = v.pre ? eval_block_bytes(v.Kmax) + sizeof(double) * 3 * (size_t)v.Nmax + pre_scratch_bytes(v.Nmax) : 0;
     return launch<k_pso_setup0>(grid_for(v.n, 65536), dim3(64), lds, v.stream, sc, v.states, v.n, v.Nmax, (const unsigned char *)v.evalBlocks,
-                                eval_block_bytes(v.Kmax), v.pre, v.Kmax);
+                                eval_block_bytes(v.Kmax), v.pre, v.Kmax, ring, (unsigned)seg, (RingCtl *)ringCtl);
 }
 hipError_t pso_eval_literal(const DevScene &sc, const BatchView &v)
 {
@@ -2491,24 +2616,20 @@
         return nparts == 4 ? go(Int<4>()) : (nparts == 2 ? go(Int<2>()) : go(Int<1>()));
     });
 }
-static size_t ring_seg_words(int n, int Nmax, int maxIt) { return (size_t)((n + PAIS_RINGS - 1) / PAIS_RINGS) * Nmax * ((size_t)maxIt + 2); }
-size_t ring_words(int n, int Nmax, int maxIt) { return ring_seg_words(n, Nmax, maxIt) * PAIS_RINGS; }
+hipError_t ring_clean(unsigned *ring, size_t ringBytes, unsigned *ctlSets, int *arrive, size_t arriveBytes, hipStream_t stream)
+{
+    hipError_t e = hipMemsetAsync(ring, 0xFF, ringBytes, stream);
+    if (e == hipSuccess) e = hipMemsetAsync(ctlSets, 0, 2 * sizeof(RingCtl) * PAIS_RINGS, stream);
+    if (e == hipSuccess) e = hipMemsetAsync(arrive, 0, arriveBytes, stream);
+    return e;
+}
 hipError_t pso_ring(const DevScene &sc, const BatchView &v, unsigned *ring, unsigned *ctl, int *arrive, unsigned long long *stat, int waves,
-                    int phase, unsigned long long timeoutTicks)
+                    unsigned long long timeoutTicks)
 {
     const int n = v.n, Nmax = v.Nmax, Kmax = v.Kmax;
     if (Nmax > 64) return hipErrorInvalidValue;
-    const size_t words = ring_words(n, Nmax, v.maxIt), seg = ring_seg_words(n, Nmax, v.maxIt);
+    const size_t seg = ring_seg_words(n, Nmax, v.maxIt);
     if (seg >= 0xFFFFFFF0ull) return hipErrorInvalidValue;
-    if (phase == 0) {
-        hipError_t e = hipMemsetAsync(ring, 0xFF, words * sizeof(unsigned), v.stream);
-        if (e != hipSuccess) return e;
-        e = hipMemsetAsync(ctl, 0, sizeof(RingCtl) * PAIS_RINGS, v.stream);
-        if (e != hipSuccess) return e;
-        e = hipMemsetAsync(arrive, 0, sizeof(int) * PAIS_ARRIVE_STRIDE * (size_t)n, v.stream);
-        if (e != hipSuccess) return e;
-        return launch<k_ring_init>(dim3((n + 255) / 256), dim3(256), 0, v.stream, v.states, n, Nmax, ring, (unsigned)seg, (RingCtl *)ctl);
-    }
     return shape_dispatch(sc, Kmax, [&](auto ns, auto bytes, auto accr) {
         constexpr int NS = ns;
         constexpr bool BYTES = bytes, ACCR = accr;
@@ -2547,18 +2668,22 @@
 }
 
 hipError_t after(const DevScene &sc, pais_patch_result *recs, int n, double *hpScratch, int grid, int *counters,
-                 unsigned long long *stat, int Kmax, double *ratios, int *nextCounters, hipStream_t stream)
+                 unsigned long long *stat, int Kmax, double *ratios, int *nextCounters, const IterTail *tail, unsigned *nextRingCtl,
+                 unsigned *ring, size_t ringWords, const unsigned *ringCtl, hipStream_t stream)
 {
     if (n <= 0) return hipSuccess;
     const int hpInLds = hp_in_lds(sc, Kmax) ? 1 : 0;
     const size_t lds = ncc_scratch_bytes(sizeof(pais_patch_result), Kmax) + (hpInLds ? hp_bytes(sc, Kmax) : 0);
     const dim3 rgrid((unsigned)(((long)n * Kmax + 63) / 64)), block(64 * AFTER_WAVES);
-    hipError_t e = launch<k_region_ratio>(rgrid, dim3(64), 0, stream, sc, recs, n, PAIS_STAGE_AFTER, ratios, Kmax);
+    hipError_t e = tail ? launch<k_iter_tail_ratio>(dim3(grid_for(tail->nRun, 65536)), dim3(64), 0, stream, sc, *tail, recs, stat, ratios)
+                        : launch<k_region_ratio>(rgrid, dim3(64), 0, stream, sc, recs, n, PAIS_STAGE_AFTER, ratios, Kmax);
     if (e == hipSuccess)
-        e = launch<k_after<1>>(dim3(grid), block, lds, stream, sc, recs, n, hpScratch, counters, stat, Kmax, ratios, hpInLds, (int *)nullptr);
+        e = launch<k_after<1>>(dim3(grid), block, lds, stream, sc, recs, n, hpScratch, counters, stat, Kmax, ratios, hpInLds, (int *)nullptr,
+                               (unsigned *)nullptr, (unsigned *)nullptr, 0u, (const unsigned *)nullptr);
     if (e == hipSuccess) e = launch<k_region_ratio>(rgrid, dim3(64), 0, stream, sc, recs, n, PAIS_STAGE_AFTER2, ratios, Kmax);
     if (e == hipSuccess)
-        e = launch<k_after<2>>(dim3(grid), block, lds, stream, sc, recs, n, hpScratch, counters, stat, Kmax, ratios, hpInLds, nextCounters);
+        e = launch<k_after<2>>(dim3(grid), block, lds, stream, sc, recs, n, hpScratch, counters, stat, Kmax, ratios, hpInLds, nextCounters,
+                               nextRingCtl, ring, (unsigned)(ringWords / PAIS_RINGS), ringCtl);
     return e;
 }
 hipError_t ncc_batch(const DevScene &sc, const pais_view_state *states, int n, pais_view_result *out, double *tables, int stride,
```

Result: no change. 203,500, median of 4 (+0.8%).
